# apcamargo/genomad

Hardware: AMD Instinct MI355X
Metric: 6 kbp windows classified/sec (higher is better)
Workload: dtype f16x3tk (conv2 read from a 137 GB table of all 14-mers in HBM - x2[t] is a function of the bases t-10 .. t+3 -, head A's pair products from an (entry, 9-mer) table, head A's y @ w_v rows from a 9-mer table, all exact f32; conv3 by Toom-Cook F(3,6) with split-f16 MFMA, 3 products per operand pair, f3

## Files before the change

genomad_amd/_lib.py:

```python
import ctypes as C
import os
from pathlib import Path

_HERE = Path(__file__).resolve().parent
LIB_PATH = Path(os.environ.get("GENOMAD_AMD_LIB", _HERE / "csrc" / "libgenomad_nn_hip.so"))

WINDOW, TOKENS, DEPTH, CH = 6000, 5997, 257, 128
PATCHES, PATCH_SIZE, POOLED, FEAT, HIDDEN, CLASSES = 2100, 4, 749, 256, 512, 3
EMBED_DIM = 512
EMB_F32, EMB_BF16 = 0, 1
EMB_DTYPES = {"f32": EMB_F32, "bf16": EMB_BF16}

PREC_F32, PREC_BF16X3, PREC_BF16, PREC_F16C8, PREC_F16X3, PREC_F16C6, PREC_F16X3TC, PREC_F16X3TK = 0, 1, 2, 3, 4, 5, 6, 7
PRECISIONS = {"f32": PREC_F32, "bf16x3": PREC_BF16X3, "f16x3": PREC_F16X3, "f16c6": PREC_F16C6, "f16x3tc": PREC_F16X3TC,
              "f16x3tk": PREC_F16X3TK}
OUT_OF_TOLERANCE = {"f16c6": 1.2e-4}
DEFAULT_PRECISION = "f16x3tc"
ERR_ARG, ERR_HIP, ERR_STATE, ERR_WEIGHTS, ERR_NOMEM = -1, -2, -3, -4, -5
OH_U8, OH_BF16, OH_F32 = 0, 1, 2
STRAND_FORWARD, STRAND_REVERSE, STRAND_BOTH = 0, 1, 2
STRANDS = {"forward": STRAND_FORWARD, "reverse": STRAND_REVERSE, "both": STRAND_BOTH}
K_FUSED, K_BACKEND, K_ENCODER, K_F32_FRONT, K_ATTR_HEAD, K_ATTR_CONTRIB, K_REGIONS = 0, 1, 2, 3, 4, 5, 6

_f32p = C.POINTER(C.c_float)
_i32p = C.POINTER(C.c_int32)


class IglooWeights(C.Structure):
    _fields_ = [("patches", _i32p), ("w_mult", _f32p), ("w_summer", _f32p), ("w_bias", _f32p),
                ("w_qk", _f32p), ("w_v", _f32p)]


class DenseBN(C.Structure):
    _fields_ = [("kernel", _f32p), ("bias", _f32p), ("gamma", _f32p), ("beta", _f32p),
                ("mean", _f32p), ("var", _f32p)]


class Weights(C.Structure):
    _fields_ = [("conv1_kernel", _f32p), ("conv1_bias", _f32p), ("conv2_kernel", _f32p),
                ("conv2_bias", _f32p), ("conv3_kernel", _f32p), ("conv3_bias", _f32p),
                ("igloo_a", IglooWeights), ("igloo_b", IglooWeights), ("enc", DenseBN),
                ("head", DenseBN), ("out_kernel", _f32p), ("out_bias", _f32p)]


class Taps(C.Structure):
    _fields_ = [(k, _f32p) for k in ("x1", "x2", "x3", "m_a", "m_b", "yp_a", "yp_b",
                                     "alpha_a", "alpha_b", "feat")]


_vp, _i64, _int, _sz, _u64 = C.c_void_p, C.c_int64, C.c_int, C.c_size_t, C.c_uint64
SIGNATURES = {
    "gnn_last_error": (C.c_char_p, []),
    "gnn_version": (_int, []),
    "gnn_has_experimental": (_int, []),
    "gnn_device_count": (_int, [C.POINTER(_int)]),
    "gnn_create": (_int, [_int, C.POINTER(_vp)]),
    "gnn_destroy": (_int, [_vp]),
    "gnn_sync": (_int, [_vp]),
    "gnn_device_info": (_int, [_vp, C.c_char_p, _sz, C.POINTER(_int), C.POINTER(_i64)]),
    "gnn_device_mem_info": (_int, [_vp, C.POINTER(_i64), C.POINTER(_i64)]),
    "gnn_device_pci_bus_id": (_int, [_vp, C.c_char_p, _sz]),
    "gnn_load_weights": (_int, [_vp, C.POINTER(Weights)]),
    "gnn_build_kmer_tables": (_int, [_vp, _i64]),
    "gnn_has_kmer_tables": (_int, [_vp]),
    "gnn_drop_kmer_tables": (_int, [_vp]),
    "gnn_kmer_tables_bytes": (_i64, []),
    "gnn_debug_kmer_table_row": (_int, [_vp, _int, _u64, _vp]),
    "gnn_dev_alloc": (_int, [_vp, _sz, C.POINTER(_vp)]),
    "gnn_dev_free": (_int, [_vp, _vp]),
    "gnn_memcpy_h2d": (_int, [_vp, _vp, _vp, _sz]),
    "gnn_memcpy_d2h": (_int, [_vp, _vp, _vp, _sz]),
    "gnn_tokenize": (_int, [_vp, _vp, _i64, _vp]),
    "gnn_tokenize_dev": (_int, [_vp, _vp, _i64, _vp]),
    "gnn_onehot_dev": (_int, [_vp, _vp, _i64, _int, _vp]),
    "gnn_classify": (_int, [_vp, _vp, _i64, _int, _vp]),
    "gnn_classify_dev": (_int, [_vp, _vp, _i64, _int, _vp]),
    "gnn_classify_dev_async": (_int, [_vp, _vp, _i64, _int, _vp]),
    "gnn_classify_flush": (_int, [_vp]),
    "gnn_segment_mean": (_int, [_vp, _vp, _vp, _i64, _i64, _vp]),
    "gnn_span_byte_count": (_int, [_vp, _vp, _vp, _vp, _i64, _int, _vp]),
    "gnn_classify_spans": (_int, [_vp, _vp, _vp, _vp, _i64, _int, _vp]),
    "gnn_classify_contigs": (_int, [_vp, _vp, _int, _i64, _vp, _i64, _int, _int, _vp, _vp, _i64, C.POINTER(_i64)]),
    "gnn_classify_contigs_embed": (_int, [_vp, _vp, _int, _i64, _vp, _i64, _int, _int, _vp, _vp, _i64, C.POINTER(_i64), _vp]),
    "gnn_scan_plan": (_int, [_vp, _i64, _int, _int, C.POINTER(_i64), C.POINTER(_i64), _vp, _vp, _vp, _vp]),
    "gnn_scan_contigs": (_int, [_vp, _vp, _int, _i64, _vp, _i64, _int, _int, _int, _vp, _vp, _i64, _vp, _vp, _i64, _vp]),
    "gnn_revcomp_spans_dev": (_int, [_vp, _vp, _vp, _vp, _i64, _vp]),
    "gnn_classify_contigs_strand": (_int, [_vp, _vp, _int, _i64, _vp, _i64, _int, _int, _vp, _vp, _i64, C.POINTER(_i64), _vp, _int, _vp,
                                           _vp]),
    "gnn_scan_contigs_strand": (_int, [_vp, _vp, _int, _i64, _vp, _i64, _int, _int, _int, _vp, _vp, _i64, _vp, _vp, _i64, _vp, _int, _vp,
                                       _vp]),
    "gnn_occlusion_plan": (_int, [_vp, _i64, _int, _int, C.POINTER(_i64), C.POINTER(_i64), _vp, _vp, _vp, _vp]),
    "gnn_occlude_spans_dev": (_int, [_vp, _vp, _vp, _vp, _vp, _vp, _i64, _vp]),
    "gnn_occlude_contigs": (_int, [_vp, _vp, _int, _i64, _vp, _i64, _int, _int, _int, _vp, _vp, _i64, _vp, _i64, _vp]),
    "gnn_attribute": (_int, [_vp, _vp, _i64, _int, _int, _vp, _vp, _vp, _vp]),
    "gnn_attribute_dev": (_int, [_vp, _vp, _i64, _int, _int, _vp, _vp, _vp, _vp]),
    "gnn_attribute_contigs": (_int, [_vp, _vp, _int, _i64, _vp, _i64, _int, _int, _int, _vp, _i64, _vp, _vp, _vp, _vp, _vp]),
    "gnn_call_regions": (_int, [_vp, _vp, _vp, _i64, C.c_double, _vp, _vp, _vp, _vp, _vp, _vp, _vp, _i64, C.POINTER(_i64)]),
    "gnn_region_states_dev": (_int, [_vp, _vp, _vp, _i64, C.c_double, _vp]),
    "gnn_debug_set_region_tile": (_int, [_vp, _int]),
    "gnn_embed": (_int, [_vp, _vp, _i64, _int, _int, _vp, _vp]),
    "gnn_embed_dev": (_int, [_vp, _vp, _i64, _int, _int, _vp, _vp]),
    "gnn_debug_forward": (_int, [_vp, _vp, _i64, _int, _vp, C.POINTER(Taps)]),
    "gnn_synth_windows_dev": (_int, [_vp, _u64, _i64, _i64, _vp]),
    "gnn_profile_enable": (_int, [_vp, _int]),
    "gnn_profile_reset": (_int, [_vp]),
    "gnn_profile_get": (_int, [_vp, _int, C.POINTER(C.c_double), C.POINTER(_i64)]),
    "gnn_set_chunk": (_int, [_vp, _i64]),
    "gnn_phase_cycles": (_int, [_vp, _int, C.POINTER(C.c_uint64)]),
    "gnn_mfma_probe": (_int, [_vp, _int, C.POINTER(C.c_double)]),
    "gnn_mfma_probe_kind": (_int, [_vp, _int, _int, C.POINTER(C.c_double)]),
    "gnn_fused_rows_per_step": (_int, [_int]),
    "gnn_debug_set_pad_skip": (_int, [_vp, _int]),
    "gnn_debug_set_time_split": (_int, [_vp, _int]),
    "gnn_debug_last_split": (_int, [_vp, C.POINTER(_int)]),
    "gnn_debug_pack_c6": (_int, [_f32p, _int, _int, C.POINTER(C.c_uint32), _sz, C.POINTER(_sz)]),
    "gnn_crc32c": (C.c_uint32, [_vp, _sz]),
    "gnn_fasta_scan": (_int, [_vp, _i64, C.POINTER(C.c_int64), C.POINTER(C.c_int64), C.POINTER(C.c_int)]),
    "gnn_fasta_pack": (_int, [_vp, _i64, _int, _vp, _vp, _vp, _vp, _i64, C.POINTER(C.c_int64)]),
    "gnn_fasta_accession_digests": (_int, [_vp, _i64, _vp, _i64, C.POINTER(C.c_int64), C.POINTER(C.c_int)]),
    "gnn_comm_unique_id": (_int, [_vp]),
    "gnn_comm_init": (_int, [_vp, _int, _int, _vp]),
    "gnn_comm_destroy": (_int, [_vp]),
    "gnn_comm_info": (_int, [_vp, C.POINTER(_int), C.POINTER(_int)]),
    "gnn_comm_gather_dev": (_int, [_vp, _vp, _vp, _sz, _int]),
    "gnn_comm_gather": (_int, [_vp, _vp, _vp, _sz, _int]),
    "gnn_comm_allgather": (_int, [_vp, _vp, _vp, _sz]),
    "gnn_comm_allreduce_max": (_int, [_vp, C.POINTER(C.c_double), _int]),
    "gnn_comm_barrier": (_int, [_vp]),
    "gnn_branch_attention": (_int, [_vp, _vp, _vp, _vp, _i64, C.c_double, _vp]),
    "gnn_score_calibration": (_int, [_vp, _vp, _vp, _vp, _vp, _vp, _vp, _vp, _vp, _i64, _vp]),
}

_lib = None


class GnnError(RuntimeError):
    pass


def load():
    global _lib
    if _lib is not None:
        return _lib
    if not LIB_PATH.is_file():
        raise GnnError(
            f"{LIB_PATH} not found: build it with genomad_amd/csrc/build.sh (or "
            "python -c 'import __graft_entry__ as g; g.build()').  There is no CPU fallback.")
    lib = C.CDLL(str(LIB_PATH))
    for name, (res, args) in SIGNATURES.items():
        fn = getattr(lib, name)
        fn.restype, fn.argtypes = res, args
    _lib = lib
    return lib


def check(rc: int):
    if rc != 0:
        msg = load().gnn_last_error()
        raise GnnError(f"libgenomad_nn_hip error {rc}: {msg.decode() if msg else '?'}")
```

genomad_amd/csrc/gnn_api.hip:

```cpp
#include <algorithm>
#include <map>
#include <mutex>
#include <cstdio>
#include <cmath>
#include <cstdlib>
#include <cstring>

#include "gnn_common.h"

namespace gnn {

static thread_local std::string g_last_error;
void set_error(const std::string& msg) { g_last_error = msg; }

bool debug_switch(const char* name) {
    static std::mutex mu;
    static std::map<std::string, bool> seen;
    std::lock_guard<std::mutex> lock(mu);
    auto it = seen.find(name);
    if (it != seen.end()) return it->second;
    const bool on = std::getenv(name) != nullptr;
    if (on)
        std::fprintf(stderr, "libgenomad_nn_hip: debug switch %s is set: NOT the production path (ordering or arithmetic may differ)\n", name);
    seen[name] = on;
    return on;
}

static void free_ws(Workspace& ws) { ws = Workspace(); }

constexpr size_t WS_BYTES_PER_WINDOW = ((size_t)2 * NPAIR + 2 * NP + (size_t)2 * POOLED * C + 4 * POOLED + FEAT) * sizeof(float);
constexpr int64_t MIN_CHUNK = 256;

static int ensure_ws(gnn_ctx* ctx, Workspace& ws, int64_t chunk, int64_t x_chunk) {
    if (ws.chunk < chunk || ws.x_chunk < x_chunk) {
        if (ctx->stream2) GNN_HIP(hipStreamSynchronize(ctx->stream2));
        ctx->back_pending[0] = ctx->back_pending[1] = false;
    }
    if (ws.chunk < chunk) {
        GNN_HIP(hipStreamSynchronize(ctx->stream));
        int rc = ws.mp.reserve((size_t)chunk * 2 * NPAIR);
        if (!rc) rc = ws.m.reserve((size_t)chunk * 2 * NP);
        if (!rc) rc = ws.yp.reserve((size_t)chunk * 2 * POOLED * C);
        if (!rc) rc = ws.logits.reserve((size_t)chunk * 2 * POOLED);
        if (!rc) rc = ws.alpha.reserve((size_t)chunk * 2 * POOLED);
        if (!rc) rc = ws.feat.reserve((size_t)chunk * FEAT);
        if (rc) {
            free_ws(ws);
            return rc;
        }
        ws.chunk = chunk;
    }
    if (ws.x_chunk < x_chunk) {
        GNN_HIP(hipStreamSynchronize(ctx->stream));
        ws.x_chunk = 0;
        for (DevBuf<float>& x : ws.x) x.reset();
        ws.tokens.reset();
        int rc = GNN_OK;
        for (DevBuf<float>& x : ws.x)
            if (!rc) rc = x.reserve((size_t)x_chunk * T * C);
        if (!rc) rc = ws.tokens.reserve((size_t)x_chunk * T);
        if (rc) {
            free_ws(ws);
            return rc;
        }
        ws.x_chunk = x_chunk;
    }
    return GNN_OK;
}

int flush_backend(gnn_ctx* ctx) {
    for (int i = 0; i < 2; ++i)
        if (ctx->back_pending[i]) {
            GNN_HIP(hipStreamWaitEvent(ctx->stream, ctx->ev_back[i], 0));
            ctx->back_pending[i] = false;
        }
    return GNN_OK;
}

int finish_pending(gnn_ctx* ctx) {
    if (ctx->back_pending[0] || ctx->back_pending[1]) {
        GNN_HIP(hipStreamSynchronize(ctx->stream2));
        ctx->back_pending[0] = ctx->back_pending[1] = false;
    }
    return GNN_OK;
}

int check_ctx(gnn_ctx* ctx, bool flush) {
    if (!ctx) {
        set_error("ctx is NULL");
        return GNN_ERR_ARG;
    }
    GNN_HIP(hipSetDevice(ctx->device));
    if (!flush) return GNN_OK;
    static const bool event_wait = debug_switch("GNN_ASYNC_EVENT_WAIT");
    return event_wait ? flush_backend(ctx) : finish_pending(ctx);
}

void build_conv1_pair_tables(const float* k1, std::vector<float>& pt) {
    pt.assign((size_t)3 * PAIR_ROWS * C, 0.f);
    auto row = [&](int j, int r) { return &pt[((size_t)j * PAIR_ROWS + r) * C]; };
    auto add = [&](float* dst, int k, int tok) {
        const float* src = k1 + ((size_t)k * GNN_DEPTH + tok) * C;
        for (int c = 0; c < C; ++c) dst[c] += src[c];
    };
    for (int j = 0; j < 3; ++j) {
        for (int code5 = 0; code5 < 1024; ++code5) {
            add(row(j, code5), 2 * j, 1 + (code5 >> 2));
            add(row(j, code5), 2 * j + 1, 1 + (code5 & 255));
        }
        for (int b = 1; b <= 256; ++b) {
            add(row(j, 1024 + b - 1), 2 * j, 0);
            add(row(j, 1024 + b - 1), 2 * j + 1, b);
        }
        for (int a = 1; a <= 256; ++a) {
            add(row(j, 1280 + a - 1), 2 * j, a);
            add(row(j, 1280 + a - 1), 2 * j + 1, 0);
        }
        add(row(j, 1536), 2 * j, 0);
        add(row(j, 1536), 2 * j + 1, 0);
        for (int b = 0; b <= 256; ++b) add(row(j, 1538 + b), 2 * j + 1, b);
    }
}

constexpr int64_t STAGE_MAX_WINDOWS = 32768;
constexpr size_t PIN_BYTES = (size_t)8 << 20;

static int64_t stage_windows(const gnn_ctx* ctx) {
    return (int64_t)std::min({ctx->stage_bases.capacity() / W, ctx->stage_scores.capacity() / GNN_CLASSES,
                              ctx->stage_scores_host.capacity() / GNN_CLASSES});
}

void free_stage(gnn_ctx* ctx) {
    ctx->stage_bases.reset();
    ctx->stage_scores.reset();
    ctx->stage_scores_host.reset();
    ctx->stage_emb.reset();
    ctx->emb_scores.reset();
    ctx->stage_attr.reset();
    for (int i = 0; i < 2; ++i) {
        ctx->pin[i].reset();
        if (ctx->pin_ev[i]) (void)hipEventDestroy(ctx->pin_ev[i]);
        ctx->pin_ev[i] = nullptr;
        ctx->pin_busy[i] = false;
    }
}

static int ensure_stage(gnn_ctx* ctx, int64_t windows) {
    int rc;
    for (int i = 0; i < 2; ++i)
        if (!ctx->pin[i]) {
            if ((rc = ctx->pin[i].reserve(PIN_BYTES))) return rc;
            GNN_HIP(hipEventCreateWithFlags(&ctx->pin_ev[i], hipEventDisableTiming));
        }
    const int64_t have = stage_windows(ctx);
    if (have >= windows) return GNN_OK;
    GNN_HIP(hipStreamSynchronize(ctx->stream));
    const size_t want = (size_t)std::max<int64_t>(windows, std::min<int64_t>(2 * have, STAGE_MAX_WINDOWS));
    ctx->stage_bases.reset();
    ctx->stage_scores.reset();
    ctx->stage_scores_host.reset();
    rc = ctx->stage_bases.reserve(want * W);
    if (!rc) rc = ctx->stage_scores.reserve(want * GNN_CLASSES);
    if (!rc && (rc = ctx->stage_scores_host.reserve(want * GNN_CLASSES))) set_error("hipHostMalloc of the score landing buffer failed");
    if (rc) {
        ctx->stage_bases.reset();
        ctx->stage_scores.reset();
    }
    return rc;
}

static int stage_upload(gnn_ctx* ctx, const uint8_t* src, size_t bytes) {
    int j = 0;
    for (size_t off = 0; off < bytes; off += PIN_BYTES, j ^= 1) {
        const size_t len = std::min(PIN_BYTES, bytes - off);
        if (ctx->pin_busy[j]) GNN_HIP(hipEventSynchronize(ctx->pin_ev[j]));
        std::memcpy(ctx->pin[j], src + off, len);
        GNN_HIP(hipMemcpyAsync(ctx->stage_bases + off, ctx->pin[j], len, hipMemcpyHostToDevice, ctx->stream));
        GNN_HIP(hipEventRecord(ctx->pin_ev[j], ctx->stream));
        ctx->pin_busy[j] = true;
    }
    return GNN_OK;
}

size_t emb_elem_bytes(int emb_dtype) {
    return emb_dtype == GNN_EMB_F32 ? sizeof(float) : emb_dtype == GNN_EMB_BF16 ? sizeof(uint16_t) : 0;
}

int classify_chunks(gnn_ctx* ctx, const uint8_t* bases_dev, int64_t n, int precision, float* scores_dev, bool defer_last,
                    void* emb_dev, int emb_dtype, const AttribOut* attr) {
    if (!ctx->has_weights) {
        set_error("gnn_load_weights has not been called");
        return GNN_ERR_STATE;
    }
    if (precision == GNN_PREC_BF16 || precision == GNN_PREC_F16C8) {
        set_error(std::string(precision == GNN_PREC_BF16 ? "GNN_PREC_BF16" : "GNN_PREC_F16C8") +
                  " was removed in round 6 (it fails the 1e-4 score tolerance; the enum value is kept so that old callers get this error)");
        return GNN_ERR_STATE;
    }
    if (precision != GNN_PREC_F32 && precision != GNN_PREC_BF16X3 && precision != GNN_PREC_F16X3 && precision != GNN_PREC_F16C6 &&
        precision != GNN_PREC_F16X3TC && precision != GNN_PREC_F16X3TK) {
        set_error("unknown precision " + std::to_string(precision));
        return GNN_ERR_ARG;
    }
    if (precision == GNN_PREC_F16X3TK && !(ctx->w.tk_x2_tbl && ctx->w.tk_mpa_tbl)) {
        set_error("GNN_PREC_F16X3TK needs the k-mer tables: call gnn_build_kmer_tables first (it answers GNN_ERR_NOMEM on a device without ~190 GB free)");
        return GNN_ERR_STATE;
    }
    const bool f32 = precision == GNN_PREC_F32;
    int64_t chunk = std::min<int64_t>(f32 ? ctx->chunk_f32 : ctx->chunk_fused, std::max<int64_t>(n, 1));
    if (!f32 && ctx->ws.chunk < chunk) {
        if (!ctx->chunk_explicit) {
            size_t free_b = 0, total_b = 0;
            if (hipMemGetInfo(&free_b, &total_b) == hipSuccess) {
                const int64_t cap = std::max<int64_t>(MIN_CHUNK, (int64_t)(free_b / 4 / WS_BYTES_PER_WINDOW) / MIN_CHUNK * MIN_CHUNK);
                if (cap < chunk) {
                    std::fprintf(stderr, "libgenomad_nn_hip: %lld windows per launch need %.1f GB of workspace, %.1f GB of device memory are free: "
                                 "using launches of %lld windows (gnn_set_chunk overrides)\n", (long long)chunk,
                                 chunk * (double)WS_BYTES_PER_WINDOW / 1e9, free_b / 1e9, (long long)cap);
                    chunk = cap;
                }
            }
        }
    }
    int rc = ensure_ws(ctx, ctx->ws, chunk, f32 ? chunk : 0);
    while (rc == GNN_ERR_NOMEM && !f32 && chunk > MIN_CHUNK) {
        chunk = std::max<int64_t>(MIN_CHUNK, chunk / 2);
        std::fprintf(stderr, "libgenomad_nn_hip: workspace allocation failed, retrying with launches of %lld windows\n", (long long)chunk);
        rc = ensure_ws(ctx, ctx->ws, chunk, 0);
    }
    if (rc) return rc;
    if (!f32 && chunk < std::min<int64_t>(ctx->chunk_fused, std::max<int64_t>(n, 1))) ctx->chunk_fused = chunk;
    if (attr && ctx->attr_g.capacity() < (size_t)chunk * FEAT * GNN_CLASSES) {
        if (ctx->stream2) GNN_HIP(hipStreamSynchronize(ctx->stream2));
        GNN_HIP(hipStreamSynchronize(ctx->stream));
        if ((rc = ctx->attr_g.reserve((size_t)chunk * FEAT * GNN_CLASSES))) return rc;
    }
    static const bool allow_overlap = !debug_switch("GNN_NO_BACKEND_OVERLAP");
    static const bool chunk_overlap = debug_switch("GNN_BACKEND_OVERLAP");
    const bool pending = ctx->back_pending[0] || ctx->back_pending[1];
    if (pending && (f32 || !allow_overlap)) {
        if ((rc = flush_backend(ctx))) return rc;
    }
    bool overlap = allow_overlap && !f32 && ((chunk_overlap && n > chunk) || defer_last || pending);
    if (overlap && ctx->alt_failed_chunk > 0 && chunk >= ctx->alt_failed_chunk && ctx->ws_alt.chunk < chunk) {
        if ((rc = flush_backend(ctx))) return rc;
        overlap = false;
    }
    if (overlap && (rc = ensure_ws(ctx, ctx->ws_alt, chunk, 0)) == GNN_ERR_NOMEM) {
        std::fprintf(stderr, "libgenomad_nn_hip: no device memory for the second workspace of %lld windows: asynchronous calls run in order "
                     "(back end not overlapped) from here on\n", (long long)chunk);
        ctx->alt_failed_chunk = chunk;
        if ((rc = flush_backend(ctx))) return rc;
        overlap = false;
    } else if (rc) {
        return rc;
    }
    if (overlap) {
        if (!ctx->stream2) {
            GNN_HIP(hipStreamCreateWithFlags(&ctx->stream2, hipStreamNonBlocking));
            for (int i = 0; i < 2; ++i) {
                GNN_HIP(hipEventCreateWithFlags(&ctx->ev_front[i], hipEventDisableTiming));
                GNN_HIP(hipEventCreateWithFlags(&ctx->ev_back[i], hipEventDisableTiming));
            }
        }
    }
    struct StreamGuard {
        gnn_ctx* c;
        hipStream_t main;
        ~StreamGuard() { c->stream = main; }
    } guard{ctx, ctx->stream};
    for (int64_t a = 0; a < n; a += chunk) {
        const int64_t m = std::min(chunk, n - a);
        const uint8_t* b = bases_dev + a * W;
        if (!f32 && (reinterpret_cast<uintptr_t>(b) & 3u)) {
            if (ctx->align_buf.capacity() < (size_t)m * W) {
                GNN_HIP(hipStreamSynchronize(guard.main));
                if ((rc = ctx->align_buf.reserve((size_t)chunk * W))) return rc;
            }
            GNN_HIP(hipMemcpyAsync(ctx->align_buf, b, (size_t)m * W, hipMemcpyDeviceToDevice, guard.main));
            b = ctx->align_buf;
        }
        const int buf = ctx->buf_cur;
        if (overlap && ctx->back_pending[buf]) {
            GNN_HIP(hipStreamWaitEvent(guard.main, ctx->ev_back[buf], 0));
            ctx->back_pending[buf] = false;
        }
        static const bool poison = debug_switch("GNN_DEBUG_POISON");
        if (poison) {
            const Workspace& ws = ctx->ws;
            const size_t mm = (size_t)std::min<int64_t>(m, ws.chunk);
            auto fill = [&](float* p, size_t per_window) -> int {
                if (p && mm) GNN_HIP(hipMemsetAsync(p, 0xFF, mm * per_window * sizeof(float), guard.main));
                return GNN_OK;
            };
            if ((rc = fill(ws.mp, 2 * NPAIR)) || (rc = fill(ws.m, 2 * NP)) || (rc = fill(ws.yp, (size_t)2 * POOLED * C)) ||
                (rc = fill(ws.logits, 2 * POOLED)) || (rc = fill(ws.alpha, 2 * POOLED)) || (rc = fill(ws.feat, FEAT)))
                return rc;
            if (emb_dev)
                GNN_HIP(hipMemsetAsync(static_cast<uint8_t*>(emb_dev) + (size_t)a * HID * emb_elem_bytes(emb_dtype), 0xFF,
                                       (size_t)m * HID * emb_elem_bytes(emb_dtype), guard.main));
        }
        if (f32) {
            ProfScope ps(ctx, GNN_K_F32_FRONT);
            if ((rc = launch_front_f32(ctx, b, m))) return rc;
        } else {
            ProfScope ps(ctx, GNN_K_FUSED);
            rc = precision == GNN_PREC_F16X3TK ? launch_front_tk(ctx, b, m)
                 : precision == GNN_PREC_F16X3TC ? launch_front_tc(ctx, b, m)
                 : precision == GNN_PREC_F16C6 ? launch_front_c6(ctx, b, m)
                                               : launch_front_x3(ctx, b, m, precision);
            if (rc) return rc;
        }
        if (overlap) {
            GNN_HIP(hipEventRecord(ctx->ev_front[buf], guard.main));
            ctx->stream = ctx->stream2;
            GNN_HIP(hipStreamWaitEvent(ctx->stream2, ctx->ev_front[buf], 0));
        }
        {
            ProfScope ps(ctx, GNN_K_BACKEND);
            void* emb = emb_dev ? static_cast<uint8_t*>(emb_dev) + (size_t)a * HID * emb_elem_bytes(emb_dtype) : nullptr;
            rc = launch_backend(ctx, m, (precision == GNN_PREC_F16X3TC || precision == GNN_PREC_F16X3TK) ? GNN_PREC_F16X3 : precision,
                                scores_dev ? scores_dev + a * GNN_CLASSES : nullptr, emb, emb_dtype, !attr);
        }
        if (attr && !rc) {
            ProfScope ps(ctx, GNN_K_ATTR_HEAD);
            rc = launch_attrib_head(ctx, m, scores_dev ? scores_dev + a * GNN_CLASSES : nullptr, *attr, a);
        }
        if (attr && !rc) {
            ProfScope ps(ctx, GNN_K_ATTR_CONTRIB);
            rc = launch_attrib_contrib(ctx, m, *attr, a);
        }
        if (overlap) {
            if (!rc) {
                GNN_HIP(hipEventRecord(ctx->ev_back[buf], ctx->stream2));
                ctx->back_pending[buf] = true;
            }
            ctx->stream = guard.main;
            std::swap(ctx->ws, ctx->ws_alt);
            ctx->buf_cur ^= 1;
        }
        if (rc) return rc;
    }
    return defer_last ? GNN_OK : flush_backend(ctx);
}

int check_embed_precision(int precision, const char* fn) {
    if (precision != GNN_PREC_F16C6) return GNN_OK;
    set_error(std::string(fn) + ": GNN_PREC_F16C6 has no embedding path (the frozen mode's dense head runs on the matrix pipe "
              "and is outside the tolerance); use f16x3tc, f16x3tk, f16x3, bf16x3 or f32");
    return GNN_ERR_ARG;
}

}

using namespace gnn;

extern "C" {

const char* gnn_last_error(void) { return g_last_error.c_str(); }

int gnn_version(void) { return 300; }

int gnn_debug_pack_c6(const float* w, int k, int n, uint32_t* out, size_t out_words, size_t* need_words) {
    std::vector<uint32_t> v;
    const int rc = c6_pack_matrix(w, k, n, v);
    if (rc) {
        set_error("gnn_debug_pack_c6: w is NULL or K is not a multiple of 128 or N not a multiple of 32");
        return rc;
    }
    if (need_words) *need_words = v.size();
    if (out) {
        if (out_words < v.size()) {
            set_error("gnn_debug_pack_c6: output buffer too small");
            return GNN_ERR_ARG;
        }
        std::memcpy(out, v.data(), v.size() * sizeof(uint32_t));
    }
    return GNN_OK;
}

int gnn_debug_set_pad_skip(gnn_ctx* ctx, int on) {
    int rc = check_ctx(ctx);
    if (rc) return rc;
    ctx->c6_pad_skip = on != 0;
    return GNN_OK;
}

int gnn_debug_set_time_split(gnn_ctx* ctx, int on) {
    int rc = check_ctx(ctx);
    if (rc) return rc;
    ctx->time_split = on != 0;
    return GNN_OK;
}

int gnn_debug_last_split(gnn_ctx* ctx, int* workgroups_per_window) {
    if (!ctx || !workgroups_per_window) {
        set_error("bad argument to gnn_debug_last_split");
        return GNN_ERR_ARG;
    }
    *workgroups_per_window = ctx->last_split;
    return GNN_OK;
}

int gnn_fused_rows_per_step(int precision) {
    switch (precision) {
        case GNN_PREC_F32: return 0;
        case GNN_PREC_F16C6: return c6_rows_per_step();
        case GNN_PREC_F16X3TC: case GNN_PREC_F16X3TK: return 96;
        case GNN_PREC_BF16X3: case GNN_PREC_F16X3: return FT;
        default: return GNN_ERR_ARG;
    }
}

uint32_t gnn_crc32c(const void* data, size_t n) {
    struct Table {
        uint32_t t[8][256];
        Table() {
            for (uint32_t i = 0; i < 256; ++i) {
                uint32_t c = i;
                for (int k = 0; k < 8; ++k) c = (c >> 1) ^ (0x82F63B78u & (0u - (c & 1u)));
                t[0][i] = c;
            }
            for (uint32_t i = 0; i < 256; ++i)
                for (int s = 1; s < 8; ++s) t[s][i] = (t[s - 1][i] >> 8) ^ t[0][t[s - 1][i] & 0xFF];
        }
    };
    static const Table table;
    const uint32_t(*tab)[256] = table.t;
    const unsigned char* p = static_cast<const unsigned char*>(data);
    uint32_t c = 0xFFFFFFFFu;
    while (n >= 8) {
        uint32_t lo, hi;
        std::memcpy(&lo, p, 4);
        std::memcpy(&hi, p + 4, 4);
        lo ^= c;
        c = tab[7][lo & 0xFF] ^ tab[6][(lo >> 8) & 0xFF] ^ tab[5][(lo >> 16) & 0xFF] ^ tab[4][lo >> 24] ^
            tab[3][hi & 0xFF] ^ tab[2][(hi >> 8) & 0xFF] ^ tab[1][(hi >> 16) & 0xFF] ^ tab[0][hi >> 24];
        p += 8;
        n -= 8;
    }
    while (n--) c = (c >> 8) ^ tab[0][(c ^ *p++) & 0xFF];
    return c ^ 0xFFFFFFFFu;
}

int gnn_device_count(int* count) {
    if (!count) {
        set_error("count is NULL");
        return GNN_ERR_ARG;
    }
    GNN_HIP(hipGetDeviceCount(count));
    return GNN_OK;
}

int gnn_create(int device, gnn_ctx** out) {
    if (!out) {
        set_error("out is NULL");
        return GNN_ERR_ARG;
    }
    *out = nullptr;
    int count = 0;
    GNN_HIP(hipGetDeviceCount(&count));
    if (device < 0 || device >= count) {
        set_error("device " + std::to_string(device) + " out of range (" + std::to_string(count) + " visible)");
        return GNN_ERR_ARG;
    }
    GNN_HIP(hipSetDevice(device));
    hipDeviceProp_t prop;
    GNN_HIP(hipGetDeviceProperties(&prop, device));
    if (std::string(prop.gcnArchName).rfind("gfx950", 0) != 0) {
        set_error(std::string("this library is built for gfx950 only; device is ") + prop.gcnArchName);
        return GNN_ERR_HIP;
    }
    gnn_ctx* ctx = new gnn_ctx();
    ctx->device = device;
    ctx->c6_pad_skip = !debug_switch("GNN_NO_PAD_SKIP");
    ctx->time_split = !debug_switch("GNN_NO_TIME_SPLIT");
    ctx->cu_count = prop.multiProcessorCount;
    hipError_t e = hipStreamCreateWithFlags(&ctx->stream, hipStreamNonBlocking);
    if (e != hipSuccess) {
        set_error(std::string("hipStreamCreate failed: ") + hipGetErrorString(e));
        delete ctx;
        return GNN_ERR_HIP;
    }
    *out = ctx;
    return GNN_OK;
}

int gnn_destroy(gnn_ctx* ctx) {
    if (!ctx) return GNN_OK;
    (void)hipSetDevice(ctx->device);
    if (ctx->stream2) (void)hipStreamSynchronize(ctx->stream2);
    (void)hipStreamSynchronize(ctx->stream);
    if (ctx->comm || ctx->comm_scratch) (void)gnn_comm_destroy(ctx);
    free_contig_ws(ctx);
    free_stage(ctx);
    if (ctx->stream2) {
        for (int i = 0; i < 2; ++i) {
            if (ctx->ev_front[i]) (void)hipEventDestroy(ctx->ev_front[i]);
            if (ctx->ev_back[i]) (void)hipEventDestroy(ctx->ev_back[i]);
        }
        (void)hipStreamDestroy(ctx->stream2);
    }
    for (auto& s : ctx->prof)
        for (auto& pr : s.pending) {
            (void)hipEventDestroy(pr.first);
            (void)hipEventDestroy(pr.second);
        }
    for (hipEvent_t e : ctx->event_pool) (void)hipEventDestroy(e);
    (void)hipStreamDestroy(ctx->stream);
    delete ctx;
    return GNN_OK;
}

int gnn_sync(gnn_ctx* ctx) {
    int rc = check_ctx(ctx);
    if (rc) return rc;
    GNN_HIP(hipStreamSynchronize(ctx->stream));
    return GNN_OK;
}

int gnn_device_info(gnn_ctx* ctx, char* name, size_t name_len, int* cus, int64_t* hbm_bytes) {
    int rc = check_ctx(ctx);
    if (rc) return rc;
    hipDeviceProp_t prop;
    GNN_HIP(hipGetDeviceProperties(&prop, ctx->device));
    if (name && name_len) {
        std::string s = std::string(prop.name) + " (" + prop.gcnArchName + ")";
        std::strncpy(name, s.c_str(), name_len - 1);
        name[name_len - 1] = 0;
    }
    if (cus) *cus = prop.multiProcessorCount;
    if (hbm_bytes) *hbm_bytes = (int64_t)prop.totalGlobalMem;
    return GNN_OK;
}

int gnn_device_pci_bus_id(gnn_ctx* ctx, char* out, size_t out_len) {
    int rc = check_ctx(ctx, false);
    if (rc) return rc;
    if (!out || out_len < 16) {
        set_error("gnn_device_pci_bus_id: out must hold at least 16 bytes");
        return GNN_ERR_ARG;
    }
    GNN_HIP(hipDeviceGetPCIBusId(out, (int)out_len, ctx->device));
    return GNN_OK;
}

int gnn_device_mem_info(gnn_ctx* ctx, int64_t* free_bytes, int64_t* total_bytes) {
    int rc = check_ctx(ctx);
    if (rc) return rc;
    size_t f = 0, t = 0;
    GNN_HIP(hipMemGetInfo(&f, &t));
    if (free_bytes) *free_bytes = (int64_t)f;
    if (total_bytes) *total_bytes = (int64_t)t;
    return GNN_OK;
}

int gnn_set_chunk(gnn_ctx* ctx, int64_t windows_per_chunk) {
    if (!ctx || windows_per_chunk < 1) {
        set_error("bad chunk");
        return GNN_ERR_ARG;
    }
    ctx->chunk_fused = windows_per_chunk;
    ctx->chunk_explicit = true;
    return GNN_OK;
}

int gnn_load_weights(gnn_ctx* ctx, const gnn_weights* w) {
    int rc = check_ctx(ctx);
    if (rc) return rc;
    if (!w) {
        set_error("weights is NULL");
        return GNN_ERR_ARG;
    }
    const void* req[] = {w->conv1_kernel, w->conv1_bias, w->conv2_kernel, w->conv2_bias, w->conv3_kernel,
                         w->conv3_bias,   w->out_kernel, w->out_bias,     w->enc.kernel,  w->enc.bias,
                         w->enc.gamma,    w->enc.beta,   w->enc.mean,     w->enc.var,     w->head.kernel,
                         w->head.bias,    w->head.gamma, w->head.beta,    w->head.mean,   w->head.var};
    for (const void* p : req)
        if (!p) {
            set_error("a weight pointer is NULL");
            return GNN_ERR_ARG;
        }
    if (ctx->has_weights) {
        set_error("weights already loaded into this ctx (create a new ctx)");
        return GNN_ERR_STATE;
    }
    DeviceWeights& d = ctx->w;
    if ((rc = upload(ctx, w->conv1_kernel, (size_t)KS * GNN_DEPTH * C, &d.conv1_k))) return rc;
    if ((rc = upload(ctx, w->conv1_bias, (size_t)C, &d.conv1_b))) return rc;
    const float* ck[2] = {w->conv2_kernel, w->conv3_kernel};
    const float* cb[2] = {w->conv2_bias, w->conv3_bias};
    for (int i = 0; i < 2; ++i) {
        if ((rc = upload(ctx, ck[i], (size_t)KS * C * C, &d.conv_k[i]))) return rc;
        if ((rc = upload(ctx, cb[i], (size_t)C, &d.conv_b[i]))) return rc;
    }
    const gnn_igloo_weights* ig[2] = {&w->igloo_a, &w->igloo_b};
    for (int h = 0; h < 2; ++h) {
        const gnn_igloo_weights* g = ig[h];
        if (!g->patches || !g->w_mult || !g->w_summer || !g->w_bias || !g->w_qk || !g->w_v) {
            set_error("an IGLOO weight pointer is NULL");
            return GNN_ERR_ARG;
        }
        std::vector<int32_t> order(NPAIR);
        for (int i = 0; i < NPAIR; ++i) {
            const int32_t t = g->patches[i];
            if (t < 0 || t >= T) {
                set_error("patch index out of range [0,5997)");
                return GNN_ERR_WEIGHTS;
            }
            order[i] = i;
        }
        std::stable_sort(order.begin(), order.end(),
                         [&](int32_t a, int32_t b) { return g->patches[a] < g->patches[b]; });
        std::vector<float> weff((size_t)NPAIR * C);
        std::vector<int32_t> pos(NPAIR), slot(NPAIR), ptr(FSTEPS + 1, 0);
        for (int e = 0; e < NPAIR; ++e) {
            const int pair = order[e], j = pair % PS;
            pos[e] = g->patches[pair];
            slot[pair] = e;
            ptr[pos[e] / FT + 1] += 1;
            for (int c = 0; c < C; ++c)
                weff[(size_t)e * C + c] = g->w_mult[(size_t)pair * C + c] * g->w_summer[j * C + c];
        }
        for (int s2 = 0; s2 < FSTEPS; ++s2) ptr[s2 + 1] += ptr[s2];
        if ((rc = upload(ctx, weff.data(), weff.size(), &d.weff_sorted[h]))) return rc;
        if ((rc = upload(ctx, pos.data(), pos.size(), &d.pos_sorted[h]))) return rc;
        if ((rc = upload(ctx, slot.data(), slot.size(), &d.slot[h]))) return rc;
        if ((rc = upload(ctx, ptr.data(), ptr.size(), &d.bucket_ptr[h]))) return rc;
        if ((rc = upload(ctx, g->w_bias, (size_t)NP, &d.w_bias[h]))) return rc;
        if ((rc = upload(ctx, g->w_qk, (size_t)NP * POOLED, &d.w_qk[h]))) return rc;
        if ((rc = upload(ctx, g->w_v, (size_t)C * C, &d.w_v[h]))) return rc;
    }
    {
        std::vector<float> pt;
        build_conv1_pair_tables(w->conv1_kernel, pt);
        if ((rc = upload(ctx, pt.data(), pt.size(), &d.conv1_pairs))) return rc;
    }
    auto fold = [&](const gnn_dense_bn& l, int in, float** dk, float** db, uint16_t** dfrag) -> int {
        std::vector<float> k((size_t)in * HID), b(HID);
        for (int o = 0; o < HID; ++o) {
            const float s = l.gamma[o] / std::sqrt(l.var[o] + BN_EPS);
            b[o] = (l.bias[o] - l.mean[o]) * s + l.beta[o];
            for (int i = 0; i < in; ++i) k[(size_t)i * HID + o] = l.kernel[(size_t)i * HID + o] * s;
        }
        int r = upload(ctx, k.data(), k.size(), dk);
        if (r) return r;
        if ((r = upload(ctx, b.data(), b.size(), db))) return r;
        const std::vector<uint16_t> fr = pack_frags(k.data(), in, HID, true);
        return upload(ctx, fr, dfrag);
    };
    if ((rc = fold(w->enc, FEAT, &d.d1_k, &d.d1_b, &d.d1_frag))) return rc;
    if ((rc = fold(w->head, HID, &d.d2_k, &d.d2_b, &d.d2_frag))) return rc;
    if ((rc = upload(ctx, w->out_kernel, (size_t)HID * GNN_CLASSES, &d.d3_k))) return rc;
    if ((rc = upload(ctx, w->out_bias, (size_t)GNN_CLASSES, &d.d3_b))) return rc;
    if ((rc = pack_fused_weights(ctx, w))) return rc;
    if ((rc = pack_fused_c6_weights(ctx, w))) return rc;
    if ((rc = pack_fused_x3_consts(ctx))) return rc;
    if ((rc = pack_fused_tc_weights(ctx, w))) return rc;
    ctx->has_weights = true;
    return GNN_OK;
}

int gnn_build_kmer_tables(gnn_ctx* ctx, int64_t reserve_bytes) {
    int rc = check_ctx(ctx);
    if (rc) return rc;
    if (!ctx->has_weights) {
        set_error("gnn_load_weights has not been called");
        return GNN_ERR_STATE;
    }
    if ((rc = finish_pending(ctx))) return rc;
    const size_t reserve = reserve_bytes >= 0 ? (size_t)reserve_bytes : 2 * (size_t)ctx->chunk_fused * WS_BYTES_PER_WINDOW + ((size_t)8 << 30);
    return build_kmer_tables(ctx, reserve);
}

int gnn_has_kmer_tables(gnn_ctx* ctx) {
    return ctx && ctx->w.tk_x2_tbl && ctx->w.tk_mpa_tbl && ctx->w.tk_pt_tbl && ctx->w.tk_x1t_tbl && ctx->w.tk_yp_const ? 1 : 0;
}

int gnn_drop_kmer_tables(gnn_ctx* ctx) {
    int rc = check_ctx(ctx);
    if (rc) return rc;
    if ((rc = finish_pending(ctx))) return rc;
    GNN_HIP(hipStreamSynchronize(ctx->stream));
    free_kmer_tables(ctx);
    return GNN_OK;
}

int64_t gnn_kmer_tables_bytes(void) { return (int64_t)kmer_tables_bytes(); }

int gnn_debug_kmer_table_row(gnn_ctx* ctx, int which, uint64_t row, float* out_host) {
    int rc = check_ctx(ctx);
    if (rc) return rc;
    if (!gnn_has_kmer_tables(ctx) || !out_host) {
        set_error("gnn_debug_kmer_table_row: no tables / NULL output");
        return GNN_ERR_STATE;
    }
    if (which == 0) {
        if (row > ((uint64_t)1 << 28)) { set_error("14-mer row out of range"); return GNN_ERR_ARG; }
        GNN_HIP(hipMemcpy(out_host, ctx->w.tk_x2_tbl + (size_t)row * C, C * sizeof(float), hipMemcpyDeviceToHost));
    } else {
        const uint64_t e = row >> 32, n = row & 0xffffffffu;
        if (e >= (uint64_t)NPAIR || n > ((uint64_t)1 << 18)) { set_error("(entry, 9-mer) out of range"); return GNN_ERR_ARG; }
        GNN_HIP(hipMemcpy(out_host, ctx->w.tk_mpa_tbl + (size_t)e * (((size_t)1 << 18) + 1) + n, sizeof(float), hipMemcpyDeviceToHost));
    }
    return GNN_OK;
}

int gnn_dev_alloc(gnn_ctx* ctx, size_t bytes, void** dev_ptr) {
    int rc = check_ctx(ctx);
    if (rc) return rc;
    if (!dev_ptr) {
        set_error("dev_ptr is NULL");
        return GNN_ERR_ARG;
    }
    DevBuf<unsigned char> b;
    if ((rc = b.reserve(bytes ? bytes : 1))) return rc;
    *dev_ptr = b.release();
    return GNN_OK;
}

int gnn_dev_free(gnn_ctx* ctx, void* dev_ptr) {
    int rc = check_ctx(ctx);
    if (rc) return rc;
    GNN_HIP(hipStreamSynchronize(ctx->stream));
    if (dev_ptr) GNN_HIP(hipFree(dev_ptr));
    return GNN_OK;
}

int gnn_memcpy_h2d(gnn_ctx* ctx, void* dst_dev, const void* src_host, size_t bytes) {
    int rc = check_ctx(ctx);
    if (rc) return rc;
    GNN_HIP(hipMemcpyAsync(dst_dev, src_host, bytes, hipMemcpyHostToDevice, ctx->stream));
    GNN_HIP(hipStreamSynchronize(ctx->stream));
    return GNN_OK;
}

int gnn_memcpy_d2h(gnn_ctx* ctx, void* dst_host, const void* src_dev, size_t bytes) {
    int rc = check_ctx(ctx);
    if (rc) return rc;
    GNN_HIP(hipMemcpyAsync(dst_host, src_dev, bytes, hipMemcpyDeviceToHost, ctx->stream));
    GNN_HIP(hipStreamSynchronize(ctx->stream));
    return GNN_OK;
}

int gnn_tokenize_dev(gnn_ctx* ctx, const uint8_t* bases_dev, int64_t n, uint16_t* tokens_dev) {
    int rc = check_ctx(ctx);
    if (rc) return rc;
    if (n < 0 || (n > 0 && (!bases_dev || !tokens_dev))) {
        set_error("bad argument to gnn_tokenize_dev");
        return GNN_ERR_ARG;
    }
    if (n == 0) return GNN_OK;
    return launch_tokenize(ctx, bases_dev, n, tokens_dev);
}

int gnn_tokenize(gnn_ctx* ctx, const uint8_t* bases_host, int64_t n, uint16_t* tokens_host) {
    int rc = check_ctx(ctx);
    if (rc) return rc;
    if (n < 0 || (n > 0 && (!bases_host || !tokens_host))) {
        set_error("bad argument to gnn_tokenize");
        return GNN_ERR_ARG;
    }
    if (n == 0) return GNN_OK;
    DevBuf<uint8_t> b;
    DevBuf<uint16_t> t;
    if ((rc = b.reserve((size_t)n * W)) || (rc = t.reserve((size_t)n * T))) return rc;
    rc = gnn_memcpy_h2d(ctx, b, bases_host, (size_t)n * W);
    if (!rc) rc = launch_tokenize(ctx, b, n, t);
    if (!rc) rc = gnn_memcpy_d2h(ctx, tokens_host, t, (size_t)n * T * sizeof(uint16_t));
    return rc;
}

int gnn_onehot_dev(gnn_ctx* ctx, const uint8_t* bases_dev, int64_t n, int dtype, void* out) {
    int rc = check_ctx(ctx);
    if (rc) return rc;
    if (n < 0 || (n > 0 && (!bases_dev || !out)) || dtype < GNN_OH_U8 || dtype > GNN_OH_F32) {
        set_error("bad argument to gnn_onehot_dev");
        return GNN_ERR_ARG;
    }
    if (n == 0) return GNN_OK;
    ProfScope ps(ctx, GNN_K_ENCODER);
    return launch_onehot(ctx, bases_dev, n, dtype, out);
}

int gnn_synth_windows_dev(gnn_ctx* ctx, uint64_t seed, int64_t first, int64_t n, uint8_t* bases_dev) {
    int rc = check_ctx(ctx);
    if (rc) return rc;
    if (n < 0 || first < 0 || (n > 0 && !bases_dev)) {
        set_error("bad argument to gnn_synth_windows_dev");
        return GNN_ERR_ARG;
    }
    if (n == 0) return GNN_OK;
    return launch_synth(ctx, seed, first, n, bases_dev);
}

int gnn_classify_dev(gnn_ctx* ctx, const uint8_t* bases_dev, int64_t n, int precision, float* scores_dev) {
    int rc = check_ctx(ctx);
    if (rc) return rc;
    if (n < 0 || (n > 0 && (!bases_dev || !scores_dev))) {
        set_error("bad argument to gnn_classify_dev");
        return GNN_ERR_ARG;
    }
    if (n == 0) return GNN_OK;
    return classify_chunks(ctx, bases_dev, n, precision, scores_dev);
}

int gnn_classify_dev_async(gnn_ctx* ctx, const uint8_t* bases_dev, int64_t n, int precision, float* scores_dev) {
    int rc = check_ctx(ctx, false);
    if (rc) return rc;
    if (n < 0 || (n > 0 && (!bases_dev || !scores_dev))) {
        set_error("bad argument to gnn_classify_dev_async");
        return GNN_ERR_ARG;
    }
    if (n == 0) return GNN_OK;
    return classify_chunks(ctx, bases_dev, n, precision, scores_dev, true);
}

int gnn_classify_flush(gnn_ctx* ctx) { return check_ctx(ctx); }

static int embed_args(int precision, int emb_dtype, const char* what) {
    if (int rc = check_embed_precision(precision, what)) return rc;
    if (!emb_elem_bytes(emb_dtype)) {
        set_error(std::string(what) + ": unknown gnn_emb_dtype " + std::to_string(emb_dtype));
        return GNN_ERR_ARG;
    }
    return GNN_OK;
}

int gnn_embed_dev(gnn_ctx* ctx, const uint8_t* bases_dev, int64_t n, int precision, int emb_dtype, void* emb_dev,
                  float* scores_dev) {
    int rc = check_ctx(ctx);
    if (rc) return rc;
    if (n < 0 || (n > 0 && (!bases_dev || !emb_dev))) {
        set_error("bad argument to gnn_embed_dev");
        return GNN_ERR_ARG;
    }
    if ((rc = embed_args(precision, emb_dtype, "gnn_embed_dev"))) return rc;
    if (n == 0) return GNN_OK;
    if (!scores_dev) {
        if (ctx->emb_scores.capacity() < (size_t)n * GNN_CLASSES) {
            GNN_HIP(hipStreamSynchronize(ctx->stream));
            if ((rc = ctx->emb_scores.reserve((size_t)n * GNN_CLASSES))) return rc;
        }
        scores_dev = ctx->emb_scores;
    }
    return classify_chunks(ctx, bases_dev, n, precision, scores_dev, false, emb_dev, emb_dtype);
}

int gnn_embed(gnn_ctx* ctx, const uint8_t* bases_host, int64_t n, int precision, int emb_dtype, void* emb_host,
              float* scores_host) {
    int rc = check_ctx(ctx);
    if (rc) return rc;
    if (n < 0 || (n > 0 && (!bases_host || !emb_host))) {
        set_error("bad argument to gnn_embed");
        return GNN_ERR_ARG;
    }
    if ((rc = embed_args(precision, emb_dtype, "gnn_embed"))) return rc;
    if (n == 0) return GNN_OK;
    const int64_t slab = std::min<int64_t>(n, STAGE_MAX_WINDOWS);
    const size_t row = (size_t)HID * emb_elem_bytes(emb_dtype);
    if ((rc = ensure_stage(ctx, slab))) return rc;
    if (ctx->stage_emb.capacity() * sizeof(float) < (size_t)slab * row) {
        GNN_HIP(hipStreamSynchronize(ctx->stream));
        if ((rc = ctx->stage_emb.reserve((size_t)slab * HID))) return rc;
    }
    for (int64_t a0 = 0; a0 < n && !rc; a0 += slab) {
        const int64_t m = std::min(slab, n - a0);
        rc = stage_upload(ctx, bases_host + a0 * W, (size_t)m * W);
        if (!rc) rc = classify_chunks(ctx, ctx->stage_bases, m, precision, ctx->stage_scores, false, ctx->stage_emb, emb_dtype);
        if (!rc) {
            if (scores_host)
                GNN_HIP(hipMemcpyAsync(ctx->stage_scores_host, ctx->stage_scores, (size_t)m * GNN_CLASSES * sizeof(float),
                                       hipMemcpyDeviceToHost, ctx->stream));
            GNN_HIP(hipMemcpyAsync(static_cast<uint8_t*>(emb_host) + (size_t)a0 * row, ctx->stage_emb, (size_t)m * row,
                                   hipMemcpyDeviceToHost, ctx->stream));
            GNN_HIP(hipStreamSynchronize(ctx->stream));
            if (scores_host)
                std::memcpy(scores_host + a0 * GNN_CLASSES, ctx->stage_scores_host, (size_t)m * GNN_CLASSES * sizeof(float));
        }
    }
    return rc;
}

int gnn_attribute_dev(gnn_ctx* ctx, const uint8_t* bases_dev, int64_t n, int precision, int bin, float* contrib_dev, float* bias_dev,
                      float* logits_dev, float* scores_dev) {
    int rc = check_ctx(ctx);
    if (rc) return rc;
    if (n < 0 || (n > 0 && (!bases_dev || !contrib_dev))) {
        set_error("bad argument to gnn_attribute_dev");
        return GNN_ERR_ARG;
    }
    if ((rc = check_attrib_args(precision, bin, "gnn_attribute_dev"))) return rc;
    if (n == 0) return GNN_OK;
    const AttribOut at{bin, contrib_dev, bias_dev, logits_dev};
    return classify_chunks(ctx, bases_dev, n, precision, scores_dev, false, nullptr, GNN_EMB_F32, &at);
}

int gnn_attribute(gnn_ctx* ctx, const uint8_t* bases_host, int64_t n, int precision, int bin, float* contrib_host, float* bias_host,
                  float* logits_host, float* scores_host) {
    int rc = check_ctx(ctx);
    if (rc) return rc;
    if (n < 0 || (n > 0 && (!bases_host || !contrib_host))) {
        set_error("bad argument to gnn_attribute");
        return GNN_ERR_ARG;
    }
    if ((rc = check_attrib_args(precision, bin, "gnn_attribute"))) return rc;
    if (n == 0) return GNN_OK;
    constexpr int64_t ATTR_SLAB = 4096;
    const int64_t slab = std::min<int64_t>(n, ATTR_SLAB);
    const size_t map = (size_t)2 * attrib_bins(bin) * GNN_CLASSES;
    if ((rc = ensure_stage(ctx, slab))) return rc;
    if (ctx->stage_attr.capacity() < (size_t)slab * (map + 2 * GNN_CLASSES)) {
        GNN_HIP(hipStreamSynchronize(ctx->stream));
        if ((rc = ctx->stage_attr.reserve((size_t)slab * (map + 2 * GNN_CLASSES)))) return rc;
    }
    float* const d_contrib = ctx->stage_attr;
    float* const d_bias = d_contrib + (size_t)slab * map;
    float* const d_logits = d_bias + (size_t)slab * GNN_CLASSES;
    const AttribOut at{bin, d_contrib, d_bias, d_logits};
    for (int64_t a0 = 0; a0 < n && !rc; a0 += slab) {
        const int64_t m = std::min(slab, n - a0);
        rc = stage_upload(ctx, bases_host + a0 * W, (size_t)m * W);
        if (!rc) rc = classify_chunks(ctx, ctx->stage_bases, m, precision, ctx->stage_scores, false, nullptr, GNN_EMB_F32, &at);
        if (!rc) {
            const size_t row = (size_t)GNN_CLASSES * sizeof(float);
            if (scores_host) GNN_HIP(hipMemcpyAsync(ctx->stage_scores_host, ctx->stage_scores, (size_t)m * row, hipMemcpyDeviceToHost, ctx->stream));
            GNN_HIP(hipMemcpyAsync(contrib_host + (size_t)a0 * map, d_contrib, (size_t)m * map * sizeof(float), hipMemcpyDeviceToHost, ctx->stream));
            if (bias_host) GNN_HIP(hipMemcpyAsync(bias_host + a0 * GNN_CLASSES, d_bias, (size_t)m * row, hipMemcpyDeviceToHost, ctx->stream));
            if (logits_host) GNN_HIP(hipMemcpyAsync(logits_host + a0 * GNN_CLASSES, d_logits, (size_t)m * row, hipMemcpyDeviceToHost, ctx->stream));
            GNN_HIP(hipStreamSynchronize(ctx->stream));
            if (scores_host) std::memcpy(scores_host + a0 * GNN_CLASSES, ctx->stage_scores_host, (size_t)m * row);
        }
    }
    return rc;
}

int gnn_classify(gnn_ctx* ctx, const uint8_t* bases_host, int64_t n, int precision, float* scores_host) {
    return gnn_debug_forward(ctx, bases_host, n, precision, scores_host, nullptr);
}

int gnn_debug_forward(gnn_ctx* ctx, const uint8_t* bases_host, int64_t n, int precision,
                      float* scores_host, const gnn_taps* taps) {
    int rc = check_ctx(ctx);
    if (rc) return rc;
    if (n < 0 || (n > 0 && (!bases_host || !scores_host))) {
        set_error("bad argument to gnn_classify");
        return GNN_ERR_ARG;
    }
    if (n == 0) return GNN_OK;
    if (taps) {
        const int64_t lim = precision == GNN_PREC_F32 ? ctx->chunk_f32 : ctx->chunk_fused;
        if (n > lim) {
            set_error("gnn_debug_forward with taps: n_windows exceeds one chunk (" + std::to_string(lim) + ")");
            return GNN_ERR_ARG;
        }
        if ((taps->x1 || taps->x2 || taps->x3) && precision != GNN_PREC_F32) {
            set_error("x1/x2/x3 taps exist only on the f32 path (the fused path keeps them in LDS)");
            return GNN_ERR_ARG;
        }
    }
    const int64_t slab = std::min<int64_t>(n, STAGE_MAX_WINDOWS);
    if ((rc = ensure_stage(ctx, slab))) return rc;
    for (int64_t a0 = 0; a0 < n && !rc; a0 += slab) {
        const int64_t m = std::min(slab, n - a0);
        rc = stage_upload(ctx, bases_host + a0 * W, (size_t)m * W);
        if (!rc) rc = classify_chunks(ctx, ctx->stage_bases, m, precision, ctx->stage_scores);
        if (!rc) {
            GNN_HIP(hipMemcpyAsync(ctx->stage_scores_host, ctx->stage_scores, (size_t)m * GNN_CLASSES * sizeof(float),
                                   hipMemcpyDeviceToHost, ctx->stream));
            GNN_HIP(hipStreamSynchronize(ctx->stream));
            std::memcpy(scores_host + a0 * GNN_CLASSES, ctx->stage_scores_host, (size_t)m * GNN_CLASSES * sizeof(float));
        }
    }
    if (!rc && taps && precision != GNN_PREC_F32 && n > ctx->chunk_fused) {
        set_error("gnn_debug_forward with taps: the launch size was reduced to " + std::to_string(ctx->chunk_fused) +
                  " windows for lack of device memory; the taps of " + std::to_string(n) + " windows do not fit one launch");
        return GNN_ERR_STATE;
    }
    if (!rc && taps) {
        const Workspace& ws = ctx->ws;
        auto out = [&](float* dst, const float* src, size_t count) {
            if (dst && !rc) rc = gnn_memcpy_d2h(ctx, dst, src, count * sizeof(float));
        };
        out(taps->x1, ws.x[0], (size_t)n * T * C);
        out(taps->x2, ws.x[1], (size_t)n * T * C);
        out(taps->x3, ws.x[2], (size_t)n * T * C);
        out(taps->feat, ws.feat, (size_t)n * FEAT);
        auto out2 = [&](float* dst_a, float* dst_b, const float* src, size_t per) {
            if ((!dst_a && !dst_b) || rc) return;
            std::vector<float> tmp((size_t)n * 2 * per);
            rc = gnn_memcpy_d2h(ctx, tmp.data(), src, tmp.size() * sizeof(float));
            if (rc) return;
            for (int64_t i = 0; i < n; ++i) {
                if (dst_a) std::memcpy(dst_a + i * per, tmp.data() + (i * 2 + 0) * per, per * sizeof(float));
                if (dst_b) std::memcpy(dst_b + i * per, tmp.data() + (i * 2 + 1) * per, per * sizeof(float));
            }
        };
        out2(taps->yp_a, taps->yp_b, ws.yp, (size_t)POOLED * C);
        out2(taps->alpha_a, taps->alpha_b, ws.alpha, (size_t)POOLED);
        out2(taps->m_a, taps->m_b, ws.m, (size_t)NP);
    }
    return rc;
}

static int upload_spans(gnn_ctx* ctx, const int64_t* starts_host, const int32_t* lens_host, int64_t n,
                        DevBuf<int64_t>& starts_dev, DevBuf<int32_t>& lens_dev) {
    for (int64_t i = 0; i < n; ++i)
        if (starts_host[i] < 0 || lens_host[i] < 0 || lens_host[i] > W) {
            set_error("span " + std::to_string(i) + " has a negative start or a length outside [0, 6000]");
            return GNN_ERR_ARG;
        }
    int rc = starts_dev.reserve((size_t)n);
    if (!rc) rc = lens_dev.reserve((size_t)n);
    if (!rc) rc = gnn_memcpy_h2d(ctx, starts_dev, starts_host, (size_t)n * sizeof(int64_t));
    if (!rc) rc = gnn_memcpy_h2d(ctx, lens_dev, lens_host, (size_t)n * sizeof(int32_t));
    return rc;
}

int gnn_span_byte_count(gnn_ctx* ctx, const uint8_t* seq_dev, const int64_t* starts_host, const int32_t* lens_host,
                        int64_t n, int byte, int32_t* counts_host) {
    int rc = check_ctx(ctx);
    if (rc) return rc;
    if (n < 0 || byte < 0 || byte > 255 || (n > 0 && (!seq_dev || !starts_host || !lens_host || !counts_host))) {
        set_error("bad argument to gnn_span_byte_count");
        return GNN_ERR_ARG;
    }
    if (n == 0) return GNN_OK;
    DevBuf<int64_t> ds;
    DevBuf<int32_t> dl, dc;
    if ((rc = upload_spans(ctx, starts_host, lens_host, n, ds, dl))) return rc;
    rc = dc.reserve((size_t)n);
    if (!rc) rc = launch_span_count(ctx, seq_dev, ds, dl, n, byte, dc);
    if (!rc) rc = gnn_memcpy_d2h(ctx, counts_host, dc, (size_t)n * sizeof(int32_t));
    return rc;
}

int gnn_classify_spans(gnn_ctx* ctx, const uint8_t* seq_dev, const int64_t* starts_host, const int32_t* lens_host,
                       int64_t n, int precision, float* scores_host) {
    int rc = check_ctx(ctx);
    if (rc) return rc;
    if (n < 0 || (n > 0 && (!seq_dev || !starts_host || !lens_host || !scores_host))) {
        set_error("bad argument to gnn_classify_spans");
        return GNN_ERR_ARG;
    }
    if (n == 0) return GNN_OK;
    DevBuf<int64_t> ds;
    DevBuf<int32_t> dl;
    if ((rc = upload_spans(ctx, starts_host, lens_host, n, ds, dl))) return rc;
    const int64_t slab = std::min<int64_t>(n, 4 * std::max<int64_t>(ctx->chunk_fused, 1));
    DevBuf<uint8_t> db;
    DevBuf<float> dsc;
    rc = db.reserve((size_t)slab * W);
    if (!rc) rc = dsc.reserve((size_t)n * GNN_CLASSES);
    for (int64_t a = 0; a < n && !rc; a += slab) {
        const int64_t m = std::min(slab, n - a);
        rc = launch_materialize(ctx, seq_dev, ds + a, dl + a, m, db);
        if (!rc) rc = classify_chunks(ctx, db, m, precision, dsc + a * GNN_CLASSES);
    }
    if (!rc) rc = gnn_memcpy_d2h(ctx, scores_host, dsc, (size_t)n * GNN_CLASSES * sizeof(float));
    return rc;
}

int gnn_revcomp_spans_dev(gnn_ctx* ctx, const uint8_t* seq_dev, const int64_t* starts_host, const int32_t* lens_host,
                          int64_t n, uint8_t* bases_dev_out) {
    int rc = check_ctx(ctx);
    if (rc) return rc;
    if (n < 0 || (n > 0 && (!seq_dev || !starts_host || !lens_host || !bases_dev_out))) {
        set_error("bad argument to gnn_revcomp_spans_dev");
        return GNN_ERR_ARG;
    }
    if ((uintptr_t)bases_dev_out & 3) {
        set_error("gnn_revcomp_spans_dev: bases_dev_out is not 4-byte aligned");
        return GNN_ERR_ARG;
    }
    if (n == 0) return GNN_OK;
    DevBuf<int64_t> ds;
    DevBuf<int32_t> dl;
    if ((rc = upload_spans(ctx, starts_host, lens_host, n, ds, dl))) return rc;
    if ((rc = launch_revcomp(ctx, seq_dev, ds, dl, n, bases_dev_out))) return rc;
    GNN_HIP(hipStreamSynchronize(ctx->stream));
    return GNN_OK;
}

int gnn_profile_enable(gnn_ctx* ctx, int on) {
    if (!ctx) {
        set_error("ctx is NULL");
        return GNN_ERR_ARG;
    }
    ctx->profile = on != 0;
    return GNN_OK;
}

static int drain_profile(gnn_ctx* ctx) {
    GNN_HIP(hipStreamSynchronize(ctx->stream));
    for (auto& s : ctx->prof) {
        for (auto& pr : s.pending) {
            float ms = 0.f;
            GNN_HIP(hipEventElapsedTime(&ms, pr.first, pr.second));
            s.total_ms += ms;
            s.launches += 1;
            ctx->event_pool.push_back(pr.first);
            ctx->event_pool.push_back(pr.second);
        }
        s.pending.clear();
    }
    return GNN_OK;
}

int gnn_phase_cycles(gnn_ctx* ctx, int on, unsigned long long* out16) {
    int rc = check_ctx(ctx);
    if (rc) return rc;
    GNN_HIP(hipStreamSynchronize(ctx->stream));
    if (out16 && ctx->phase_cycles)
        GNN_HIP(hipMemcpy(out16, ctx->phase_cycles, 16 * sizeof(unsigned long long), hipMemcpyDeviceToHost));
    if (on) {
        if ((rc = ctx->phase_cycles.reserve(16))) return rc;
        GNN_HIP(hipMemset(ctx->phase_cycles, 0, 16 * sizeof(unsigned long long)));
    } else {
        ctx->phase_cycles.reset();
    }
    return GNN_OK;
}

int gnn_profile_reset(gnn_ctx* ctx) {
    int rc = check_ctx(ctx);
    if (rc) return rc;
    if ((rc = drain_profile(ctx))) return rc;
    for (auto& s : ctx->prof) {
        s.total_ms = 0.0;
        s.launches = 0;
    }
    return GNN_OK;
}

int gnn_profile_get(gnn_ctx* ctx, int kernel_id, double* total_ms, int64_t* launches) {
    int rc = check_ctx(ctx);
    if (rc) return rc;
    if (kernel_id < 0 || kernel_id >= GNN_K_COUNT) {
        set_error("bad kernel id");
        return GNN_ERR_ARG;
    }
    if ((rc = drain_profile(ctx))) return rc;
    if (total_ms) *total_ms = ctx->prof[kernel_id].total_ms;
    if (launches) *launches = ctx->prof[kernel_id].launches;
    return GNN_OK;
}

}
```

genomad_amd/csrc/gnn_backend.hip:

```cpp
#include <cstdlib>

#include "gnn_common.h"

namespace gnn {

__global__ __launch_bounds__(256) void m_kernel(const float* __restrict__ mp, const float* __restrict__ w_bias0,
                                                const float* __restrict__ w_bias1,
                                                const int32_t* __restrict__ slot0,
                                                const int32_t* __restrict__ slot1, float* __restrict__ m) {
    __shared__ float s[NPAIR];
    const int wi = blockIdx.x, h = blockIdx.y;
    const float* w_bias = h ? w_bias1 : w_bias0;
    const int32_t* slot = h ? slot1 : slot0;
    const float4* src = reinterpret_cast<const float4*>(mp + ((size_t)wi * 2 + h) * NPAIR);
    for (int i = threadIdx.x; i < NPAIR / 4; i += 256) reinterpret_cast<float4*>(s)[i] = src[i];
    __syncthreads();
    for (int p = threadIdx.x; p < NP; p += 256) {
        const int4 sl = reinterpret_cast<const int4*>(slot)[p];
        m[((size_t)wi * 2 + h) * NP + p] = w_bias[p] + s[sl.x] + s[sl.y] + s[sl.z] + s[sl.w];
    }
}

constexpr int LW = 64, LQ = 128, LK = 16;

__global__ __launch_bounds__(256) void logits_kernel(const float* __restrict__ m,
                                                     const float* __restrict__ w_qk0,
                                                     const float* __restrict__ w_qk1, int n,
                                                     float* __restrict__ logits) {
    __shared__ __attribute__((aligned(16))) float ms[LK][LW + 4];
    __shared__ __attribute__((aligned(16))) float qs[LK][LQ];
    const int h = blockIdx.z;
    const float* w_qk = h ? w_qk1 : w_qk0;
    const int w0 = blockIdx.y * LW;
    const int q0 = blockIdx.x * LQ;
    const int tw = threadIdx.x >> 4;
    const int tq = threadIdx.x & 15;
    float acc[4][8];
#pragma unroll
    for (int i = 0; i < 4; ++i)
#pragma unroll
        for (int k = 0; k < 8; ++k) acc[i][k] = 0.f;
    for (int p0 = 0; p0 < NP; p0 += LK) {
        {
            const int w = threadIdx.x >> 2, pq = (threadIdx.x & 3) * 4;
            float4 v = make_float4(0.f, 0.f, 0.f, 0.f);
            if (w0 + w < n && p0 + pq < NP)
                v = *reinterpret_cast<const float4*>(m + ((size_t)(w0 + w) * 2 + h) * NP + p0 + pq);
            ms[pq][w] = v.x;
            ms[pq + 1][w] = v.y;
            ms[pq + 2][w] = v.z;
            ms[pq + 3][w] = v.w;
        }
        for (int i = threadIdx.x; i < LK * LQ; i += 256) {
            const int q = i % LQ, p = i / LQ;
            qs[p][q] = (p0 + p < NP && q0 + q < POOLED) ? w_qk[(size_t)(p0 + p) * POOLED + q0 + q] : 0.f;
        }
        __syncthreads();
#pragma unroll 4
        for (int p = 0; p < LK; ++p) {
            const float4 a = *reinterpret_cast<const float4*>(&ms[p][tw * 4]);
            const float4 b0 = *reinterpret_cast<const float4*>(&qs[p][tq * 4]);
            const float4 b1 = *reinterpret_cast<const float4*>(&qs[p][64 + tq * 4]);
            const float av[4] = {a.x, a.y, a.z, a.w};
            const float bv[8] = {b0.x, b0.y, b0.z, b0.w, b1.x, b1.y, b1.z, b1.w};
#pragma unroll
            for (int i = 0; i < 4; ++i)
#pragma unroll
                for (int k = 0; k < 8; ++k) acc[i][k] = fmaf(av[i], bv[k], acc[i][k]);
        }
        __syncthreads();
    }
#pragma unroll
    for (int i = 0; i < 4; ++i) {
        const int w = w0 + tw * 4 + i;
        if (w >= n) continue;
#pragma unroll
        for (int k = 0; k < 8; ++k) {
            const int q = q0 + (k >> 2) * 64 + tq * 4 + (k & 3);
            if (q < POOLED) logits[((size_t)w * 2 + h) * POOLED + q] = acc[i][k];
        }
    }
}

typedef __bf16 bf16x8 __attribute__((ext_vector_type(8)));
typedef float f32x16 __attribute__((ext_vector_type(16)));

struct QkA {
    float4 v[2][2];
};
struct QkB {
    uint4 v[2][2];
};

__device__ __forceinline__ void qk_load(QkA& a, QkB& b, const float* __restrict__ mrow0, const float* __restrict__ mrow1,
                                        const uint4* __restrict__ bfrag, int ks, int lane) {
    const int k = ks * 16 + (lane >> 5) * 8;
    const float* rows[2] = {mrow0, mrow1};
#pragma unroll
    for (int mb = 0; mb < 2; ++mb) {
        if (k + 8 <= NP) {
            a.v[mb][0] = *reinterpret_cast<const float4*>(rows[mb] + k);
            a.v[mb][1] = *reinterpret_cast<const float4*>(rows[mb] + k + 4);
        } else {
            float t[8];
#pragma unroll
            for (int e = 0; e < 8; ++e) t[e] = k + e < NP ? rows[mb][k + e] : 0.f;
            a.v[mb][0] = make_float4(t[0], t[1], t[2], t[3]);
            a.v[mb][1] = make_float4(t[4], t[5], t[6], t[7]);
        }
    }
    const uint4* bp = bfrag + (size_t)ks * (QK_NBLK * 2 * 64);
#pragma unroll
    for (int nb = 0; nb < 2; ++nb) {
        b.v[nb][0] = bp[nb * 2 * 64];
        b.v[nb][1] = bp[nb * 2 * 64 + 64];
    }
}

template <int PASSES, bool F16>
__device__ __forceinline__ void qk_mfma(const QkA& a, const QkB& b, f32x16 (&acc)[2][2]) {
    typedef float f32x8 __attribute__((ext_vector_type(8)));
    typedef _Float16 f16x8q __attribute__((ext_vector_type(8)));
#pragma unroll
    for (int mb = 0; mb < 2; ++mb) {
        const f32x8 x = {a.v[mb][0].x, a.v[mb][0].y, a.v[mb][0].z, a.v[mb][0].w,
                         a.v[mb][1].x, a.v[mb][1].y, a.v[mb][1].z, a.v[mb][1].w};
        if constexpr (F16) {
            const f16x8q ah = __builtin_convertvector(x, f16x8q);
            const f16x8q al = __builtin_convertvector(x - __builtin_convertvector(ah, f32x8), f16x8q);
#pragma unroll
            for (int nb = 0; nb < 2; ++nb) {
                const f16x8q bh = __builtin_bit_cast(f16x8q, b.v[nb][0]);
                if constexpr (PASSES == 3) {
                    const f16x8q bl = __builtin_bit_cast(f16x8q, b.v[nb][1]);
                    acc[mb][nb] = __builtin_amdgcn_mfma_f32_32x32x16_f16(ah, bl, acc[mb][nb], 0, 0, 0);
                    acc[mb][nb] = __builtin_amdgcn_mfma_f32_32x32x16_f16(al, bh, acc[mb][nb], 0, 0, 0);
                }
                acc[mb][nb] = __builtin_amdgcn_mfma_f32_32x32x16_f16(ah, bh, acc[mb][nb], 0, 0, 0);
            }
        } else {
            const bf16x8 ah = __builtin_convertvector(x, bf16x8);
            const bf16x8 al = __builtin_convertvector(x - __builtin_convertvector(ah, f32x8), bf16x8);
#pragma unroll
            for (int nb = 0; nb < 2; ++nb) {
                const bf16x8 bh = __builtin_bit_cast(bf16x8, b.v[nb][0]);
                if constexpr (PASSES == 3) {
                    const bf16x8 bl = __builtin_bit_cast(bf16x8, b.v[nb][1]);
                    acc[mb][nb] = __builtin_amdgcn_mfma_f32_32x32x16_bf16(ah, bl, acc[mb][nb], 0, 0, 0);
                    acc[mb][nb] = __builtin_amdgcn_mfma_f32_32x32x16_bf16(al, bh, acc[mb][nb], 0, 0, 0);
                }
                acc[mb][nb] = __builtin_amdgcn_mfma_f32_32x32x16_bf16(ah, bh, acc[mb][nb], 0, 0, 0);
            }
        }
    }
}

template <int PASSES, bool F16 = false>
__global__ __launch_bounds__(256) void logits_mfma_kernel(const float* __restrict__ m, const uint4* __restrict__ frag0,
                                                          const uint4* __restrict__ frag1, int n,
                                                          float* __restrict__ logits) {
    const int lane = threadIdx.x & 63, wave = threadIdx.x >> 6;
    const int h = blockIdx.z;
    const int w0 = blockIdx.y * 64;
    const int nb0 = blockIdx.x * 8 + wave * 2;
    const uint4* bfrag = (h ? frag1 : frag0) + (size_t)nb0 * 2 * 64 + lane;
    const float* mrow0 = m + ((size_t)min(w0 + (lane & 31), n - 1) * 2 + h) * NP;
    const float* mrow1 = m + ((size_t)min(w0 + 32 + (lane & 31), n - 1) * 2 + h) * NP;
    f32x16 acc[2][2];
#pragma unroll
    for (int i = 0; i < 2; ++i)
#pragma unroll
        for (int j = 0; j < 2; ++j)
#pragma unroll
            for (int r = 0; r < 16; ++r) acc[i][j][r] = 0.f;
    QkA a0, a1;
    QkB b0, b1;
    qk_load(a0, b0, mrow0, mrow1, bfrag, 0, lane);
#pragma unroll 1
    for (int ks = 0; ks < QK_KSTEPS; ks += 2) {
        qk_load(a1, b1, mrow0, mrow1, bfrag, ks + 1, lane);
        qk_mfma<PASSES, F16>(a0, b0, acc);
        qk_load(a0, b0, mrow0, mrow1, bfrag, min(ks + 2, QK_KSTEPS - 1), lane);
        qk_mfma<PASSES, F16>(a1, b1, acc);
    }
#pragma unroll
    for (int mb = 0; mb < 2; ++mb)
#pragma unroll
        for (int r = 0; r < 16; ++r) {
            const int w = w0 + mb * 32 + (r & 3) + 8 * (r >> 2) + 4 * (lane >> 5);
            if (w >= n) continue;
#pragma unroll
            for (int nb = 0; nb < 2; ++nb) {
                const int q = (nb0 + nb) * 32 + (lane & 31);
                if (q < POOLED) logits[((size_t)w * 2 + h) * POOLED + q] = acc[mb][nb][r];
            }
        }
}

__global__ __launch_bounds__(256) void attn_kernel(const float* __restrict__ logits,
                                                   const float* __restrict__ yp,
                                                   float* __restrict__ alpha_out,
                                                   float* __restrict__ feat) {
    __shared__ float a[POOLED + 3];
    __shared__ float red[256];
    const int wi = blockIdx.x, h = blockIdx.y;
    const float* lg = logits + ((size_t)wi * 2 + h) * POOLED;
    float mx = -INFINITY;
    for (int q = threadIdx.x; q < POOLED; q += 256) {
        const float v = lg[q];
        a[q] = v;
        mx = fmaxf(mx, v);
    }
    red[threadIdx.x] = mx;
    __syncthreads();
    for (int s = 128; s > 0; s >>= 1) {
        if (threadIdx.x < s) red[threadIdx.x] = fmaxf(red[threadIdx.x], red[threadIdx.x + s]);
        __syncthreads();
    }
    mx = red[0];
    __syncthreads();
    float sum = 0.f;
    for (int q = threadIdx.x; q < POOLED; q += 256) {
        const float e = expf(a[q] - mx);
        a[q] = e;
        sum += e;
    }
    red[threadIdx.x] = sum;
    __syncthreads();
    for (int s = 128; s > 0; s >>= 1) {
        if (threadIdx.x < s) red[threadIdx.x] += red[threadIdx.x + s];
        __syncthreads();
    }
    const float inv = 1.f / red[0];
    __syncthreads();
    for (int q = threadIdx.x; q < POOLED; q += 256) {
        const float v = a[q] * inv;
        a[q] = v;
        alpha_out[((size_t)wi * 2 + h) * POOLED + q] = v;
    }
    __syncthreads();
    const int cq = threadIdx.x & 31, g = threadIdx.x >> 5;
    const float4* y = reinterpret_cast<const float4*>(yp + ((size_t)wi * 2 + h) * POOLED * C) + cq;
    float4 acc = make_float4(0.f, 0.f, 0.f, 0.f);
    int q = g;
    for (; q + 24 < POOLED; q += 32) {
        typedef float ntf4 __attribute__((ext_vector_type(4)));
        const ntf4* yn = reinterpret_cast<const ntf4*>(y);
        const ntf4 v0 = __builtin_nontemporal_load(yn + (size_t)q * (C / 4)), v1 = __builtin_nontemporal_load(yn + (size_t)(q + 8) * (C / 4)),
                   v2 = __builtin_nontemporal_load(yn + (size_t)(q + 16) * (C / 4)), v3 = __builtin_nontemporal_load(yn + (size_t)(q + 24) * (C / 4));
        const float a0 = a[q], a1 = a[q + 8], a2 = a[q + 16], a3 = a[q + 24];
        acc.x = fmaf(a0, v0.x, acc.x); acc.y = fmaf(a0, v0.y, acc.y); acc.z = fmaf(a0, v0.z, acc.z); acc.w = fmaf(a0, v0.w, acc.w);
        acc.x = fmaf(a1, v1.x, acc.x); acc.y = fmaf(a1, v1.y, acc.y); acc.z = fmaf(a1, v1.z, acc.z); acc.w = fmaf(a1, v1.w, acc.w);
        acc.x = fmaf(a2, v2.x, acc.x); acc.y = fmaf(a2, v2.y, acc.y); acc.z = fmaf(a2, v2.z, acc.z); acc.w = fmaf(a2, v2.w, acc.w);
        acc.x = fmaf(a3, v3.x, acc.x); acc.y = fmaf(a3, v3.y, acc.y); acc.z = fmaf(a3, v3.z, acc.z); acc.w = fmaf(a3, v3.w, acc.w);
    }
    for (; q < POOLED; q += 8) {
        const float4 v = y[(size_t)q * (C / 4)];
        const float aq = a[q];
        acc.x = fmaf(aq, v.x, acc.x); acc.y = fmaf(aq, v.y, acc.y); acc.z = fmaf(aq, v.z, acc.z); acc.w = fmaf(aq, v.w, acc.w);
    }
    __shared__ float4 part[8][32];
    part[g][cq] = acc;
    __syncthreads();
    if (threadIdx.x < 128) {
        const int c = threadIdx.x;
        float s = 0.f;
#pragma unroll
        for (int k = 0; k < 8; ++k) s += reinterpret_cast<const float*>(&part[k][c >> 2])[c & 3];
        feat[(size_t)wi * FEAT + h * C + c] = s;
    }
}

constexpr int DW = 8;

__device__ __forceinline__ uint16_t f32_to_bf16_rne(float v) {
    const uint32_t u = __float_as_uint(v);
    if ((u & 0x7fffffffu) > 0x7f800000u) return (uint16_t)((u >> 16) | 0x0040u);
    return (uint16_t)((u + 0x7fffu + ((u >> 16) & 1u)) >> 16);
}

template <int EMB>
__global__ __launch_bounds__(512) void dense_kernel(const float* __restrict__ feat,
                                                    const float* __restrict__ d1k, const float* __restrict__ d1b,
                                                    const float* __restrict__ d2k, const float* __restrict__ d2b,
                                                    const float* __restrict__ d3k, const float* __restrict__ d3b,
                                                    int n, float* __restrict__ scores, void* __restrict__ emb) {
    __shared__ float f[DW][FEAT];
    __shared__ float h1[DW][HID];
    __shared__ float h2[DW][HID];
    __shared__ float lg[DW][4];
    const int w0 = blockIdx.x * DW;
    const int j = threadIdx.x;
    for (int i = j; i < DW * FEAT; i += 512) {
        const int w = i / FEAT, k = i % FEAT;
        f[w][k] = (w0 + w < n) ? feat[(size_t)(w0 + w) * FEAT + k] : 0.f;
    }
    __syncthreads();
    float acc[DW];
#pragma unroll
    for (int w = 0; w < DW; ++w) acc[w] = d1b[j];
    for (int k = 0; k < FEAT; ++k) {
        const float wv = d1k[(size_t)k * HID + j];
#pragma unroll
        for (int w = 0; w < DW; ++w) acc[w] = fmaf(f[w][k], wv, acc[w]);
    }
#pragma unroll
    for (int w = 0; w < DW; ++w) h1[w][j] = acc[w] < 0.f ? 0.f : acc[w];
    if constexpr (EMB == GNN_EMB_F32 + 1) {
#pragma unroll
        for (int w = 0; w < DW; ++w)
            if (w0 + w < n) static_cast<float*>(emb)[(size_t)(w0 + w) * HID + j] = acc[w] < 0.f ? 0.f : acc[w];
    } else if constexpr (EMB == GNN_EMB_BF16 + 1) {
#pragma unroll
        for (int w = 0; w < DW; ++w)
            if (w0 + w < n) static_cast<uint16_t*>(emb)[(size_t)(w0 + w) * HID + j] = f32_to_bf16_rne(acc[w] < 0.f ? 0.f : acc[w]);
    }
    __syncthreads();
#pragma unroll
    for (int w = 0; w < DW; ++w) acc[w] = d2b[j];
    for (int k = 0; k < HID; ++k) {
        const float wv = d2k[(size_t)k * HID + j];
#pragma unroll
        for (int w = 0; w < DW; ++w) acc[w] = fmaf(h1[w][k], wv, acc[w]);
    }
#pragma unroll
    for (int w = 0; w < DW; ++w) h2[w][j] = acc[w] < 0.f ? 0.f : acc[w];
    __syncthreads();
    const int wave = j >> 6, lane = j & 63;
    for (int o = wave; o < DW * GNN_CLASSES; o += 8) {
        const int w = o / GNN_CLASSES, cl = o % GNN_CLASSES;
        float s = 0.f;
        for (int k = lane; k < HID; k += 64) s = fmaf(h2[w][k], d3k[(size_t)k * GNN_CLASSES + cl], s);
#pragma unroll
        for (int off = 32; off >= 1; off >>= 1) s += __shfl_xor(s, off, 64);
        if (lane == 0) lg[w][cl] = s + d3b[cl];
    }
    __syncthreads();
    if (j < DW && w0 + j < n) {
        const float a = lg[j][0], b = lg[j][1], c = lg[j][2];
        const float mx = fmaxf(a, fmaxf(b, c));
        const float ea = expf(a - mx), eb = expf(b - mx), ec = expf(c - mx);
        const float inv = 1.f / (ea + eb + ec);
        float* o = scores + (size_t)(w0 + j) * GNN_CLASSES;
        o[0] = ea * inv;
        o[1] = eb * inv;
        o[2] = ec * inv;
    }
}

constexpr int DM_MB = 1;
constexpr int DM_ROWS = 32 * DM_MB;
constexpr int DM_STRIDE = HID + 4;

template <int KSTEPS, bool FROM_LDS>
__device__ __forceinline__ void dense_mfma_layer(const float* __restrict__ a0, int row_stride, const uint4* __restrict__ frag,
                                                 int wave, int lane, f32x16 (&acc)[DM_MB][4]) {
    typedef float f32x8 __attribute__((ext_vector_type(8)));
    typedef _Float16 f16x8 __attribute__((ext_vector_type(8)));
#pragma unroll
    for (int i = 0; i < DM_MB; ++i)
#pragma unroll
        for (int j = 0; j < 4; ++j)
#pragma unroll
            for (int r = 0; r < 16; ++r) acc[i][j][r] = 0.f;
#pragma unroll 2
    for (int ks = 0; ks < KSTEPS; ++ks) {
        const int k = ks * 16 + (lane >> 5) * 8;
        f16x8 ah[DM_MB], al[DM_MB];
#pragma unroll
        for (int mb = 0; mb < DM_MB; ++mb) {
            const float4 lo4 = *reinterpret_cast<const float4*>(a0 + mb * row_stride + k), hi4 = *reinterpret_cast<const float4*>(a0 + mb * row_stride + k + 4);
            const f32x8 x = {lo4.x, lo4.y, lo4.z, lo4.w, hi4.x, hi4.y, hi4.z, hi4.w};
            ah[mb] = __builtin_convertvector(x, f16x8);
            al[mb] = __builtin_convertvector(x - __builtin_convertvector(ah[mb], f32x8), f16x8);
        }
        const uint4* bp = frag + ((size_t)ks * (HID / 32) + wave * 4) * 2 * 64 + lane;
#pragma unroll
        for (int nb = 0; nb < 4; ++nb) {
            const f16x8 bh = __builtin_bit_cast(f16x8, bp[nb * 2 * 64]), bl = __builtin_bit_cast(f16x8, bp[nb * 2 * 64 + 64]);
#pragma unroll
            for (int mb = 0; mb < DM_MB; ++mb) {
                acc[mb][nb] = __builtin_amdgcn_mfma_f32_32x32x16_f16(ah[mb], bl, acc[mb][nb], 0, 0, 0);
                acc[mb][nb] = __builtin_amdgcn_mfma_f32_32x32x16_f16(al[mb], bh, acc[mb][nb], 0, 0, 0);
                acc[mb][nb] = __builtin_amdgcn_mfma_f32_32x32x16_f16(ah[mb], bh, acc[mb][nb], 0, 0, 0);
            }
        }
    }
}

__device__ __forceinline__ void dense_mfma_store(float* __restrict__ hs, const float* __restrict__ bias, int wave, int lane,
                                                 const f32x16 (&acc)[DM_MB][4]) {
#pragma unroll
    for (int nb = 0; nb < 4; ++nb) {
        const int col = (wave * 4 + nb) * 32 + (lane & 31);
        const float b = bias[col];
#pragma unroll
        for (int mb = 0; mb < DM_MB; ++mb)
#pragma unroll
            for (int r = 0; r < 16; ++r) {
                const int row = mb * 32 + (r & 3) + 8 * (r >> 2) + 4 * (lane >> 5);
                const float v = acc[mb][nb][r] + b;
                hs[row * DM_STRIDE + col] = v < 0.f ? 0.f : v;
            }
    }
}

__global__ __launch_bounds__(256) void dense_mfma_kernel(const float* __restrict__ feat, const uint4* __restrict__ f1,
                                                         const float* __restrict__ d1b, const uint4* __restrict__ f2,
                                                         const float* __restrict__ d2b, const float* __restrict__ d3k,
                                                         const float* __restrict__ d3b, int n, float* __restrict__ scores) {
    __shared__ __attribute__((aligned(16))) float hs[DM_ROWS * DM_STRIDE];
    __shared__ float lg[DM_ROWS][4];
    const int lane = threadIdx.x & 63, wave = threadIdx.x >> 6;
    const int w0 = blockIdx.x * DM_ROWS;
    f32x16 acc[DM_MB][4];
    static_assert(DM_MB == 1, "the first layer's row clamp is written for one 32-window block per workgroup");
    dense_mfma_layer<FEAT / 16, false>(feat + (size_t)min(w0 + (lane & 31), n - 1) * FEAT, 32 * FEAT, f1, wave, lane, acc);
    dense_mfma_store(hs, d1b, wave, lane, acc);
    __syncthreads();
    dense_mfma_layer<HID / 16, true>(hs + (lane & 31) * DM_STRIDE, 32 * DM_STRIDE, f2, wave, lane, acc);
    __syncthreads();
    dense_mfma_store(hs, d2b, wave, lane, acc);
    __syncthreads();
    for (int o = wave; o < DM_ROWS * GNN_CLASSES; o += 4) {
        const int w = o / GNN_CLASSES, cl = o % GNN_CLASSES;
        float s = 0.f;
        for (int k = lane; k < HID; k += 64) s = fmaf(hs[w * DM_STRIDE + k], d3k[(size_t)k * GNN_CLASSES + cl], s);
#pragma unroll
        for (int off = 32; off >= 1; off >>= 1) s += __shfl_xor(s, off, 64);
        if (lane == 0) lg[w][cl] = s + d3b[cl];
    }
    __syncthreads();
    const int j = threadIdx.x;
    if (j < DM_ROWS && w0 + j < n) {
        const float a = lg[j][0], b = lg[j][1], c = lg[j][2];
        const float mx = fmaxf(a, fmaxf(b, c));
        const float ea = expf(a - mx), eb = expf(b - mx), ec = expf(c - mx);
        const float inv = 1.f / (ea + eb + ec);
        float* o = scores + (size_t)(w0 + j) * GNN_CLASSES;
        o[0] = ea * inv;
        o[1] = eb * inv;
        o[2] = ec * inv;
    }
}

int launch_backend(gnn_ctx* ctx, int64_t n, int precision, float* scores_dev, void* emb_dev, int emb_dtype, bool dense) {
    if (emb_dev && (precision == GNN_PREC_F16C6 || precision == GNN_PREC_F16C8 || (emb_dtype != GNN_EMB_F32 && emb_dtype != GNN_EMB_BF16))) {
        set_error("embeddings: the dense head of this arithmetic does not produce them (f16c6 is frozen), or a bad gnn_emb_dtype");
        return GNN_ERR_ARG;
    }
    const DeviceWeights& d = ctx->w;
    Workspace& ws = ctx->ws;
    hipLaunchKernelGGL(m_kernel, dim3((unsigned)n, 2), dim3(256), 0, ctx->stream, ws.mp, d.w_bias[0], d.w_bias[1],
                       d.slot[0], d.slot[1], ws.m);
    static_assert(QK_KSTEPS % 2 == 0 && QK_NBLK % 8 == 0, "logits_mfma_kernel tiling");
    static const bool logits_f32 = debug_switch("GNN_LOGITS_F32");
    const dim3 qk_grid(QK_NBLK / 8, (unsigned)((n + 63) / 64), 2);
    const uint4* qf0 = reinterpret_cast<const uint4*>(d.wqk_frag[0]);
    const uint4* qf1 = reinterpret_cast<const uint4*>(d.wqk_frag[1]);
    if (precision == GNN_PREC_BF16X3 || precision == GNN_PREC_F16C8 || precision == GNN_PREC_F16C6)
        hipLaunchKernelGGL(logits_mfma_kernel<3>, qk_grid, dim3(256), 0, ctx->stream, ws.m, qf0, qf1, (int)n, ws.logits);
    else if (precision == GNN_PREC_BF16)
        hipLaunchKernelGGL(logits_mfma_kernel<1>, qk_grid, dim3(256), 0, ctx->stream, ws.m, qf0, qf1, (int)n, ws.logits);
    else if (precision == GNN_PREC_F16X3 && !logits_f32)
        hipLaunchKernelGGL((logits_mfma_kernel<3, true>), qk_grid, dim3(256), 0, ctx->stream, ws.m,
                           reinterpret_cast<const uint4*>(d.wqk_frag_h[0]), reinterpret_cast<const uint4*>(d.wqk_frag_h[1]), (int)n, ws.logits);
    else
        hipLaunchKernelGGL(logits_kernel, dim3((POOLED + LQ - 1) / LQ, (unsigned)((n + LW - 1) / LW), 2), dim3(256), 0,
                           ctx->stream, ws.m, d.w_qk[0], d.w_qk[1], (int)n, ws.logits);
    hipLaunchKernelGGL(attn_kernel, dim3((unsigned)n, 2), dim3(256), 0, ctx->stream, ws.logits, ws.yp, ws.alpha,
                       ws.feat);
    if (!dense) {
        GNN_HIP(hipGetLastError());
        return GNN_OK;
    }
    if (precision != GNN_PREC_F16C6 && precision != GNN_PREC_F16C8) {
        const dim3 grid((unsigned)((n + DW - 1) / DW));
        if (!emb_dev)
            hipLaunchKernelGGL(dense_kernel<0>, grid, dim3(512), 0, ctx->stream, ws.feat, d.d1_k, d.d1_b, d.d2_k, d.d2_b, d.d3_k,
                               d.d3_b, (int)n, scores_dev, nullptr);
        else if (emb_dtype == GNN_EMB_F32)
            hipLaunchKernelGGL(dense_kernel<GNN_EMB_F32 + 1>, grid, dim3(512), 0, ctx->stream, ws.feat, d.d1_k, d.d1_b, d.d2_k, d.d2_b,
                               d.d3_k, d.d3_b, (int)n, scores_dev, emb_dev);
        else
            hipLaunchKernelGGL(dense_kernel<GNN_EMB_BF16 + 1>, grid, dim3(512), 0, ctx->stream, ws.feat, d.d1_k, d.d1_b, d.d2_k, d.d2_b,
                               d.d3_k, d.d3_b, (int)n, scores_dev, emb_dev);
    } else {
        hipLaunchKernelGGL(dense_mfma_kernel, dim3((unsigned)((n + DM_ROWS - 1) / DM_ROWS)), dim3(256), 0, ctx->stream, ws.feat,
                           reinterpret_cast<const uint4*>(d.d1_frag), d.d1_b, reinterpret_cast<const uint4*>(d.d2_frag), d.d2_b,
                           d.d3_k, d.d3_b, (int)n, scores_dev);
    }
    GNN_HIP(hipGetLastError());
    return GNN_OK;
}

__global__ void segment_mean_kernel(const float* __restrict__ scores, const int64_t* __restrict__ ids,
                                    int64_t n, int64_t n_seg, float* __restrict__ out) {
    const int64_t i = (int64_t)blockIdx.x * blockDim.x + threadIdx.x;
    if (i >= n_seg * GNN_CLASSES) return;
    const int64_t seg = i / GNN_CLASSES;
    const int cl = (int)(i % GNN_CLASSES);
    int64_t lo = 0, hi = n;
    while (lo < hi) {
        const int64_t mid = (lo + hi) >> 1;
        if (ids[mid] < seg) lo = mid + 1; else hi = mid;
    }
    const int64_t a = lo;
    hi = n;
    while (lo < hi) {
        const int64_t mid = (lo + hi) >> 1;
        if (ids[mid] <= seg) lo = mid + 1; else hi = mid;
    }
    float s = 0.f;
    for (int64_t k = a; k < lo; ++k) s += scores[k * GNN_CLASSES + cl];
    out[i] = lo > a ? s / (float)(lo - a) : 0.f;
}

}

using namespace gnn;

extern "C" int gnn_segment_mean(gnn_ctx* ctx, const float* scores_host, const int64_t* ids_host, int64_t n,
                                int64_t n_segments, float* out_host) {
    if (!ctx || n < 0 || n_segments < 0 || (n > 0 && (!scores_host || !ids_host)) ||
        (n_segments > 0 && !out_host)) {
        set_error("bad argument to gnn_segment_mean");
        return GNN_ERR_ARG;
    }
    if (n_segments == 0) return GNN_OK;
    for (int64_t i = 1; i < n; ++i)
        if (ids_host[i] < ids_host[i - 1]) {
            set_error("segment ids are not sorted");
            return GNN_ERR_ARG;
        }
    if (n > 0 && (ids_host[0] < 0 || ids_host[n - 1] >= n_segments)) {
        set_error("segment id out of range");
        return GNN_ERR_ARG;
    }
    GNN_HIP(hipSetDevice(ctx->device));
    DevBuf<float> ds, dout;
    DevBuf<int64_t> di;
    int rc = ds.reserve(std::max<size_t>(1, (size_t)n * GNN_CLASSES));
    if (!rc) rc = di.reserve(std::max<size_t>(1, (size_t)n));
    if (!rc) rc = dout.reserve((size_t)n_segments * GNN_CLASSES);
    auto step = [&](hipError_t e, const char* what) {
        if (rc == GNN_OK && e != hipSuccess) {
            set_error(std::string(what) + " failed: " + hipGetErrorString(e));
            rc = GNN_ERR_HIP;
        }
    };
    if (n > 0 && rc == GNN_OK) {
        step(hipMemcpyAsync(ds, scores_host, (size_t)n * GNN_CLASSES * sizeof(float), hipMemcpyHostToDevice, ctx->stream), "copy scores");
        step(hipMemcpyAsync(di, ids_host, (size_t)n * sizeof(int64_t), hipMemcpyHostToDevice, ctx->stream), "copy ids");
    }
    if (rc == GNN_OK) {
        const int64_t threads = n_segments * GNN_CLASSES;
        hipLaunchKernelGGL(segment_mean_kernel, dim3((unsigned)((threads + 255) / 256)), dim3(256), 0, ctx->stream,
                           ds.get(), di.get(), n, n_segments, dout.get());
        step(hipGetLastError(), "segment_mean launch");
        step(hipMemcpyAsync(out_host, dout, (size_t)n_segments * GNN_CLASSES * sizeof(float), hipMemcpyDeviceToHost, ctx->stream), "copy out");
        step(hipStreamSynchronize(ctx->stream), "sync");
    }
    return rc;
}
```

genomad_amd/csrc/gnn_common.h:

```cpp
#pragma once
#include <hip/hip_runtime.h>
#include <stdint.h>
#include <algorithm>
#include <string>
#include <vector>

#include "../../include/genomad_nn.h"
#include "gnn_devmem.h"

namespace gnn {

constexpr int W = GNN_WINDOW;
constexpr int T = GNN_TOKENS;
constexpr int C = GNN_CH;
constexpr int KS = GNN_KSIZE;
constexpr int NP = GNN_PATCHES;
constexpr int PS = GNN_PATCH_SIZE;
constexpr int NPAIR = NP * PS;
constexpr int POOLED = GNN_POOLED;
constexpr int FEAT = GNN_FEAT;
constexpr int HID = GNN_HIDDEN;
constexpr float LRELU = 0.1f;
constexpr float BN_EPS = 1e-3f;

constexpr int FT = 128;
constexpr int FSTEPS = (T + FT - 1) / FT;
constexpr int PAIR_ROWS = 1024 + 256 + 256 + 1 + 1 + 257;
constexpr int QK_KSTEPS = (NP + 15) / 16;
constexpr int QK_NBLK = (POOLED + 31) / 32;

void set_error(const std::string& msg);
bool debug_switch(const char* name);

#define GNN_HIP(call)                                                                          \
    do {                                                                                       \
        hipError_t e_ = (call);                                                                \
        if (e_ != hipSuccess) {                                                                \
            gnn::set_error(std::string(#call) + " failed: " + hipGetErrorString(e_));          \
            return GNN_ERR_HIP;                                                                \
        }                                                                                      \
    } while (0)

struct DeviceWeights {
    float* conv1_k = nullptr;
    float* conv1_b = nullptr;
    float* conv_k[2] = {nullptr, nullptr};
    float* conv_b[2] = {nullptr, nullptr};
    float* weff_sorted[2] = {nullptr, nullptr};
    int32_t* pos_sorted[2] = {nullptr, nullptr};
    int32_t* slot[2] = {nullptr, nullptr};
    int32_t* bucket_ptr[2] = {nullptr, nullptr};
    float* conv1_pairs = nullptr;
    float* w_bias[2] = {nullptr, nullptr};
    float* w_qk[2] = {nullptr, nullptr};
    float* w_v[2] = {nullptr, nullptr};
    float* d1_k = nullptr;
    float* d1_b = nullptr;
    float* d2_k = nullptr;
    float* d2_b = nullptr;
    float* d3_k = nullptr;
    float* d3_b = nullptr;
    uint16_t* d1_frag = nullptr;
    uint16_t* d2_frag = nullptr;
    uint16_t* conv_frag[2] = {nullptr, nullptr};
    uint16_t* wv_frag[2] = {nullptr, nullptr};
    uint16_t* wqk_frag[2] = {nullptr, nullptr};
    uint16_t* wqk_frag_h[2] = {nullptr, nullptr};
    uint16_t* conv_frag_h[2] = {nullptr, nullptr};
    uint16_t* wv_frag_h[2] = {nullptr, nullptr};
    uint32_t* conv_c6[2] = {nullptr, nullptr};
    uint32_t* wv_c6[2] = {nullptr, nullptr};
    float* conv1_pairs6 = nullptr;
    float* weff6[2] = {nullptr, nullptr};
    int32_t* bucket_ptr6[2] = {nullptr, nullptr};
    DevBuf<float> c6_yp_const;
    DevBuf<float> c6_mp_const;
    uint16_t* tc_frag[2] = {nullptr, nullptr};
    float tc_inv_s[2] = {1.f, 1.f};
    int32_t* bucket_ptr96[2] = {nullptr, nullptr};
    DevBuf<float> tc_yp_const;
    DevBuf<float> tc_mp_const;
    DevBuf<float> tc_wva_tbl;
    DevBuf<float> tk_x2_tbl;
    DevBuf<float> tk_mpa_tbl;
    DevBuf<float> tk_x1t_tbl;
    DevBuf<float> tk_pt_tbl;
    DevBuf<float> tk_yp_const;
    DevBuf<float> tk_mp_const;
    DevBuf<float> x3_yp_const[2];
    DevBuf<float> x3_mp_const[2];
};

struct Workspace {
    int64_t chunk = 0;
    DevBuf<uint16_t> tokens;
    DevBuf<float> x[3];
    int64_t x_chunk = 0;
    DevBuf<float> mp;
    DevBuf<float> m;
    DevBuf<float> yp;
    DevBuf<float> logits;
    DevBuf<float> alpha;
    DevBuf<float> feat;
};

constexpr int MIN_TAIL = 2500;
constexpr int MAX_N = 4000;
constexpr int64_t PIECE = 64ll << 20;

struct RegionWorkspace {
    int tile = 256;
    PinnedBuf<int64_t> h_off;
    hipEvent_t tables_read = nullptr;
    DevBuf<int64_t> d_off;
    DevBuf<int64_t> d_transfer, d_entry;
    DevBuf<uint8_t> d_comp, d_exit;
    DevBuf<uint8_t> d_psi;
    DevBuf<float> d_track;
    DevBuf<uint8_t> d_state, d_flag;
    DevBuf<int32_t> d_blk_count;
    DevBuf<int64_t> d_blk_off;
    DevBuf<int64_t> d_r_contig, d_r_lo, d_r_hi, d_r_evidence, d_r_qsum;
    DevBuf<uint8_t> d_r_state;
    ~RegionWorkspace() {
        if (tables_read) (void)hipEventDestroy(tables_read);
    }
};

struct ContigWorkspace {
    hipStream_t copy_stream = nullptr;
    std::vector<hipEvent_t> piece_done;
    std::vector<int64_t> starts, ids;
    std::vector<int32_t> lens, window_n, counts;
    DevBuf<uint8_t> seq;
    DevBuf<int64_t> d_starts, d_ids;
    DevBuf<int32_t> d_lens, d_window_n, d_counts;
    DevBuf<float> d_scores;
    DevBuf<uint8_t> d_bases;
    DevBuf<float> d_out;
    DevBuf<float> d_emb, d_emb_sum;
    DevBuf<int32_t> d_emb_kept;
    std::vector<int64_t> win_off, bin_off;
    DevBuf<int64_t> d_win_off, d_bin_off;
    DevBuf<float> d_track;
    DevBuf<int32_t> d_cover;
    DevBuf<float> d_scores_rev, d_scores_mix, d_slab_scores, d_out_strand;
    DevBuf<float> d_emb_sum_rev;
    DevBuf<int32_t> d_emb_kept_rev;
    std::vector<int64_t> blk_off;
    DevBuf<int64_t> d_blk_off;
    DevBuf<float> d_occ;
    DevBuf<float> d_attr;
    RegionWorkspace regions;

    size_t span_cap() const {
        return std::min({d_starts.capacity(), d_ids.capacity(), d_lens.capacity(), d_window_n.capacity(), d_counts.capacity(),
                         d_scores.capacity() / GNN_CLASSES});
    }
    size_t strand_cap() const { return std::min(d_scores_rev.capacity(), d_scores_mix.capacity()) / GNN_CLASSES; }
    size_t off_cap() const { return std::min(d_win_off.capacity(), d_bin_off.capacity()); }
    size_t bin_cap() const { return std::min(d_track.capacity() / GNN_CLASSES, d_cover.capacity()); }
};

template <typename F>
static inline void for_each_window(int64_t len, int64_t stride, int single_window, F&& f) {
    for (int64_t k = 0; k * stride < len; ++k) {
        const int64_t l = std::min<int64_t>(W, len - k * stride);
        if (l < MIN_TAIL && k > 0) break;
        f(k, l);
        if (l < MIN_TAIL || (single_window && k == 0) || k * stride + W >= len) break;
    }
}

struct WindowWalk {
    int64_t* win_off = nullptr;
    int64_t* bin_off = nullptr;
    int64_t windows = 0, bins = 0;
};
template <typename F>
static int walk_windows(const int64_t* offsets, int64_t n_contigs, int64_t stride, int single_window, WindowWalk& out, F&& f) {
    for (int64_t c = 0; c < n_contigs; ++c)
        if (offsets[c + 1] < offsets[c]) {
            set_error("contig offsets are not non-decreasing");
            return GNN_ERR_ARG;
        }
    out.windows = out.bins = 0;
    if (out.win_off) out.win_off[0] = 0;
    if (out.bin_off) out.bin_off[0] = 0;
    for (int64_t c = 0; c < n_contigs; ++c) {
        const int64_t len = offsets[c + 1] - offsets[c];
        for_each_window(len, stride, single_window, [&](int64_t k, int64_t l) {
            f(c, k, l);
            ++out.windows;
        });
        out.bins += (len + stride - 1) / stride;
        if (out.win_off) out.win_off[c + 1] = out.windows;
        if (out.bin_off) out.bin_off[c + 1] = out.bins;
    }
    return GNN_OK;
}

__host__ __device__ inline bool window_kept(int32_t window_n, int32_t n_count) {
    return window_n == 0 || n_count <= MAX_N;
}

template <typename Tp>
static int reserve_roomy(DevBuf<Tp>& b, size_t need) {
    return b.reserve(need, need / 4 + 64);
}

template <typename... Bufs>
static void reset_all(Bufs&... bufs) {
    (bufs.reset(), ...);
}

template <typename... P, typename... A>
static int launch_1d(void (*kernel)(P...), int64_t cells, hipStream_t stream, A&&... args) {
    hipLaunchKernelGGL(kernel, dim3((unsigned)((cells + 255) / 256)), dim3(256), 0, stream, static_cast<P>(args)...);
    GNN_HIP(hipGetLastError());
    return GNN_OK;
}

struct AttribOut {
    int bin;
    float* contrib;
    float* bias;
    float* logits;
};
static inline int attrib_bins(int bin) { return (POOLED + bin - 1) / bin; }

struct ProfileSlot {
    double total_ms = 0.0;
    int64_t launches = 0;
    std::vector<std::pair<hipEvent_t, hipEvent_t>> pending;
};

}

struct gnn_ctx {
    int device = 0;
    hipStream_t stream = nullptr;
    bool has_weights = false;
    gnn::DeviceWeights w;
    gnn::Workspace ws;
    gnn::Workspace ws_alt;
    hipStream_t stream2 = nullptr;
    hipEvent_t ev_front[2] = {nullptr, nullptr}, ev_back[2] = {nullptr, nullptr};
    bool back_pending[2] = {false, false};
    int buf_cur = 0;
    int64_t chunk_fused = 16384;
    int64_t alt_failed_chunk = 0;
    bool chunk_explicit = false;
    int64_t chunk_f32 = 64;
    bool profile = false;
    gnn::ProfileSlot prof[GNN_K_COUNT];
    std::vector<hipEvent_t> event_pool;
    std::vector<gnn::DevBuf<unsigned char>> owned;
    int cu_count = 0;
    int last_split = 1;
    bool time_split = true;
    bool c6_pad_skip = true;
    gnn::DevBuf<unsigned long long> phase_cycles;
    gnn::ContigWorkspace* contig_ws = nullptr;
    gnn::DevBuf<uint8_t> stage_bases;
    gnn::DevBuf<float> stage_emb;
    gnn::DevBuf<float> emb_scores;
    gnn::DevBuf<float> stage_attr;
    gnn::DevBuf<float> attr_g;
    gnn::DevBuf<float> stage_scores;
    gnn::PinnedBuf<float> stage_scores_host;
    gnn::PinnedBuf<uint8_t> pin[2];
    hipEvent_t pin_ev[2] = {nullptr, nullptr};
    bool pin_busy[2] = {false, false};
    gnn::DevBuf<uint8_t> align_buf;
    void* comm = nullptr;
    int comm_ranks = 1, comm_rank = 0;
    gnn::DevBuf<unsigned char> comm_scratch;
};

namespace gnn {

struct ProfScope {
    gnn_ctx* ctx;
    int id;
    hipEvent_t a = nullptr, b = nullptr;
    ProfScope(gnn_ctx* c, int kid) : ctx(c), id(kid) {
        if (!ctx->profile) return;
        auto take = [&]() {
            hipEvent_t e = nullptr;
            if (!ctx->event_pool.empty()) {
                e = ctx->event_pool.back();
                ctx->event_pool.pop_back();
            } else if (hipEventCreate(&e) != hipSuccess) {
                e = nullptr;
            }
            return e;
        };
        a = take();
        b = take();
        if (a) (void)hipEventRecord(a, ctx->stream);
    }
    ~ProfScope() {
        if (!ctx->profile || !a || !b) return;
        (void)hipEventRecord(b, ctx->stream);
        ctx->prof[id].pending.emplace_back(a, b);
    }
};

template <typename Tp>
int upload(gnn_ctx* ctx, const Tp* host, size_t count, Tp** dev) {
    DevBuf<unsigned char> b;
    if (int rc = b.upload(reinterpret_cast<const unsigned char*>(host), count * sizeof(Tp))) return rc;
    *dev = reinterpret_cast<Tp*>(b.get());
    ctx->owned.emplace_back(std::move(b));
    return GNN_OK;
}
template <typename Tp>
int upload(gnn_ctx* ctx, const std::vector<Tp>& v, Tp** dev) {
    return upload(ctx, v.data(), v.size(), dev);
}

template <typename Run>
int all_n_consts(gnn_ctx* ctx, DevBuf<float>& yp, DevBuf<float>& mp, Run&& run) {
    DevBuf<uint8_t> bn;
    int rc = bn.reserve(W);
    if (!rc) rc = yp.reserve((size_t)2 * POOLED * C);
    if (!rc) rc = mp.reserve((size_t)2 * NPAIR);
    if (rc) return rc;
    hipError_t e = hipMemsetAsync(bn, 'N', W, ctx->stream);
    if (e == hipSuccess) {
        run(bn.get(), yp.get(), mp.get());
        e = hipGetLastError();
    }
    if (e == hipSuccess) e = hipStreamSynchronize(ctx->stream);
    if (e == hipSuccess) return GNN_OK;
    yp.reset();
    mp.reset();
    set_error(std::string("the all-N window's launch failed: ") + hipGetErrorString(e));
    return GNN_ERR_HIP;
}

int launch_tokenize(gnn_ctx* ctx, const uint8_t* bases, int64_t n, uint16_t* tokens);
int launch_onehot(gnn_ctx* ctx, const uint8_t* bases, int64_t n, int dtype, void* out);
int launch_synth(gnn_ctx* ctx, uint64_t seed, int64_t first, int64_t n, uint8_t* bases);
int launch_span_count(gnn_ctx* ctx, const uint8_t* seq, const int64_t* starts, const int32_t* lens, int64_t n,
                      int byte, int32_t* counts);
int launch_materialize(gnn_ctx* ctx, const uint8_t* seq, const int64_t* starts, const int32_t* lens, int64_t n,
                       uint8_t* bases);
int launch_revcomp(gnn_ctx* ctx, const uint8_t* seq, const int64_t* starts, const int32_t* lens, int64_t n,
                   uint8_t* bases);
int launch_occlude(gnn_ctx* ctx, const uint8_t* seq, const int64_t* starts, const int32_t* lens, const int64_t* blk_off,
                   int64_t n_windows, int64_t pair0, int block, const int32_t* lo, const int32_t* hi, int64_t n_rows, uint8_t* bases);
int launch_masked_segment_mean(gnn_ctx* ctx, const float* scores, const int64_t* ids, const int32_t* window_n, const int32_t* counts,
                               int64_t n, int64_t n_seg, float* out);
int launch_front_f32(gnn_ctx* ctx, const uint8_t* bases, int64_t n);
int launch_backend(gnn_ctx* ctx, int64_t n, int precision, float* scores_dev, void* emb_dev = nullptr, int emb_dtype = GNN_EMB_F32,
                   bool dense = true);
int check_attrib_args(int precision, int bin, const char* fn);
int launch_attrib_head(gnn_ctx* ctx, int64_t n, float* scores_dev, const AttribOut& at, int64_t row0);
int launch_attrib_contrib(gnn_ctx* ctx, int64_t n, const AttribOut& at, int64_t row0);
int classify_chunks(gnn_ctx* ctx, const uint8_t* bases_dev, int64_t n, int precision, float* scores_dev, bool defer_last = false,
                    void* emb_dev = nullptr, int emb_dtype = GNN_EMB_F32, const AttribOut* attr = nullptr);
size_t emb_elem_bytes(int emb_dtype);
int flush_backend(gnn_ctx* ctx);
int finish_pending(gnn_ctx* ctx);
int check_ctx(gnn_ctx* ctx, bool flush = true);
int check_embed_precision(int precision, const char* fn);
void free_stage(gnn_ctx* ctx);

struct ContigIn {
    gnn_ctx* ctx;
    const uint8_t* seq;
    int seq_on_host;
    int64_t seq_bytes;
    const int64_t* offsets;
    int64_t n_contigs;
    int single_window, precision;
    int64_t stride;
};

class SeqFeed {
  public:
    int begin(const ContigIn& in, ContigWorkspace& w);
    int upto(int64_t end);
    const uint8_t* dev() const { return dev_; }

  private:
    gnn_ctx* ctx_ = nullptr;
    ContigWorkspace* w_ = nullptr;
    const uint8_t* host_ = nullptr;
    const uint8_t* dev_ = nullptr;
    int64_t bytes_ = 0, n_pieces_ = 0, uploaded_ = 0;
};

int contig_begin(const ContigIn& in, const char* fn, bool outputs_ok, ContigWorkspace** w);
int plan_windows(const ContigIn& in, ContigWorkspace& w, bool csr, int block);
int upload_span_table(gnn_ctx* ctx, ContigWorkspace& w);
int slab_pass(const ContigIn& in, ContigWorkspace& w, SeqFeed& feed, int64_t a, int64_t m, bool fwd, bool rev, float* scores,
              float* emb, const AttribOut* attr = nullptr);
int64_t kept_windows(const ContigWorkspace& w, uint8_t* mask_or_null, int64_t* ids_or_null);
void free_contig_ws(gnn_ctx* ctx);

int launch_front_c6(gnn_ctx* ctx, const uint8_t* bases, int64_t n);
int launch_front_x3(gnn_ctx* ctx, const uint8_t* bases, int64_t n, int precision);
int launch_front_tc(gnn_ctx* ctx, const uint8_t* bases, int64_t n);
int launch_front_tk(gnn_ctx* ctx, const uint8_t* bases, int64_t n);
int build_kmer_tables(gnn_ctx* ctx, size_t reserve);
void free_kmer_tables(gnn_ctx* ctx);
size_t kmer_tables_bytes();
int build_wva_rows_table(gnn_ctx* ctx, const float* w_kc, float* tbl);
int pack_fused_tc_weights(gnn_ctx* ctx, const gnn_weights* w);
int pack_fused_x3_consts(gnn_ctx* ctx);

int pack_fused_weights(gnn_ctx* ctx, const gnn_weights* w);
std::vector<uint16_t> pack_frags(const float* wmat, int K, int N, bool f16 = false);
int pack_fused_c6_weights(gnn_ctx* ctx, const gnn_weights* w);
int c6_rows_per_step();
int c6_pack_matrix(const float* wmat, int K, int N, std::vector<uint32_t>& out);
void build_conv1_pair_tables(const float* conv1_kernel, std::vector<float>& pt);

}
```

genomad_amd/csrc/gnn_fused_tk.hip:

```cpp
#include <chrono>
#include <vector>
#include <cstdio>

#include "gnn_tc_dev.h"

#define __noinline__ __noinline__

namespace gnn {
namespace tk {

using namespace tc;

constexpr int YP_NT = 2;
constexpr uint32_t X2_ROWS = (1u << 28) + 1u;
constexpr uint32_t X2_NN = 1u << 28;
constexpr uint32_t K9_ROWS = (1u << 18) + 1u;
constexpr uint32_t K9_NN = 1u << 18;
constexpr int QUADS = W / 4;
constexpr int QUAD_N = QUADS + 4;
constexpr int QUAD_OFF = VRING_OFF + VRING * VSLOT;
constexpr int BIASK_OFF = QUAD_OFF + ((QUAD_N * 2 + 15) / 16) * 16;
constexpr int DIRTY_OFF = BIASK_OFF + C * 4;
constexpr int DIRTY_MAX = BUF_ROWS;
constexpr int PIDX_N = 32;
constexpr int PIDX_OFF = DIRTY_OFF + ((4 + DIRTY_MAX + 15) / 16) * 16;
constexpr int BKT_OFF = PIDX_OFF + 4 * PIDX_N * 4;
constexpr int LASTK_OFF = BKT_OFF + 2 * (STEPST + 1) * 4;
constexpr int SMEMK = LASTK_OFF + 16;
constexpr int X2_PER_WAVE = (BUF_ROWS + 3) / 4;
static_assert(SMEMK <= 160 * 1024, "LDS budget");

struct ArgsK {
    const uint8_t* bases;
    const unsigned char* tcw3;
    float inv_s3;
    const float* conv_b3;
    const unsigned char* wv_w;
    const float* weff_b;
    const int32_t* pos_sorted[2];
    const int32_t* bucket_ptr[2];
    const unsigned char* wva_tbl;
    const float* x2_tbl;
    const float* mpa_tbl;
    const float* x1t_tbl;
    const float* pt_tbl;
    const float* conv2_b;
    const float* weff_a;
    float* mp;
    float* yp;
    const float* yp_c;
    const float* mp_c;
    unsigned long long* cycles;
    int split;
};

__device__ __forceinline__ uint32_t quad_of(uint32_t w4) {
    uint32_t code = 0, dirty = 0;
#pragma unroll
    for (int i = 0; i < 4; ++i) {
        const uint32_t d = wva_digit((w4 >> (8 * i)) & 255u);
        code = (code << 2) | (d & 3u);
        dirty = (dirty << 1) | (d >> 2);
    }
    return (dirty << 8) | code;
}
template <int LEN>
__device__ __forceinline__ void kmer_q(const uint16_t* __restrict__ quads, int b, uint32_t& code, uint32_t& dirty) {
    constexpr int NQ = (LEN + 6) / 4;
    const int q0 = b >> 2, r = b & 3;
    unsigned long long c = 0;
    uint32_t d = 0;
#pragma unroll
    for (int i = 0; i < NQ; ++i) {
        const uint32_t v = quads[q0 + i];
        c = (c << 8) | (v & 255u);
        d = (d << 4) | (v >> 8);
    }
    const int drop = 4 * NQ - r - LEN;
    code = (uint32_t)(c >> (2 * drop)) & ((1u << (2 * LEN)) - 1u);
    dirty = (d >> drop) & ((1u << LEN) - 1u);
}
template <int LEN>
__device__ __forceinline__ bool all_n_tokens(uint32_t dirty) {
    const uint32_t clean = ~dirty & ((1u << LEN) - 1u);
    return ((clean & (clean >> 1) & (clean >> 2) & (clean >> 3)) & ((1u << (LEN - 3)) - 1u)) == 0u;
}
constexpr uint32_t ROW_DIRTY = 0x80000000u;
__device__ __forceinline__ uint32_t x2_index(const uint16_t* __restrict__ quads, int t) {
    if (t < 10) return ROW_DIRTY | X2_NN;
    uint32_t code, dirty;
    kmer_q<14>(quads, min(t, T - 1) - 10, code, dirty);
    if (dirty == 0u) return code;
    return all_n_tokens<14>(dirty) ? X2_NN : (ROW_DIRTY | X2_NN);
}
__device__ __forceinline__ uint32_t wva_index_q(const uint16_t* __restrict__ quads, int t) {
    uint32_t code, dirty;
    kmer_q<9>(quads, max(t - 5, 0), code, dirty);
    if (t >= 5 && dirty == 0u) return code;
    const int np = min(t, 5) + 4;
    uint32_t i5 = 0;
#pragma unroll
    for (int k = 0; k < 9; ++k) {
        const uint32_t d = ((dirty >> (8 - k)) & 1u) ? 4u : (code >> (2 * (8 - k))) & 3u;
        i5 = k < np ? i5 * 5u + d : i5;
    }
    return t < 5 ? WvaTable::s5_off(t) + i5 : WvaTable::D5_OFF + i5;
}
__device__ __forceinline__ uint32_t wva_step_index_q(const uint16_t* __restrict__ quads, int t0, int hw, int lane) {
    return wva_index_q(quads, wva_row(t0, hw, lane));
}

__device__ __noinline__ float pair_a_slow(const uint16_t* __restrict__ quads, const float* __restrict__ x1t, const float* __restrict__ weff_a, int e, int u) {
    const float4* x = reinterpret_cast<const float4*>(x1t + (size_t)wva_index_q(quads, u) * C);
    const float4* w = reinterpret_cast<const float4*>(weff_a + (size_t)e * C);
    float s0 = 0.f, s1 = 0.f, s2 = 0.f, s3 = 0.f;
#pragma unroll 8
    for (int i = 0; i < C / 4; ++i) {
        const float4 xv = x[i], wv = w[i];
        s0 = fmaf(xv.x, wv.x, s0);
        s1 = fmaf(xv.y, wv.y, s1);
        s2 = fmaf(xv.z, wv.z, s2);
        s3 = fmaf(xv.w, wv.w, s3);
    }
    return (s0 + s2) + (s1 + s3);
}
__device__ __forceinline__ uint32_t dirty_count(const unsigned char* __restrict__ smem) {
    return *reinterpret_cast<const volatile uint32_t*>(smem + DIRTY_OFF);
}
template <int NT, bool PIDX>
__device__ __noinline__ void dirty_rows_fill(unsigned char* __restrict__ smem, unsigned char* __restrict__ buf, int tb, const uint16_t* __restrict__ quads,
                                             const float* __restrict__ pt, const float* __restrict__ conv2_b, int tid) {
    const int n = (int)dirty_count(smem);
    const unsigned char* drows = smem + DIRTY_OFF + 4;
    const int c = tid & (C - 1);
    const float b2 = conv2_b[c];
    constexpr int G = NT / 128, U = 4;
    for (int i0 = tid >> 7; i0 < n; i0 += G * U) {
        float v[U][KS];
        int rr[U], tt[U];
#pragma unroll
        for (int u = 0; u < U; ++u) {
            const int i = min(i0 + u * G, n - 1);
            rr[u] = drows[i];
            tt[u] = min(tb + rr[u], T - 1);
#pragma unroll
            for (int j = 0; j < KS; ++j) {
                const int p = tt[u] - CARRY + j;
                const uint32_t row = PIDX ? reinterpret_cast<const uint32_t*>(smem + PIDX_OFF)[(rr[u] / X2_PER_WAVE) * PIDX_N + rr[u] % X2_PER_WAVE + j]
                                          : wva_index_q(quads, max(p, 0));
                v[u][j] = pt[((size_t)j * WvaTable::ROWS + row) * C + c];
                v[u][j] = p >= 0 ? v[u][j] : 0.f;
            }
        }
#pragma unroll
        for (int u = 0; u < U; ++u) {
            if (i0 + u * G < n) {
                float s = b2;
#pragma unroll
                for (int j = 0; j < KS; ++j) s += v[u][j];
                s = vmax_raw(s, s * LRELU);
                *reinterpret_cast<float*>(buf + rr[u] * ROWX + c * 4) = tt[u] >= 0 ? s : 0.f;
            }
        }
    }
}

constexpr int DIRTY_FAST_MAX = 16;
__device__ __forceinline__ void dirty_rows_fill_prologue(unsigned char* __restrict__ smem, unsigned char* __restrict__ buf, int tb,
                                                         const uint16_t* __restrict__ quads, const float* __restrict__ pt,
                                                         const float* __restrict__ conv2_b, int tid) {
    const int n = (int)dirty_count(smem);
    if (n > DIRTY_FAST_MAX) {
        dirty_rows_fill<512, false>(smem, buf, tb, quads, pt, conv2_b, tid);
        return;
    }
    const unsigned char* drows = smem + DIRTY_OFF + 4;
    uint32_t* idxs = reinterpret_cast<uint32_t*>(smem + VRING_OFF);
    if (tid < n * KS) {
        const int i = tid / KS, j = tid - i * KS;
        const int t = min(tb + drows[i], T - 1), p = t - CARRY + j;
        idxs[tid] = (t >= 0 && p >= 0) ? wva_index_q(quads, p) : ~0u;
    }
    __syncthreads();
    const int c = tid & (C - 1), q = tid >> 7;
    float v[DIRTY_FAST_MAX / 4][KS];
#pragma unroll
    for (int k = 0; k < DIRTY_FAST_MAX / 4; ++k)
#pragma unroll
        for (int j = 0; j < KS; ++j) {
            const int i = q + 4 * k;
            const uint32_t idx = i < n ? idxs[i * KS + j] : ~0u;
            v[k][j] = idx != ~0u ? pt[((size_t)j * WvaTable::ROWS + idx) * C + c] : 0.f;
        }
    const float b2 = conv2_b[c];
#pragma unroll
    for (int k = 0; k < DIRTY_FAST_MAX / 4; ++k) {
        const int i = q + 4 * k;
        if (i < n) {
            const int r = drows[i];
            float s = b2;
#pragma unroll
            for (int j = 0; j < KS; ++j) s += v[k][j];
            s = vmax_raw(s, s * LRELU);
            *reinterpret_cast<float*>(buf + r * ROWX + c * 4) = (tb + r) >= 0 ? s : 0.f;
        }
    }
}

struct X2Rows {
    u32x4 v[X2_PER_WAVE / 2];
};
__device__ __forceinline__ uint32_t x2_rows_index(unsigned char* __restrict__ smem, const uint16_t* __restrict__ quads, int tb, int w, int lane, bool list) {
    const int r = min(X2_PER_WAVE * w + min(lane, X2_PER_WAVE - 1), BUF_ROWS - 1);
    const uint32_t idx = x2_index(quads, tb + r);
    const bool mine = list && (idx & ROW_DIRTY) && lane < X2_PER_WAVE && X2_PER_WAVE * w + lane < BUF_ROWS;
    if (mine) {
        uint32_t* dl = reinterpret_cast<uint32_t*>(smem + DIRTY_OFF);
        const uint32_t slot = atomicAdd(dl, 1u);
        smem[DIRTY_OFF + 4 + slot] = (unsigned char)r;
    }
    if (__builtin_amdgcn_ballot_w64(mine) && lane < PIDX_N - 1)
        reinterpret_cast<uint32_t*>(smem + PIDX_OFF)[w * PIDX_N + lane] = wva_index_q(quads, min(max(tb + X2_PER_WAVE * w - CARRY + lane, 0), T - 1));
    return idx;
}
template <int I0, int I1>
__device__ __forceinline__ void x2_rows_issue(X2Rows& x, const float* __restrict__ tbl, uint32_t my_row, int lane) {
    static_assert(I0 % 2 == 0 && I1 % 2 == 0, "two rows per request");
#pragma unroll
    for (int i = I0 / 2; i < I1 / 2; ++i) {
        const uint32_t r0 = __builtin_amdgcn_readlane(my_row, 2 * i), r1 = __builtin_amdgcn_readlane(my_row, 2 * i + 1);
        const uint32_t row = (lane < 32 ? r0 : r1) & ~ROW_DIRTY;
        const unsigned char* p = reinterpret_cast<const unsigned char*>(tbl) + (size_t)row * (C * 4) + (lane & 31) * 16;
        x.v[i] = __builtin_nontemporal_load(reinterpret_cast<const u32x4*>(p));
    }
}
__device__ __forceinline__ void x2_rows_store(const X2Rows& x, unsigned char* __restrict__ buf, uint32_t my_row, int w, int lane) {
#pragma unroll
    for (int i = 0; i < X2_PER_WAVE / 2; ++i) {
        const int r = X2_PER_WAVE * w + 2 * i + (lane >> 5);
        const uint32_t r0 = __builtin_amdgcn_readlane(my_row, 2 * i), r1 = __builtin_amdgcn_readlane(my_row, 2 * i + 1);
        const bool dirty = ((lane < 32 ? r0 : r1) & ROW_DIRTY) != 0u;
        if (r < BUF_ROWS && !dirty) *reinterpret_cast<u32x4*>(buf + r * ROWX + (lane & 31) * 16) = x.v[i];
    }
}

template <bool PROF>
__global__ __launch_bounds__(512, 2) void fused_front_tk_kernel(ArgsK a) {
    __shared__ __attribute__((aligned(16))) unsigned char smem[SMEMK];
    const unsigned long long t_entry = PROF ? __builtin_readcyclecounter() : 0ull;
    uint16_t* quads = reinterpret_cast<uint16_t*>(smem + QUAD_OFF);
    float* bias_s = reinterpret_cast<float*>(smem + BIASK_OFF);
    int* s_last = reinterpret_cast<int*>(smem + LASTK_OFF);
    const int tid = threadIdx.x;
    const int lane = tid & 63;
    const int wave = __builtin_amdgcn_readfirstlane(tid >> 6);
    const bool helper = wave >= 4;
    const int hw = wave & 3;
    const int ht = tid & 255;
    const int64_t wi = blockIdx.x / a.split;
    const int part = blockIdx.x % a.split;
    const uint8_t* bases = a.bases + wi * W;
    float* mp_w[2] = {a.mp + (wi * 2 + 0) * NPAIR, a.mp + (wi * 2 + 1) * NPAIR};
    const int woff = hw * WNBLK_B;

    for (int q = tid; q < QUAD_N; q += 512)
        quads[q] = q < QUADS ? (uint16_t)quad_of(reinterpret_cast<const uint32_t*>(bases)[q]) : (uint16_t)0;
    if (tid < C) bias_s[tid] = a.conv_b3[tid];
    int* bkt = reinterpret_cast<int*>(smem + BKT_OFF);
    if (tid >= 128 && tid < 128 + 2 * (STEPST + 1)) bkt[tid - 128] = a.bucket_ptr[(tid - 128) / (STEPST + 1)][(tid - 128) % (STEPST + 1)];
    if (tid == 0) {
        *s_last = -1;
        *reinterpret_cast<uint32_t*>(smem + DIRTY_OFF) = 0u;
    }
    __syncthreads();
    if (a.yp_c) {
        int last = -1;
        for (int q = tid; q < QUADS; q += 512) {
            const uint32_t clean = ~((uint32_t)quads[q] >> 8) & 15u;
            if (clean) last = max(last, 4 * q + 3 - (int)__builtin_ctz(clean));
        }
        if (last >= 0) atomicMax(s_last, last);
    }
    __syncthreads();
    const int nsteps = a.yp_c ? max(1, min(STEPST, (*s_last + 1 + 15 + FTT - 1) / FTT)) : STEPST;
    const int per = (nsteps + a.split - 1) / a.split;
    const int s_lo = min(part * per, nsteps), s_hi = min(s_lo + per, nsteps);
    unsigned jitter_state = 0x9E3779B9u * (unsigned)(wave + 1) + (unsigned)blockIdx.x * 7919u;
    (void)jitter_state;
    unsigned long long cyc[16] = {0, 0, 0, 0, 0, 0, 0, 0, 0, 0, 0, 0, 0, 0, 0, 0};
    unsigned long long tick_ = 0;
    if constexpr (PROF) tick_ = t_entry;

    if (s_hi > s_lo) {
        WvaRows w0;
        {
            const int tb = s_lo * FTT - CARRY;
            unsigned char* buf = smem + (s_lo & 1) * BUF_BYTES;
            constexpr int PR = 14;
            const int r = min(PR * wave + min(lane, PR - 1), BUF_ROWS - 1);
            const uint32_t idx = x2_index(quads, tb + r);
            if ((idx & ROW_DIRTY) && lane < PR && PR * wave + lane < BUF_ROWS) {
                const uint32_t slot = atomicAdd(reinterpret_cast<uint32_t*>(smem + DIRTY_OFF), 1u);
                smem[DIRTY_OFF + 4 + slot] = (unsigned char)r;
            }
            u32x4 v[PR / 2];
#pragma unroll
            for (int i = 0; i < PR / 2; ++i) {
                const uint32_t r0 = __builtin_amdgcn_readlane(idx, 2 * i), r1 = __builtin_amdgcn_readlane(idx, 2 * i + 1);
                const uint32_t row = (lane < 32 ? r0 : r1) & ~ROW_DIRTY;
                const unsigned char* p = reinterpret_cast<const unsigned char*>(a.x2_tbl) + (size_t)row * (C * 4) + (lane & 31) * 16;
                v[i] = __builtin_nontemporal_load(reinterpret_cast<const u32x4*>(p));
            }
            if (!helper)
                wva_issue(w0, make_wrsrc(a.wva_tbl, (int)(WvaTable::ROWS * WvaTable::ROW_BYTES)), wva_step_index_q(quads, s_lo * FTT, hw, lane), lane);
#pragma unroll
            for (int i = 0; i < PR / 2; ++i) {
                const int rr = PR * wave + 2 * i + (lane >> 5);
                const uint32_t r0 = __builtin_amdgcn_readlane(idx, 2 * i), r1 = __builtin_amdgcn_readlane(idx, 2 * i + 1);
                const bool dirty = ((lane < 32 ? r0 : r1) & ROW_DIRTY) != 0u;
                if (rr < BUF_ROWS && !dirty) *reinterpret_cast<u32x4*>(buf + rr * ROWX + (lane & 31) * 16) = v[i];
            }
            __syncthreads();
            GNN_TICK(6)
            if (dirty_count(smem)) {
                dirty_rows_fill_prologue(smem, buf, tb, quads, a.pt_tbl, a.conv2_b, tid);
                __syncthreads();
                if (tid == 0) *reinterpret_cast<uint32_t*>(smem + DIRTY_OFF) = 0u;
            }
            __syncthreads();
            GNN_TICK(7)
        }

        if (!helper) {
            __builtin_amdgcn_s_setprio(2);
            const wrsrc_t cw = make_wrsrc(a.tcw3 + woff, 64 * WUNIT_B - woff);
            const wrsrc_t vw = make_wrsrc(a.wv_w + woff, 8 * WUNIT_B - woff);
            const wrsrc_t tblr = make_wrsrc(a.wva_tbl, (int)(WvaTable::ROWS * WvaTable::ROW_BYTES));
            const wrsrc_t yp_w = make_wrsrc(reinterpret_cast<const unsigned char*>(a.yp + wi * 2 * (size_t)POOLED * C), 2 * POOLED * C * 4);
            WU ring[RINGT];
            prime_tc(ring, cw, 0, lane);
            wva_pool_store<YP_NT>(w0, yp_w, s_lo * FTT, hw, lane);
            {
                const HLane h0 = hlane(smem, (s_lo & 1) * BUF_BYTES, hw, lane);
                Raw16 rm;
                load_rows(rm, h0, 1);
                transform_store(rm, h0, 1);
            }
            uint32_t wva_next = wva_step_index_q(quads, (s_lo + 1) * FTT, hw, lane);
            asm volatile("s_waitcnt lgkmcnt(0)" ::: "memory");
            GNN_TICK(6)
#pragma unroll 1
            for (int step = s_lo; step < s_hi; ++step) {
                const int t0 = step * FTT;
                const int xoff = (step & 1) * BUF_BYTES, yoff = BUF_BYTES - xoff;
                f32x16 acc[NXI];
#pragma unroll
                for (int xi = 0; xi < NXI; ++xi)
#pragma unroll
                    for (int r = 0; r < 16; ++r) acc[xi][r] = 0.f;
                GNN_TICK(5)
                conv_tc(smem, cw, 0, ring, acc, lane, jitter_state);
                GNN_TICK(0)
                prime_wv(ring, vw, lane);
                epilogue_x3(smem + xoff, acc, a.inv_s3, bias_s, hw, lane);
                GNN_TICK(1)
                TC_BARRIER_W();
                GNN_TICK(2)
                {
                    WvaRows wr;
                    wva_issue(wr, tblr, wva_next, lane);
                    f32x16 ac[NMB];
#pragma unroll
                    for (int mb = 0; mb < NMB; ++mb)
#pragma unroll
                        for (int r = 0; r < 16; ++r) ac[mb][r] = 0.f;
                    wv_tile(smem, xoff + CARRY * ROWX, ring, ac, lane);
                    prime_tc(ring, cw, 0, lane);
                    wv_pool_store<YP_NT>(ac, yp_w, POOLED * C * 4, t0, hw, lane);
                    GNN_TICK(3)
                    if (step + 1 < s_hi) {
                        const HLane hn = hlane(smem, yoff, hw, lane);
                        Raw16 rm;
                        load_rows(rm, hn, 1);
                        transform_store(rm, hn, 1);
                        wva_pool_store<YP_NT>(wr, yp_w, t0 + FTT, hw, lane);
                    }
                    wva_next = wva_step_index_q(quads, t0 + 2 * FTT, hw, lane);
                    asm volatile("s_waitcnt lgkmcnt(0)" ::: "memory");
                    GNN_TICK(4)
                }
            }
        } else {
            __builtin_amdgcn_s_setprio(3);
            if constexpr (PROF) tick_ = __builtin_readcyclecounter();
            Raw16 ra, rb;
            PairPass p0, p1, p2;
            p0.u = p1.u = p2.u = 0;
            struct StepA {
                int ea, ea_end, ua;
            };
            StepA cur, nxt;
            cur.ea = cur.ea_end = cur.ua = 0;
            float va = 0.f;
            bool va_slow = false, nxt_slow = false;
            const float* nxt_ptr = a.mpa_tbl;
            auto fetch = [&](int st, bool valid) {
                nxt.ea = valid ? bkt[st] + ht : 0;
                nxt.ea_end = valid ? bkt[st + 1] : 0;
                nxt.ua = nxt.ea < nxt.ea_end ? a.pos_sorted[0][nxt.ea] : 0;
            };
            auto locate = [&]() {
                nxt_slow = false;
                uint32_t code = 0, dirty = 0;
                if (nxt.ea < nxt.ea_end) {
                    kmer_q<9>(quads, max(nxt.ua - 5, 0), code, dirty);
                    const bool nn = all_n_tokens<9>(dirty);
                    nxt_slow = nxt.ua < 5 || (dirty != 0u && !nn);
                }
                nxt_ptr = a.mpa_tbl + ((size_t)max(nxt.ea, 0) * K9_ROWS + (dirty == 0u ? code : K9_NN));
            };
            fetch(s_lo, true);
            {
                const HLane h0 = hlane(smem, (s_lo & 1) * BUF_BYTES, hw, lane);
                load_rows(ra, h0, 0);
                transform_store(ra, h0, 0);
                load_rows(ra, h0, 2);
            }
            __builtin_amdgcn_s_waitcnt(0x0F70);

#pragma unroll 1
            for (int step = s_lo; step < s_hi; ++step) {
                const int t0 = step * FTT;
                const int xoff = (step & 1) * BUF_BYTES, yoff = BUF_BYTES - xoff;
                const HLane hx = hlane(smem, xoff, hw, lane), hy = hlane(smem, yoff, hw, lane);
                const bool more = step + 1 < s_hi;
                const bool prev = step > s_lo;
                const PairJob jb = {smem + xoff, a.weff_b, a.pos_sorted[1], mp_w[1], t0, bkt[STEPST + 1 + step], bkt[STEPST + 1 + step + 1]};
                const PairJob jp = {smem + yoff, a.weff_b, a.pos_sorted[1], mp_w[1], t0 - FTT, prev ? bkt[STEPST + 1 + step - 1] : 0, prev ? bkt[STEPST + 1 + step] : 0};
                locate();
                cur = nxt;
                va_slow = nxt_slow;
                const float* va_ptr = nxt_ptr;
                X2Rows xr;
                const uint32_t my_row = x2_rows_index(smem, quads, t0 + FTT - CARRY, hw, lane, more);
                GNN_REGION_END();
                x2_rows_issue<0, X2_PER_WAVE>(xr, a.x2_tbl, my_row, lane);
                GNN_REGION_END();
                va = cur.ea < cur.ea_end ? __builtin_nontemporal_load(va_ptr) : 0.f;
                GNN_TICK(15)
                pass_compute(p0, jp, 0, hw, lane);
                pass_compute(p1, jp, 1, hw, lane);
                pass_compute(p2, jp, 2, hw, lane);
                pass_rest(p0, jp, 3, hw, lane);
                TC_HPRIO_HIGH();
                HBAR_W(14, 8);
                load_rows(rb, hx, 3);
                transform_store(ra, hx, 2);
                HBAR_W(9, 8);
                load_rows(ra, hx, 4);
                transform_store(rb, hx, 0);
                HBAR_W(10, 8);
                load_rows(rb, hx, 5);
                transform_store(ra, hx, 1);
                HBAR_W(10, 8);
                load_rows(ra, hx, 6);
                transform_store(rb, hx, 2);
                HBAR_W(10, 8);
                load_rows(rb, hx, 7);
                transform_store(ra, hx, 0);
                HBAR_W(10, 8);
                transform_store(rb, hx, 1);
                HBAR_W(11, 8);
                x2_rows_store(xr, smem + yoff, my_row, hw, lane);
                if (more && dirty_count(smem)) {
                    dirty_rows_fill<256, true>(smem, smem + yoff, t0 + FTT - CARRY, quads, a.pt_tbl, a.conv2_b, ht);
                }
                HBAR_W(12, 8);
                TC_HPRIO_LOW();
                if (ht == 0) *reinterpret_cast<volatile uint32_t*>(smem + DIRTY_OFF) = 0u;
                if (more) {
                    load_rows(ra, hy, 0);
                    transform_store(ra, hy, 0);
                    load_rows(ra, hy, 2);
                }
                if (cur.ea < cur.ea_end) {
                    if (va_slow) va = pair_a_slow(quads, a.x1t_tbl, a.weff_a, cur.ea, cur.ua);
                    mp_w[0][cur.ea] = va;
                    for (int e = cur.ea + 256; e < cur.ea_end; e += 256) {
                        const int u = a.pos_sorted[0][e];
                        uint32_t code, dirty;
                        kmer_q<9>(quads, max(u - 5, 0), code, dirty);
                        const bool nn = all_n_tokens<9>(dirty);
                        mp_w[0][e] = (u < 5 || (dirty != 0u && !nn)) ? pair_a_slow(quads, a.x1t_tbl, a.weff_a, e, u)
                                                                      : a.mpa_tbl[(size_t)e * K9_ROWS + (dirty == 0u ? code : K9_NN)];
                    }
                }
                pass_issue(p0, jb, 0, hw, lane);
                pass_issue(p1, jb, 1, hw, lane);
                pass_issue(p2, jb, 2, hw, lane);
                fetch(step + 1, more);
                asm volatile("s_waitcnt lgkmcnt(0)" ::: "memory");
                HBAR(13, 8);
                __builtin_amdgcn_s_waitcnt(0x0F70);
            }
            {
                const int ls = s_hi - 1;
                const PairJob jl = {smem + (ls & 1) * BUF_BYTES, a.weff_b, a.pos_sorted[1], mp_w[1], ls * FTT, bkt[STEPST + 1 + ls], bkt[STEPST + 1 + ls + 1]};
                pass_compute(p0, jl, 0, hw, lane);
                pass_compute(p1, jl, 1, hw, lane);
                pass_compute(p2, jl, 2, hw, lane);
                pass_rest(p0, jl, 3, hw, lane);
            }
        }
    }
    __syncthreads();
    if (nsteps < STEPST && part == a.split - 1) {
        const int q0 = nsteps * (FTT / GNN_POOL);
        const int nrow4 = (POOLED - q0) * (C / 4);
        for (int i = tid; i < 2 * nrow4; i += 512) {
            const int h = i >= nrow4, j = i - h * nrow4;
            const size_t off = (size_t)h * POOLED * C + (size_t)q0 * C + (size_t)j * 4;
            *reinterpret_cast<float4*>(a.yp + wi * 2 * (size_t)POOLED * C + off) = *reinterpret_cast<const float4*>(a.yp_c + off);
        }
#pragma unroll
        for (int h = 0; h < 2; ++h)
            for (int e = a.bucket_ptr[h][nsteps] + tid; e < NPAIR; e += 512) mp_w[h][e] = a.mp_c[h * NPAIR + e];
    }
    if constexpr (PROF) {
        if (tid == 0)
            for (int i = 0; i < 8; ++i) atomicAdd(a.cycles + i, cyc[i]);
        if (tid == 256)
            for (int i = 8; i < 16; ++i) atomicAdd(a.cycles + i, cyc[i]);
    }
}

__global__ __launch_bounds__(128) void x1tab_kernel(const float* __restrict__ pairs6, float* __restrict__ x1tab) {
    const uint32_t n = blockIdx.x;
    const int c = threadIdx.x;
    int tk[6];
#pragma unroll
    for (int i = 0; i < 6; ++i) tk[i] = n == K9_NN ? 0 : 1 + (int)((n >> (2 * (5 - i))) & 255u);
    const int perm = ((c >> 2) & 3) * 32 + (c >> 4) * 4 + (c & 3);
    float v = 0.f;
#pragma unroll
    for (int j = 0; j < 3; ++j) v += pairs6[((size_t)j * PAIR_ROWS + pair_row(tk[2 * j], tk[2 * j + 1])) * C + perm];
    x1tab[(size_t)n * C + c] = vmax_raw(v, v * LRELU);
}
constexpr int PJ_ROWS = 64;
__global__ __launch_bounds__(128) void pj_kernel(const float* __restrict__ x1tab, const float* __restrict__ conv2_k, double* __restrict__ P) {
    __shared__ float xs[C];
    const int c = threadIdx.x, j = blockIdx.y;
    float wcol[C];
#pragma unroll
    for (int k = 0; k < C; ++k) wcol[k] = conv2_k[((size_t)j * C + k) * C + c];
    const uint32_t r_end = min((uint32_t)(blockIdx.x + 1) * PJ_ROWS, K9_ROWS);
    for (uint32_t n = blockIdx.x * PJ_ROWS; n < r_end; ++n) {
        xs[c] = x1tab[(size_t)n * C + c];
        __syncthreads();
        double acc = 0.0;
#pragma unroll
        for (int k = 0; k < C; ++k) acc = __builtin_fma((double)xs[k], (double)wcol[k], acc);
        P[((size_t)j * K9_ROWS + n) * C + c] = acc;
        __syncthreads();
    }
}
constexpr uint32_t X2TAB_ROWS = 128;
__global__ __launch_bounds__(256) void x2tab_kernel(const double* __restrict__ P, const float* __restrict__ conv2_b, float* __restrict__ tbl) {
    const int sub = threadIdx.x & 31;
    double b[4];
#pragma unroll
    for (int i = 0; i < 4; ++i) b[i] = (double)conv2_b[sub * 4 + i];
    for (uint32_t k = 0; k < X2TAB_ROWS / 8; ++k) {
        const uint32_t row = blockIdx.x * X2TAB_ROWS + k * 8u + (threadIdx.x >> 5);
        if (row >= X2_ROWS) return;
        double s[4] = {b[0], b[1], b[2], b[3]};
#pragma unroll
        for (int j = 0; j < KS; ++j) {
            const uint32_t n9 = row == X2_NN ? K9_NN : (row >> (2 * (5 - j))) & 0x3FFFFu;
            const double4 p = *reinterpret_cast<const double4*>(P + ((size_t)j * K9_ROWS + n9) * C + sub * 4);
            s[0] += p.x; s[1] += p.y; s[2] += p.z; s[3] += p.w;
        }
        float4 o;
        float v;
        v = (float)s[0]; o.x = vmax_raw(v, v * LRELU);
        v = (float)s[1]; o.y = vmax_raw(v, v * LRELU);
        v = (float)s[2]; o.z = vmax_raw(v, v * LRELU);
        v = (float)s[3]; o.w = vmax_raw(v, v * LRELU);
        *reinterpret_cast<float4*>(tbl + (size_t)row * C + sub * 4) = o;
    }
}
constexpr int MPA_T = 64, MPA_LD = C + 1;
__global__ __launch_bounds__(256) void mpa_kernel(const float* __restrict__ x1tab, const float* __restrict__ weff_a, float* __restrict__ tbl) {
    __shared__ float xa[MPA_T * MPA_LD], wb[MPA_T * MPA_LD];
    const uint32_t n0 = blockIdx.x * MPA_T;
    const int e0 = blockIdx.y * MPA_T;
    for (int i = threadIdx.x; i < MPA_T * C; i += 256) {
        const int r = i >> 7, k = i & (C - 1);
        xa[r * MPA_LD + k] = n0 + r < K9_ROWS ? x1tab[(size_t)(n0 + r) * C + k] : 0.f;
        wb[r * MPA_LD + k] = e0 + r < NPAIR ? weff_a[(size_t)(e0 + r) * C + k] : 0.f;
    }
    __syncthreads();
    const int tn = threadIdx.x & 15, te = threadIdx.x >> 4;
    double acc[4][4];
#pragma unroll
    for (int i = 0; i < 4; ++i)
#pragma unroll
        for (int j = 0; j < 4; ++j) acc[i][j] = 0.0;
    for (int k = 0; k < C; ++k) {
        double x[4], w[4];
#pragma unroll
        for (int i = 0; i < 4; ++i) {
            x[i] = (double)xa[(tn + 16 * i) * MPA_LD + k];
            w[i] = (double)wb[(te * 4 + i) * MPA_LD + k];
        }
#pragma unroll
        for (int i = 0; i < 4; ++i)
#pragma unroll
            for (int j = 0; j < 4; ++j) acc[i][j] = __builtin_fma(x[i], w[j], acc[i][j]);
    }
#pragma unroll
    for (int j = 0; j < 4; ++j) {
        const int e = e0 + te * 4 + j;
        if (e >= NPAIR) continue;
#pragma unroll
        for (int i = 0; i < 4; ++i) {
            const uint32_t n = n0 + tn + 16 * i;
            if (n < K9_ROWS) tbl[(size_t)e * K9_ROWS + n] = (float)acc[i][j];
        }
    }
}

static void fill_args(const gnn_ctx* ctx, ArgsK& a, const uint8_t* bases) {
    const DeviceWeights& d = ctx->w;
    a.bases = bases;
    a.tcw3 = reinterpret_cast<const unsigned char*>(d.tc_frag[1]);
    a.inv_s3 = d.tc_inv_s[1];
    a.conv_b3 = d.conv_b[1];
    a.wv_w = reinterpret_cast<const unsigned char*>(d.wv_frag_h[1]);
    a.weff_b = d.weff6[1];
    for (int i = 0; i < 2; ++i) {
        a.pos_sorted[i] = d.pos_sorted[i];
        a.bucket_ptr[i] = d.bucket_ptr96[i];
    }
    a.wva_tbl = reinterpret_cast<const unsigned char*>(d.tc_wva_tbl.get());
    a.x2_tbl = d.tk_x2_tbl;
    a.mpa_tbl = d.tk_mpa_tbl;
    a.x1t_tbl = d.tk_x1t_tbl;
    a.pt_tbl = d.tk_pt_tbl;
    a.conv2_b = d.conv_b[0];
    a.weff_a = d.weff_sorted[0];
    a.cycles = nullptr;
    a.split = 1;
}

static void launch(const ArgsK& a, bool prof, unsigned nwin, hipStream_t stream) {
    const unsigned n = nwin * (unsigned)a.split;
    if (prof) hipLaunchKernelGGL((fused_front_tk_kernel<true>), dim3(n), dim3(512), 0, stream, a);
    else hipLaunchKernelGGL((fused_front_tk_kernel<false>), dim3(n), dim3(512), 0, stream, a);
}

}

size_t kmer_tables_bytes() {
    return (size_t)tk::X2_ROWS * C * 4 + (size_t)NPAIR * tk::K9_ROWS * 4 + (size_t)(KS + 1) * tc::WvaTable::ROWS * C * 4;
}

void free_kmer_tables(gnn_ctx* ctx) {
    DeviceWeights& d = ctx->w;
    for (DevBuf<float>* b : {&d.tk_x2_tbl, &d.tk_mpa_tbl, &d.tk_pt_tbl, &d.tk_x1t_tbl, &d.tk_yp_const, &d.tk_mp_const}) b->reset();
}

int build_kmer_tables(gnn_ctx* ctx, size_t reserve) {
    using namespace tk;
    DeviceWeights& d = ctx->w;
    if (d.tk_x2_tbl && d.tk_mpa_tbl && d.tk_pt_tbl && d.tk_x1t_tbl && d.tk_yp_const) return GNN_OK;
    free_kmer_tables(ctx);
    const size_t x2_b = (size_t)X2_ROWS * C * 4, mpa_b = (size_t)NPAIR * K9_ROWS * 4;
    const size_t x1_b = (size_t)K9_ROWS * C * 4, p_b = (size_t)KS * K9_ROWS * C * 8;
    size_t free_b = 0, total_b = 0;
    GNN_HIP(hipMemGetInfo(&free_b, &total_b));
    const size_t pt_b = (size_t)KS * WvaTable::ROWS * C * 4, x1t_b = (size_t)WvaTable::ROWS * C * 4;
    const size_t need = x2_b + mpa_b + pt_b + x1t_b + x1_b + p_b + reserve;
    if (free_b < need) {
        set_error("k-mer tables: " + std::to_string(need >> 30) + " GiB needed (" + std::to_string((x2_b + mpa_b) >> 30) + " GiB of tables, the rest workspace reserve), " +
                  std::to_string(free_b >> 30) + " GiB free on the device: GNN_PREC_F16X3TC keeps serving");
        return GNN_ERR_NOMEM;
    }
    DevBuf<float> x2, mpa, x1, pt, x1t, eye;
    DevBuf<double> P;
    auto fail = [&](hipError_t e, const char* what) {
        (void)hipGetLastError();
        set_error(std::string("k-mer tables: ") + what + " failed: " + hipGetErrorString(e));
        return e == hipErrorOutOfMemory ? GNN_ERR_NOMEM : GNN_ERR_HIP;
    };
    hipError_t e;
    static const bool timing = debug_switch("GNN_TABLE_TIMING");
    auto t_last = std::chrono::steady_clock::now();
    auto lap = [&](const char* what) {
        if (!timing) return;
        (void)hipStreamSynchronize(ctx->stream);
        const auto now = std::chrono::steady_clock::now();
        std::fprintf(stderr, "genomad_nn k-mer tables: %-40s %.3f s\n", what, std::chrono::duration<double>(now - t_last).count());
        t_last = now;
    };
    int rc;
    if ((rc = x2.reserve(x2_b / 4, 0, "k-mer tables: hipMalloc of the 14-mer table"))) return rc;
    lap("hipMalloc 137 GB");
    if ((rc = mpa.reserve(mpa_b / 4, 0, "k-mer tables: hipMalloc of head A's pair-product table"))) return rc;
    if ((rc = x1.reserve(x1_b / 4, 0, "k-mer tables: hipMalloc of the 9-mer x1 table"))) return rc;
    if ((rc = pt.reserve(pt_b / 4, 0, "k-mer tables: hipMalloc of conv2's tap tables"))) return rc;
    if ((rc = x1t.reserve(x1t_b / 4, 0, "k-mer tables: hipMalloc of the x1 table"))) return rc;
    if ((rc = eye.reserve((size_t)C * C, 0, "k-mer tables: hipMalloc of the identity"))) return rc;
    if ((rc = P.reserve(p_b / 8, 0, "k-mer tables: hipMalloc of the f64 tap tables"))) return rc;
    {
        std::vector<float> id((size_t)C * C, 0.f);
        for (int k = 0; k < C; ++k) id[(size_t)k * C + k] = 1.f;
        if ((e = hipMemcpy(eye, id.data(), id.size() * 4, hipMemcpyHostToDevice)) != hipSuccess) return fail(e, "upload of the identity");
        if (build_wva_rows_table(ctx, eye, x1t)) return fail(hipGetLastError(), "launch of the x1 table build");
    }
    lap("hipMalloc of the other four");
    for (int j = 0; j < KS; ++j)
        if (build_wva_rows_table(ctx, d.conv_k[0] + (size_t)j * C * C, pt + (size_t)j * WvaTable::ROWS * C)) return fail(hipGetLastError(), "launch of a tap-table build");
    lap("tap tables over WvaTable's rows (6 x 2.7 M)");
    hipStream_t st = ctx->stream;
    hipLaunchKernelGGL(x1tab_kernel, dim3(K9_ROWS), dim3(128), 0, st, d.conv1_pairs6, x1.get());
    if ((e = hipGetLastError()) != hipSuccess) return fail(e, "launch of x1tab_kernel");
    lap("x1 per 9-mer");
    hipLaunchKernelGGL(pj_kernel, dim3((K9_ROWS + PJ_ROWS - 1) / PJ_ROWS, KS), dim3(128), 0, st, x1.get(), d.conv_k[0], P.get());
    if ((e = hipGetLastError()) != hipSuccess) return fail(e, "launch of pj_kernel");
    lap("f64 tap tables per 9-mer");
    hipLaunchKernelGGL(x2tab_kernel, dim3((X2_ROWS + X2TAB_ROWS - 1) / X2TAB_ROWS), dim3(256), 0, st, P.get(), d.conv_b[0], x2.get());
    if ((e = hipGetLastError()) != hipSuccess) return fail(e, "launch of x2tab_kernel");
    lap("x2 per 14-mer (137 GB)");
    hipLaunchKernelGGL(mpa_kernel, dim3((K9_ROWS + MPA_T - 1) / MPA_T, (NPAIR + MPA_T - 1) / MPA_T), dim3(256), 0, st, x1.get(),
                       d.weff_sorted[0], mpa.get());
    if ((e = hipGetLastError()) != hipSuccess) return fail(e, "launch of mpa_kernel");
    if ((e = hipStreamSynchronize(st)) != hipSuccess) return fail(e, "building the tables");
    lap("head A's pair products (8.8 GB)");
    x1.reset();
    P.reset();
    eye.reset();
    d.tk_x2_tbl = std::move(x2);
    d.tk_mpa_tbl = std::move(mpa);
    d.tk_pt_tbl = std::move(pt);
    d.tk_x1t_tbl = std::move(x1t);
    rc = all_n_consts(ctx, d.tk_yp_const, d.tk_mp_const, [&](const uint8_t* bn, float* yp, float* mp) {
        ArgsK a;
        fill_args(ctx, a, bn);
        a.mp = mp;
        a.yp = yp;
        a.yp_c = nullptr;
        a.mp_c = nullptr;
        launch(a, false, 1, st);
    });
    if (rc) {
        free_kmer_tables(ctx);
        set_error(std::string("k-mer tables: ") + gnn_last_error());
    }
    return rc;
}

int launch_front_tk(gnn_ctx* ctx, const uint8_t* bases, int64_t n) {
    using namespace tk;
    if (!ctx->w.tk_x2_tbl || !ctx->w.tk_mpa_tbl) {
        set_error("f16x3tk: the k-mer tables have not been built (gnn_build_kmer_tables)");
        return GNN_ERR_STATE;
    }
    if (reinterpret_cast<uintptr_t>(bases) & 3u) {
        set_error("f16x3tk: the window buffer must be 4-byte aligned");
        return GNN_ERR_ARG;
    }
    ArgsK a;
    fill_args(ctx, a, bases);
    a.mp = ctx->ws.mp;
    a.yp = ctx->ws.yp;
    a.yp_c = ctx->c6_pad_skip ? ctx->w.tk_yp_const.get() : nullptr;
    a.mp_c = ctx->c6_pad_skip ? ctx->w.tk_mp_const.get() : nullptr;
    a.cycles = ctx->phase_cycles;
    if (ctx->time_split && n > 0 && ctx->cu_count > 0) a.split = (int)std::max<int64_t>(1, std::min<int64_t>(4, ctx->cu_count / n));
    ctx->last_split = a.split;
    launch(a, ctx->phase_cycles != nullptr, (unsigned)n, ctx->stream);
    GNN_HIP(hipGetLastError());
    return GNN_OK;
}

}
```

include/genomad_nn.h:

```cpp
#ifndef GENOMAD_NN_H
#define GENOMAD_NN_H

#include <stddef.h>
#include <stdint.h>

#ifdef __cplusplus
extern "C" {
#endif

#define GNN_WINDOW 6000
#define GNN_TOKENS 5997
#define GNN_DEPTH 257
#define GNN_CH 128
#define GNN_KSIZE 6
#define GNN_PATCHES 2100
#define GNN_PATCH_SIZE 4
#define GNN_POOL 8
#define GNN_POOLED 749
#define GNN_FEAT 256
#define GNN_HIDDEN 512
#define GNN_CLASSES 3
#define GNN_EMBED_DIM 512

typedef enum gnn_status {
    GNN_OK = 0,
    GNN_ERR_ARG = -1,
    GNN_ERR_HIP = -2,
    GNN_ERR_STATE = -3,
    GNN_ERR_WEIGHTS = -4,
    GNN_ERR_NOMEM = -5
} gnn_status;

typedef enum gnn_precision {
    GNN_PREC_F32 = 0,
    GNN_PREC_BF16X3 = 1,
    GNN_PREC_BF16 = 2,
    GNN_PREC_F16C8 = 3,
    GNN_PREC_F16C6 = 5,
    GNN_PREC_F16X3TC = 6,
    GNN_PREC_F16X3TK = 7,
    GNN_PREC_F16X3 = 4
} gnn_precision;

int gnn_has_experimental(void);

typedef enum gnn_onehot_dtype { GNN_OH_U8 = 0, GNN_OH_BF16 = 1, GNN_OH_F32 = 2 } gnn_onehot_dtype;

typedef enum gnn_emb_dtype { GNN_EMB_F32 = 0, GNN_EMB_BF16 = 1 } gnn_emb_dtype;

typedef struct gnn_igloo_weights {
    const int32_t* patches;
    const float* w_mult;
    const float* w_summer;
    const float* w_bias;
    const float* w_qk;
    const float* w_v;
} gnn_igloo_weights;

typedef struct gnn_dense_bn {
    const float* kernel;
    const float* bias;
    const float* gamma;
    const float* beta;
    const float* mean;
    const float* var;
} gnn_dense_bn;

typedef struct gnn_weights {
    const float* conv1_kernel;
    const float* conv1_bias;
    const float* conv2_kernel;
    const float* conv2_bias;
    const float* conv3_kernel;
    const float* conv3_bias;
    gnn_igloo_weights igloo_a;
    gnn_igloo_weights igloo_b;
    gnn_dense_bn enc;
    gnn_dense_bn head;
    const float* out_kernel;
    const float* out_bias;
} gnn_weights;

typedef struct gnn_taps {
    float* x1;
    float* x2;
    float* x3;
    float* m_a;
    float* m_b;
    float* yp_a;
    float* yp_b;
    float* alpha_a;
    float* alpha_b;
    float* feat;
} gnn_taps;

typedef struct gnn_ctx gnn_ctx;

const char* gnn_last_error(void);
int gnn_version(void);
int gnn_device_count(int* count);
int gnn_create(int device, gnn_ctx** out);
int gnn_destroy(gnn_ctx* ctx);
int gnn_sync(gnn_ctx* ctx);
int gnn_device_info(gnn_ctx* ctx, char* name, size_t name_len, int* cus, int64_t* hbm_bytes);
int gnn_device_pci_bus_id(gnn_ctx* ctx, char* out, size_t out_len);
int gnn_device_mem_info(gnn_ctx* ctx, int64_t* free_bytes, int64_t* total_bytes);

int gnn_load_weights(gnn_ctx* ctx, const gnn_weights* w);

int gnn_build_kmer_tables(gnn_ctx* ctx, int64_t reserve_bytes);
int gnn_has_kmer_tables(gnn_ctx* ctx);
int gnn_drop_kmer_tables(gnn_ctx* ctx);
int64_t gnn_kmer_tables_bytes(void);
int gnn_debug_kmer_table_row(gnn_ctx* ctx, int which, uint64_t row, float* out_host);

int gnn_dev_alloc(gnn_ctx* ctx, size_t bytes, void** dev_ptr);
int gnn_dev_free(gnn_ctx* ctx, void* dev_ptr);
int gnn_memcpy_h2d(gnn_ctx* ctx, void* dst_dev, const void* src_host, size_t bytes);
int gnn_memcpy_d2h(gnn_ctx* ctx, void* dst_host, const void* src_dev, size_t bytes);

int gnn_tokenize(gnn_ctx* ctx, const uint8_t* bases_host, int64_t n_windows, uint16_t* tokens_host);
int gnn_tokenize_dev(gnn_ctx* ctx, const uint8_t* bases_dev, int64_t n_windows, uint16_t* tokens_dev);

int gnn_onehot_dev(gnn_ctx* ctx, const uint8_t* bases_dev, int64_t n_windows, int onehot_dtype,
                   void* onehot_dev);

int gnn_classify(gnn_ctx* ctx, const uint8_t* bases_host, int64_t n_windows, int precision,
                 float* scores_host);
int gnn_classify_dev_async(gnn_ctx* ctx, const uint8_t* bases_dev, int64_t n_windows, int precision, float* scores_dev);
int gnn_classify_flush(gnn_ctx* ctx);

int gnn_classify_dev(gnn_ctx* ctx, const uint8_t* bases_dev, int64_t n_windows, int precision,
                     float* scores_dev);

int gnn_embed(gnn_ctx* ctx, const uint8_t* bases_host, int64_t n_windows, int precision, int emb_dtype, void* emb_host,
              float* scores_host_or_null);
int gnn_embed_dev(gnn_ctx* ctx, const uint8_t* bases_dev, int64_t n_windows, int precision, int emb_dtype, void* emb_dev,
                  float* scores_dev_or_null);

int gnn_segment_mean(gnn_ctx* ctx, const float* scores_host, const int64_t* ids_host, int64_t n,
                     int64_t n_segments, float* out_host);

int gnn_span_byte_count(gnn_ctx* ctx, const uint8_t* seq_dev, const int64_t* starts_host,
                        const int32_t* lens_host, int64_t n_spans, int byte, int32_t* counts_host);
int gnn_classify_spans(gnn_ctx* ctx, const uint8_t* seq_dev, const int64_t* starts_host,
                       const int32_t* lens_host, int64_t n_spans, int precision, float* scores_host);

int gnn_classify_contigs(gnn_ctx* ctx, const uint8_t* seq, int seq_on_host, int64_t seq_bytes,
                         const int64_t* offsets_host, int64_t n_contigs, int single_window, int precision,
                         float* contig_scores_host, int64_t* window_ids_host, int64_t ids_capacity,
                         int64_t* n_windows_out);
int gnn_classify_contigs_embed(gnn_ctx* ctx, const uint8_t* seq, int seq_on_host, int64_t seq_bytes,
                               const int64_t* offsets_host, int64_t n_contigs, int single_window, int precision,
                               float* contig_scores_host, int64_t* window_ids_host, int64_t ids_capacity,
                               int64_t* n_windows_out, float* contig_emb_host);

int gnn_scan_plan(const int64_t* offsets_host, int64_t n_contigs, int stride, int single_window, int64_t* n_windows_out,
                  int64_t* n_bins_out, int64_t* win_offsets_or_null, int64_t* bin_offsets_or_null, int64_t* starts_or_null,
                  int32_t* lens_or_null);
int gnn_scan_contigs(gnn_ctx* ctx, const uint8_t* seq, int seq_on_host, int64_t seq_bytes, const int64_t* offsets_host,
                     int64_t n_contigs, int stride, int single_window, int precision, float* window_scores_host,
                     uint8_t* window_kept_host_or_null, int64_t windows_capacity, float* track_host_or_null,
                     int32_t* cover_host_or_null, int64_t bins_capacity, float* contig_scores_host_or_null);

typedef enum gnn_strand { GNN_STRAND_FORWARD = 0, GNN_STRAND_REVERSE = 1, GNN_STRAND_BOTH = 2 } gnn_strand;
int gnn_revcomp_spans_dev(gnn_ctx* ctx, const uint8_t* seq_dev, const int64_t* starts_host, const int32_t* lens_host, int64_t n_spans,
                          uint8_t* bases_dev_out);
int gnn_classify_contigs_strand(gnn_ctx* ctx, const uint8_t* seq, int seq_on_host, int64_t seq_bytes, const int64_t* offsets_host,
                                int64_t n_contigs, int single_window, int precision, float* contig_scores_host,
                                int64_t* window_ids_host, int64_t ids_capacity, int64_t* n_windows_out, float* contig_emb_host_or_null,
                                int strand, float* contig_scores_fwd_host_or_null, float* contig_scores_rev_host_or_null);
int gnn_scan_contigs_strand(gnn_ctx* ctx, const uint8_t* seq, int seq_on_host, int64_t seq_bytes, const int64_t* offsets_host,
                            int64_t n_contigs, int stride, int single_window, int precision, float* window_scores_host,
                            uint8_t* window_kept_host_or_null, int64_t windows_capacity, float* track_host_or_null,
                            int32_t* cover_host_or_null, int64_t bins_capacity, float* contig_scores_host_or_null, int strand,
                            float* window_scores_fwd_host_or_null, float* window_scores_rev_host_or_null);

int gnn_occlusion_plan(const int64_t* offsets_host, int64_t n_contigs, int block, int single_window,
                       int64_t* n_windows_out, int64_t* n_pairs_out, int64_t* win_offsets_or_null,
                       int64_t* starts_or_null, int32_t* lens_or_null, int64_t* blk_offsets_or_null);
int gnn_occlude_spans_dev(gnn_ctx* ctx, const uint8_t* seq_dev, const int64_t* starts_host, const int32_t* lens_host,
                          const int32_t* lo_host, const int32_t* hi_host, int64_t n_spans, uint8_t* bases_dev_out);
int gnn_occlude_contigs(gnn_ctx* ctx, const uint8_t* seq, int seq_on_host, int64_t seq_bytes, const int64_t* offsets_host,
                        int64_t n_contigs, int block, int single_window, int precision, float* window_scores_host,
                        uint8_t* window_kept_host_or_null, int64_t windows_capacity, float* delta_host,
                        int64_t pairs_capacity, float* contig_scores_host_or_null);

int gnn_attribute(gnn_ctx* ctx, const uint8_t* bases_host, int64_t n_windows, int precision, int bin, float* contrib_host,
                  float* bias_host_or_null, float* logits_host_or_null, float* scores_host_or_null);
int gnn_attribute_dev(gnn_ctx* ctx, const uint8_t* bases_dev, int64_t n_windows, int precision, int bin, float* contrib_dev,
                      float* bias_dev_or_null, float* logits_dev_or_null, float* scores_dev_or_null);
int gnn_attribute_contigs(gnn_ctx* ctx, const uint8_t* seq, int seq_on_host, int64_t seq_bytes, const int64_t* offsets_host,
                          int64_t n_contigs, int bin, int single_window, int precision, float* contrib_host, int64_t windows_capacity,
                          float* bias_host_or_null, float* logits_host_or_null, float* window_scores_host_or_null,
                          uint8_t* window_kept_host_or_null, float* contig_scores_host_or_null);

int gnn_call_regions(gnn_ctx* ctx, const float* track_host, const int64_t* bin_offsets_host, int64_t n_contigs, double penalty,
                     uint8_t* state_host_or_null, int64_t* region_contig, int64_t* region_lo, int64_t* region_hi,
                     uint8_t* region_state, int64_t* region_evidence, int64_t* region_qsum, int64_t regions_capacity,
                     int64_t* n_regions_out);
int gnn_region_states_dev(gnn_ctx* ctx, const float* track_dev, const int64_t* bin_offsets_host, int64_t n_contigs, double penalty,
                          uint8_t* state_dev);
int gnn_debug_set_region_tile(gnn_ctx* ctx, int bins);

int gnn_fasta_scan(const uint8_t* text, int64_t n, int64_t* n_headers, int64_t* header_bytes, int* has_cr);
int gnn_fasta_pack(const uint8_t* text, int64_t n, int strip_n, uint8_t* seq_out, int64_t* offsets,
                   uint8_t* headers_out, int64_t* header_offsets, int64_t capacity, int64_t* n_records);
int gnn_fasta_accession_digests(const uint8_t* text, int64_t n, uint64_t* digests, int64_t capacity, int64_t* n_records,
                                int* needs_python);

int gnn_branch_attention(gnn_ctx* ctx, const double* w_host, const double* b1_host, const double* b2_host,
                         int64_t n, double temperature, double* out_host);
int gnn_score_calibration(gnn_ctx* ctx, const double* scores_host, const double* composition3,
                          const double* kernel1, const double* bias1, const double* kernel2,
                          const double* bias2, const double* kernel3, const double* bias3, int64_t n,
                          double* out_host);

uint32_t gnn_crc32c(const void* data_host, size_t n_bytes);

int gnn_debug_forward(gnn_ctx* ctx, const uint8_t* bases_host, int64_t n_windows, int precision,
                      float* scores_host, const gnn_taps* taps);

#define GNN_COMM_ID_BYTES 128
int gnn_comm_unique_id(uint8_t* id128);
int gnn_comm_init(gnn_ctx* ctx, int n_ranks, int rank, const uint8_t* id128);
int gnn_comm_destroy(gnn_ctx* ctx);
int gnn_comm_info(gnn_ctx* ctx, int* n_ranks, int* rank);
int gnn_comm_gather_dev(gnn_ctx* ctx, const void* send_dev, void* recv_dev, size_t bytes_per_rank, int root);
int gnn_comm_gather(gnn_ctx* ctx, const void* send_host, void* recv_host, size_t bytes_per_rank, int root);
int gnn_comm_allgather(gnn_ctx* ctx, const void* send_host, void* recv_host, size_t bytes_per_rank);
int gnn_comm_allreduce_max(gnn_ctx* ctx, double* values_host, int n);
int gnn_comm_barrier(gnn_ctx* ctx);

int gnn_synth_windows_dev(gnn_ctx* ctx, uint64_t seed, int64_t first, int64_t n_windows,
                          uint8_t* bases_dev);

#define GNN_K_FUSED 0
#define GNN_K_BACKEND 1
#define GNN_K_ENCODER 2
#define GNN_K_F32_FRONT 3
#define GNN_K_ATTR_HEAD 4
#define GNN_K_ATTR_CONTRIB 5
#define GNN_K_REGIONS 6
#define GNN_K_COUNT 7
int gnn_profile_enable(gnn_ctx* ctx, int on);
int gnn_profile_reset(gnn_ctx* ctx);
int gnn_profile_get(gnn_ctx* ctx, int kernel_id, double* total_ms, int64_t* launches);

int gnn_phase_cycles(gnn_ctx* ctx, int on, unsigned long long* out16);

int gnn_mfma_probe(gnn_ctx* ctx, int ms_target, double* tflops_out);
int gnn_mfma_probe_kind(gnn_ctx* ctx, int kind, int ms_target, double* tflops_out);

int gnn_fused_rows_per_step(int precision);

int gnn_debug_set_pad_skip(gnn_ctx* ctx, int on);

int gnn_debug_set_time_split(gnn_ctx* ctx, int on);
int gnn_debug_last_split(gnn_ctx* ctx, int* workgroups_per_window);

int gnn_debug_pack_c6(const float* w, int k, int n, uint32_t* out, size_t out_words, size_t* need_words);

int gnn_set_chunk(gnn_ctx* ctx, int64_t windows_per_chunk);

#ifdef __cplusplus
}
#endif
#endif
```

Before: 313,500.

## Fuse head A attention pooling into the tk front kernel with look-ahead pair products

Measured after the change: 316,700 (median of 6 runs). 1.01x the previous value.

```diff
diff --git a/genomad_amd/_lib.py b/genomad_amd/_lib.py
--- a/genomad_amd/_lib.py
+++ b/genomad_amd/_lib.py
@@ -112,6 +112,9 @@
     "gnn_fused_rows_per_step": (_int, [_int]),
     "gnn_debug_set_pad_skip": (_int, [_vp, _int]),
     "gnn_debug_set_time_split": (_int, [_vp, _int]),
+    "gnn_debug_set_fuse_head_a": (_int, [_vp, _int]),
+    "gnn_debug_last_head_a_fused": (_int, [_vp, C.POINTER(_int)]),
+    "gnn_debug_workspace": (_int, [_vp, _int, _i64, _vp]),
     "gnn_debug_last_split": (_int, [_vp, C.POINTER(_int)]),
     "gnn_debug_pack_c6": (_int, [_f32p, _int, _int, C.POINTER(C.c_uint32), _sz, C.POINTER(_sz)]),
     "gnn_crc32c": (C.c_uint32, [_vp, _sz]),
diff --git a/genomad_amd/csrc/gnn_api.hip b/genomad_amd/csrc/gnn_api.hip
--- a/genomad_amd/csrc/gnn_api.hip
+++ b/genomad_amd/csrc/gnn_api.hip
@@ -187,7 +187,7 @@
 }
 
 int classify_chunks(gnn_ctx* ctx, const uint8_t* bases_dev, int64_t n, int precision, float* scores_dev, bool defer_last,
-                    void* emb_dev, int emb_dtype, const AttribOut* attr) {
+                    void* emb_dev, int emb_dtype, const AttribOut* attr, bool need_yp) {
     if (!ctx->has_weights) {
         set_error("gnn_load_weights has not been called");
         return GNN_ERR_STATE;
@@ -267,8 +267,11 @@
     struct StreamGuard {
         gnn_ctx* c;
         hipStream_t main;
-        ~StreamGuard() { c->stream = main; }
+        ~StreamGuard() { c->stream = main; c->head_a_ready = nullptr; }
     } guard{ctx, ctx->stream};
+    ctx->head_a_ready = nullptr;
+    const bool fuse_a = precision == GNN_PREC_F16X3TK && !attr && !need_yp && !overlap &&
+                        (ctx->fuse_head_a == 2 || (ctx->fuse_head_a == 1 && n > chunk));
     for (int64_t a = 0; a < n; a += chunk) {
         const int64_t m = std::min(chunk, n - a);
         const uint8_t* b = bases_dev + a * W;
@@ -286,6 +289,7 @@
             ctx->back_pending[buf] = false;
         }
         static const bool poison = debug_switch("GNN_DEBUG_POISON");
+        const bool look_ahead = fuse_a && !poison && b == bases_dev + a * W && a + chunk < n;
         if (poison) {
             const Workspace& ws = ctx->ws;
             const size_t mm = (size_t)std::min<int64_t>(m, ws.chunk);
@@ -305,7 +309,8 @@
             if ((rc = launch_front_f32(ctx, b, m))) return rc;
         } else {
             ProfScope ps(ctx, GNN_K_FUSED);
-            rc = precision == GNN_PREC_F16X3TK ? launch_front_tk(ctx, b, m)
+            rc = precision == GNN_PREC_F16X3TK ? launch_front_tk(ctx, b, m, !fuse_a, look_ahead ? bases_dev + (a + chunk) * W : nullptr,
+                                                                 look_ahead ? std::min(chunk, n - a - chunk) : 0)
                  : precision == GNN_PREC_F16X3TC ? launch_front_tc(ctx, b, m)
                  : precision == GNN_PREC_F16C6 ? launch_front_c6(ctx, b, m)
                                                : launch_front_x3(ctx, b, m, precision);
@@ -320,7 +325,8 @@
             ProfScope ps(ctx, GNN_K_BACKEND);
             void* emb = emb_dev ? static_cast<uint8_t*>(emb_dev) + (size_t)a * HID * emb_elem_bytes(emb_dtype) : nullptr;
             rc = launch_backend(ctx, m, (precision == GNN_PREC_F16X3TC || precision == GNN_PREC_F16X3TK) ? GNN_PREC_F16X3 : precision,
-                                scores_dev ? scores_dev + a * GNN_CLASSES : nullptr, emb, emb_dtype, !attr);
+                                scores_dev ? scores_dev + a * GNN_CLASSES : nullptr, emb, emb_dtype, !attr,
+                                precision == GNN_PREC_F16X3TK && ctx->head_a_fused);
         }
         if (attr && !rc) {
             ProfScope ps(ctx, GNN_K_ATTR_HEAD);
@@ -384,6 +390,37 @@
     if (rc) return rc;
     ctx->c6_pad_skip = on != 0;
     return GNN_OK;
+}
+
+int gnn_debug_set_fuse_head_a(gnn_ctx* ctx, int on) {
+    int rc = check_ctx(ctx);
+    if (rc) return rc;
+    ctx->fuse_head_a = on < 0 ? 0 : on > 2 ? 2 : on;
+    return GNN_OK;
+}
+
+int gnn_debug_last_head_a_fused(gnn_ctx* ctx, int* fused) {
+    if (!ctx || !fused) {
+        set_error("bad argument to gnn_debug_last_head_a_fused");
+        return GNN_ERR_ARG;
+    }
+    *fused = ctx->head_a_fused ? 1 : 0;
+    return GNN_OK;
+}
+
+int gnn_debug_workspace(gnn_ctx* ctx, int which, int64_t n_windows, float* out_host) {
+    int rc = check_ctx(ctx);
+    if (rc) return rc;
+    const Workspace& ws = ctx->ws;
+    const size_t per = which == 0 ? (size_t)2 * NPAIR : which == 1 ? (size_t)2 * POOLED : which == 2 ? (size_t)FEAT : 0;
+    if (!per || n_windows < 0 || n_windows > ws.chunk || (n_windows > 0 && !out_host)) {
+        set_error("bad argument to gnn_debug_workspace (which: 0 pair products, 1 attention weights, 2 features; n_windows within the last launch)");
+        return GNN_ERR_ARG;
+    }
+    if (n_windows == 0) return GNN_OK;
+    GNN_HIP(hipStreamSynchronize(ctx->stream));
+    const float* src = which == 0 ? ws.mp.get() : which == 1 ? ws.alpha.get() : ws.feat.get();
+    return gnn_memcpy_d2h(ctx, out_host, src, (size_t)n_windows * per * sizeof(float));
 }
 
 int gnn_debug_set_time_split(gnn_ctx* ctx, int on) {
@@ -475,6 +512,7 @@
     ctx->device = device;
     ctx->c6_pad_skip = !debug_switch("GNN_NO_PAD_SKIP");
     ctx->time_split = !debug_switch("GNN_NO_TIME_SPLIT");
+    ctx->fuse_head_a = debug_switch("GNN_NO_FUSE_A") ? 0 : 1;
     ctx->cu_count = prop.multiProcessorCount;
     hipError_t e = hipStreamCreateWithFlags(&ctx->stream, hipStreamNonBlocking);
     if (e != hipSuccess) {
@@ -964,7 +1002,8 @@
     for (int64_t a0 = 0; a0 < n && !rc; a0 += slab) {
         const int64_t m = std::min(slab, n - a0);
         rc = stage_upload(ctx, bases_host + a0 * W, (size_t)m * W);
-        if (!rc) rc = classify_chunks(ctx, ctx->stage_bases, m, precision, ctx->stage_scores);
+        if (!rc) rc = classify_chunks(ctx, ctx->stage_bases, m, precision, ctx->stage_scores, false, nullptr, GNN_EMB_F32, nullptr,
+                                      taps != nullptr);
         if (!rc) {
             GNN_HIP(hipMemcpyAsync(ctx->stage_scores_host, ctx->stage_scores, (size_t)m * GNN_CLASSES * sizeof(float),
                                    hipMemcpyDeviceToHost, ctx->stream));
diff --git a/genomad_amd/csrc/gnn_backend.hip b/genomad_amd/csrc/gnn_backend.hip
--- a/genomad_amd/csrc/gnn_backend.hip
+++ b/genomad_amd/csrc/gnn_backend.hip
@@ -7,9 +7,9 @@
 __global__ __launch_bounds__(256) void m_kernel(const float* __restrict__ mp, const float* __restrict__ w_bias0,
                                                 const float* __restrict__ w_bias1,
                                                 const int32_t* __restrict__ slot0,
-                                                const int32_t* __restrict__ slot1, float* __restrict__ m) {
+                                                const int32_t* __restrict__ slot1, float* __restrict__ m, int h0) {
     __shared__ float s[NPAIR];
-    const int wi = blockIdx.x, h = blockIdx.y;
+    const int wi = blockIdx.x, h = blockIdx.y + h0;
     const float* w_bias = h ? w_bias1 : w_bias0;
     const int32_t* slot = h ? slot1 : slot0;
     const float4* src = reinterpret_cast<const float4*>(mp + ((size_t)wi * 2 + h) * NPAIR);
@@ -26,10 +26,10 @@
 __global__ __launch_bounds__(256) void logits_kernel(const float* __restrict__ m,
                                                      const float* __restrict__ w_qk0,
                                                      const float* __restrict__ w_qk1, int n,
-                                                     float* __restrict__ logits) {
+                                                     float* __restrict__ logits, int h0) {
     __shared__ __attribute__((aligned(16))) float ms[LK][LW + 4];
     __shared__ __attribute__((aligned(16))) float qs[LK][LQ];
-    const int h = blockIdx.z;
+    const int h = blockIdx.z + h0;
     const float* w_qk = h ? w_qk1 : w_qk0;
     const int w0 = blockIdx.y * LW;
     const int q0 = blockIdx.x * LQ;
@@ -158,9 +158,9 @@
 template <int PASSES, bool F16 = false>
 __global__ __launch_bounds__(256) void logits_mfma_kernel(const float* __restrict__ m, const uint4* __restrict__ frag0,
                                                           const uint4* __restrict__ frag1, int n,
-                                                          float* __restrict__ logits) {
+                                                          float* __restrict__ logits, int h0) {
     const int lane = threadIdx.x & 63, wave = threadIdx.x >> 6;
-    const int h = blockIdx.z;
+    const int h = blockIdx.z + h0;
     const int w0 = blockIdx.y * 64;
     const int nb0 = blockIdx.x * 8 + wave * 2;
     const uint4* bfrag = (h ? frag1 : frag0) + (size_t)nb0 * 2 * 64 + lane;
@@ -197,14 +197,8 @@
         }
 }
 
-__global__ __launch_bounds__(256) void attn_kernel(const float* __restrict__ logits,
-                                                   const float* __restrict__ yp,
-                                                   float* __restrict__ alpha_out,
-                                                   float* __restrict__ feat) {
-    __shared__ float a[POOLED + 3];
-    __shared__ float red[256];
-    const int wi = blockIdx.x, h = blockIdx.y;
-    const float* lg = logits + ((size_t)wi * 2 + h) * POOLED;
+__device__ __forceinline__ void softmax_pooled(const float* __restrict__ lg, float* __restrict__ a, float* __restrict__ red,
+                                               float* __restrict__ alpha_out) {
     float mx = -INFINITY;
     for (int q = threadIdx.x; q < POOLED; q += 256) {
         const float v = lg[q];
@@ -236,9 +230,66 @@
     for (int q = threadIdx.x; q < POOLED; q += 256) {
         const float v = a[q] * inv;
         a[q] = v;
-        alpha_out[((size_t)wi * 2 + h) * POOLED + q] = v;
-    }
-    __syncthreads();
+        alpha_out[q] = v;
+    }
+    __syncthreads();
+}
+
+__global__ __launch_bounds__(256) void alpha_kernel(const float* __restrict__ logits, float* __restrict__ alpha_out) {
+    __shared__ float a[POOLED + 3];
+    __shared__ float red[256];
+    const size_t row = (size_t)blockIdx.x * 2 * POOLED;
+    softmax_pooled(logits + row, a, red, alpha_out + row);
+}
+
+__global__ __launch_bounds__(256) void attn_kernel(const float* __restrict__ logits,
+                                                   const float* __restrict__ yp,
+                                                   float* __restrict__ alpha_out,
+                                                   float* __restrict__ feat, int h0) {
+    __shared__ float a[POOLED + 3];
+    __shared__ float red[256];
+    __shared__ float4 part[8][32];
+    const int wi = blockIdx.x, h = blockIdx.y + h0;
+    softmax_pooled(logits + ((size_t)wi * 2 + h) * POOLED, a, red, alpha_out + ((size_t)wi * 2 + h) * POOLED);
+    if (h == 0) {
+        float* ps = reinterpret_cast<float*>(part);
+        if (threadIdx.x < 128) {
+            typedef float ntf4 __attribute__((ext_vector_type(4)));
+            const int g = threadIdx.x >> 5, cq = threadIdx.x & 31;
+            const ntf4* y = reinterpret_cast<const ntf4*>(yp + (size_t)wi * 2 * POOLED * C) + cq;
+            float4 acc = make_float4(0.f, 0.f, 0.f, 0.f);
+            constexpr int STEPS = (POOLED + HEAD_A_STEP_ROWS - 1) / HEAD_A_STEP_ROWS;
+            constexpr int U = 6;
+            for (int s0 = 0; s0 < STEPS; s0 += U) {
+                ntf4 v[U][HEAD_A_WAVE_ROWS];
+#pragma unroll
+                for (int u = 0; u < U; ++u)
+#pragma unroll
+                    for (int p = 0; p < HEAD_A_WAVE_ROWS; ++p) {
+                        const int q = min((s0 + u) * HEAD_A_STEP_ROWS + g * HEAD_A_WAVE_ROWS + p, POOLED - 1);
+                        v[u][p] = __builtin_nontemporal_load(y + (size_t)q * (C / 4));
+                    }
+#pragma unroll
+                for (int u = 0; u < U; ++u)
+#pragma unroll
+                    for (int p = 0; p < HEAD_A_WAVE_ROWS; ++p) {
+                        const int q = (s0 + u) * HEAD_A_STEP_ROWS + g * HEAD_A_WAVE_ROWS + p;
+                        if (q < POOLED) {
+                            const float aq = a[q];
+                            acc.x = fmaf(aq, v[u][p].x, acc.x); acc.y = fmaf(aq, v[u][p].y, acc.y);
+                            acc.z = fmaf(aq, v[u][p].z, acc.z); acc.w = fmaf(aq, v[u][p].w, acc.w);
+                        }
+                    }
+            }
+            *reinterpret_cast<float4*>(ps + g * C + 4 * cq) = acc;
+        }
+        __syncthreads();
+        if (threadIdx.x < C) {
+            const int c = threadIdx.x;
+            feat[(size_t)wi * FEAT + c] = (ps[c] + ps[C + c]) + (ps[2 * C + c] + ps[3 * C + c]);
+        }
+        return;
+    }
     const int cq = threadIdx.x & 31, g = threadIdx.x >> 5;
     const float4* y = reinterpret_cast<const float4*>(yp + ((size_t)wi * 2 + h) * POOLED * C) + cq;
     float4 acc = make_float4(0.f, 0.f, 0.f, 0.f);
@@ -259,7 +310,6 @@
         const float aq = a[q];
         acc.x = fmaf(aq, v.x, acc.x); acc.y = fmaf(aq, v.y, acc.y); acc.z = fmaf(aq, v.z, acc.z); acc.w = fmaf(aq, v.w, acc.w);
     }
-    __shared__ float4 part[8][32];
     part[g][cq] = acc;
     __syncthreads();
     if (threadIdx.x < 128) {
@@ -444,32 +494,46 @@
     }
 }
 
-int launch_backend(gnn_ctx* ctx, int64_t n, int precision, float* scores_dev, void* emb_dev, int emb_dtype, bool dense) {
+static void launch_m_logits(gnn_ctx* ctx, int64_t n, int precision, int h0, int nh) {
+    const DeviceWeights& d = ctx->w;
+    Workspace& ws = ctx->ws;
+    hipLaunchKernelGGL(m_kernel, dim3((unsigned)n, (unsigned)nh), dim3(256), 0, ctx->stream, ws.mp, d.w_bias[0], d.w_bias[1],
+                       d.slot[0], d.slot[1], ws.m, h0);
+    static_assert(QK_KSTEPS % 2 == 0 && QK_NBLK % 8 == 0, "logits_mfma_kernel tiling");
+    static const bool logits_f32 = debug_switch("GNN_LOGITS_F32");
+    const dim3 qk_grid(QK_NBLK / 8, (unsigned)((n + 63) / 64), (unsigned)nh);
+    const uint4* qf0 = reinterpret_cast<const uint4*>(d.wqk_frag[0]);
+    const uint4* qf1 = reinterpret_cast<const uint4*>(d.wqk_frag[1]);
+    if (precision == GNN_PREC_BF16X3 || precision == GNN_PREC_F16C8 || precision == GNN_PREC_F16C6)
+        hipLaunchKernelGGL(logits_mfma_kernel<3>, qk_grid, dim3(256), 0, ctx->stream, ws.m, qf0, qf1, (int)n, ws.logits, h0);
+    else if (precision == GNN_PREC_BF16)
+        hipLaunchKernelGGL(logits_mfma_kernel<1>, qk_grid, dim3(256), 0, ctx->stream, ws.m, qf0, qf1, (int)n, ws.logits, h0);
+    else if (precision == GNN_PREC_F16X3 && !logits_f32)
+        hipLaunchKernelGGL((logits_mfma_kernel<3, true>), qk_grid, dim3(256), 0, ctx->stream, ws.m,
+                           reinterpret_cast<const uint4*>(d.wqk_frag_h[0]), reinterpret_cast<const uint4*>(d.wqk_frag_h[1]), (int)n, ws.logits, h0);
+    else
+        hipLaunchKernelGGL(logits_kernel, dim3((POOLED + LQ - 1) / LQ, (unsigned)((n + LW - 1) / LW), (unsigned)nh), dim3(256), 0,
+                           ctx->stream, ws.m, d.w_qk[0], d.w_qk[1], (int)n, ws.logits, h0);
+}
+
+int launch_head_a_weights(gnn_ctx* ctx, int64_t n, int precision) {
+    launch_m_logits(ctx, n, precision, 0, 1);
+    hipLaunchKernelGGL(alpha_kernel, dim3((unsigned)n), dim3(256), 0, ctx->stream, ctx->ws.logits.get(), ctx->ws.alpha.get());
+    GNN_HIP(hipGetLastError());
+    return GNN_OK;
+}
+
+int launch_backend(gnn_ctx* ctx, int64_t n, int precision, float* scores_dev, void* emb_dev, int emb_dtype, bool dense, bool head_a_done) {
     if (emb_dev && (precision == GNN_PREC_F16C6 || precision == GNN_PREC_F16C8 || (emb_dtype != GNN_EMB_F32 && emb_dtype != GNN_EMB_BF16))) {
         set_error("embeddings: the dense head of this arithmetic does not produce them (f16c6 is frozen), or a bad gnn_emb_dtype");
         return GNN_ERR_ARG;
     }
     const DeviceWeights& d = ctx->w;
     Workspace& ws = ctx->ws;
-    hipLaunchKernelGGL(m_kernel, dim3((unsigned)n, 2), dim3(256), 0, ctx->stream, ws.mp, d.w_bias[0], d.w_bias[1],
-                       d.slot[0], d.slot[1], ws.m);
-    static_assert(QK_KSTEPS % 2 == 0 && QK_NBLK % 8 == 0, "logits_mfma_kernel tiling");
-    static const bool logits_f32 = debug_switch("GNN_LOGITS_F32");
-    const dim3 qk_grid(QK_NBLK / 8, (unsigned)((n + 63) / 64), 2);
-    const uint4* qf0 = reinterpret_cast<const uint4*>(d.wqk_frag[0]);
-    const uint4* qf1 = reinterpret_cast<const uint4*>(d.wqk_frag[1]);
-    if (precision == GNN_PREC_BF16X3 || precision == GNN_PREC_F16C8 || precision == GNN_PREC_F16C6)
-        hipLaunchKernelGGL(logits_mfma_kernel<3>, qk_grid, dim3(256), 0, ctx->stream, ws.m, qf0, qf1, (int)n, ws.logits);
-    else if (precision == GNN_PREC_BF16)
-        hipLaunchKernelGGL(logits_mfma_kernel<1>, qk_grid, dim3(256), 0, ctx->stream, ws.m, qf0, qf1, (int)n, ws.logits);
-    else if (precision == GNN_PREC_F16X3 && !logits_f32)
-        hipLaunchKernelGGL((logits_mfma_kernel<3, true>), qk_grid, dim3(256), 0, ctx->stream, ws.m,
-                           reinterpret_cast<const uint4*>(d.wqk_frag_h[0]), reinterpret_cast<const uint4*>(d.wqk_frag_h[1]), (int)n, ws.logits);
-    else
-        hipLaunchKernelGGL(logits_kernel, dim3((POOLED + LQ - 1) / LQ, (unsigned)((n + LW - 1) / LW), 2), dim3(256), 0,
-                           ctx->stream, ws.m, d.w_qk[0], d.w_qk[1], (int)n, ws.logits);
-    hipLaunchKernelGGL(attn_kernel, dim3((unsigned)n, 2), dim3(256), 0, ctx->stream, ws.logits, ws.yp, ws.alpha,
-                       ws.feat);
+    const int h0 = head_a_done ? 1 : 0, nh = 2 - h0;
+    launch_m_logits(ctx, n, precision, h0, nh);
+    hipLaunchKernelGGL(attn_kernel, dim3((unsigned)n, (unsigned)nh), dim3(256), 0, ctx->stream, ws.logits, ws.yp, ws.alpha,
+                       ws.feat, h0);
     if (!dense) {
         GNN_HIP(hipGetLastError());
         return GNN_OK;
diff --git a/genomad_amd/csrc/gnn_common.h b/genomad_amd/csrc/gnn_common.h
--- a/genomad_amd/csrc/gnn_common.h
+++ b/genomad_amd/csrc/gnn_common.h
@@ -19,6 +19,7 @@
 constexpr int NPAIR = NP * PS;
 constexpr int POOLED = GNN_POOLED;
 constexpr int FEAT = GNN_FEAT;
+constexpr int HEAD_A_STEP_ROWS = 12, HEAD_A_WAVE_ROWS = 3;
 constexpr int HID = GNN_HIDDEN;
 constexpr float LRELU = 0.1f;
 constexpr float BN_EPS = 1e-3f;
@@ -260,6 +261,11 @@
     int last_split = 1;
     bool time_split = true;
     bool c6_pad_skip = true;
+    int fuse_head_a = 1;
+    const uint8_t* head_a_ready = nullptr;
+    int64_t head_a_ready_n = 0;
+    const float* head_a_ready_mp = nullptr;
+    bool head_a_fused = false;
     gnn::DevBuf<unsigned long long> phase_cycles;
     gnn::ContigWorkspace* contig_ws = nullptr;
     gnn::DevBuf<uint8_t> stage_bases;
@@ -355,12 +361,13 @@
                                int64_t n, int64_t n_seg, float* out);
 int launch_front_f32(gnn_ctx* ctx, const uint8_t* bases, int64_t n);
 int launch_backend(gnn_ctx* ctx, int64_t n, int precision, float* scores_dev, void* emb_dev = nullptr, int emb_dtype = GNN_EMB_F32,
-                   bool dense = true);
+                   bool dense = true, bool head_a_done = false);
+int launch_head_a_weights(gnn_ctx* ctx, int64_t n, int precision);
 int check_attrib_args(int precision, int bin, const char* fn);
 int launch_attrib_head(gnn_ctx* ctx, int64_t n, float* scores_dev, const AttribOut& at, int64_t row0);
 int launch_attrib_contrib(gnn_ctx* ctx, int64_t n, const AttribOut& at, int64_t row0);
 int classify_chunks(gnn_ctx* ctx, const uint8_t* bases_dev, int64_t n, int precision, float* scores_dev, bool defer_last = false,
-                    void* emb_dev = nullptr, int emb_dtype = GNN_EMB_F32, const AttribOut* attr = nullptr);
+                    void* emb_dev = nullptr, int emb_dtype = GNN_EMB_F32, const AttribOut* attr = nullptr, bool need_yp = false);
 size_t emb_elem_bytes(int emb_dtype);
 int flush_backend(gnn_ctx* ctx);
 int finish_pending(gnn_ctx* ctx);
@@ -404,7 +411,8 @@
 int launch_front_c6(gnn_ctx* ctx, const uint8_t* bases, int64_t n);
 int launch_front_x3(gnn_ctx* ctx, const uint8_t* bases, int64_t n, int precision);
 int launch_front_tc(gnn_ctx* ctx, const uint8_t* bases, int64_t n);
-int launch_front_tk(gnn_ctx* ctx, const uint8_t* bases, int64_t n);
+int launch_front_tk(gnn_ctx* ctx, const uint8_t* bases, int64_t n, bool store_yp_a = true, const uint8_t* bases_next = nullptr,
+                    int64_t n_next = 0);
 int build_kmer_tables(gnn_ctx* ctx, size_t reserve);
 void free_kmer_tables(gnn_ctx* ctx);
 size_t kmer_tables_bytes();
diff --git a/genomad_amd/csrc/gnn_fused_tk.hip b/genomad_amd/csrc/gnn_fused_tk.hip
--- a/genomad_amd/csrc/gnn_fused_tk.hip
+++ b/genomad_amd/csrc/gnn_fused_tk.hip
@@ -26,7 +26,8 @@
 constexpr int PIDX_OFF = DIRTY_OFF + ((4 + DIRTY_MAX + 15) / 16) * 16;
 constexpr int BKT_OFF = PIDX_OFF + 4 * PIDX_N * 4;
 constexpr int LASTK_OFF = BKT_OFF + 2 * (STEPST + 1) * 4;
-constexpr int SMEMK = LASTK_OFF + 16;
+constexpr int QUADN_OFF = LASTK_OFF + 16;
+constexpr int SMEMK = QUADN_OFF + ((QUAD_N * 2 + 15) / 16) * 16;
 constexpr int X2_PER_WAVE = (BUF_ROWS + 3) / 4;
 static_assert(SMEMK <= 160 * 1024, "LDS budget");
 
@@ -52,6 +53,10 @@
     const float* mp_c;
     unsigned long long* cycles;
     int split;
+    const float* alpha;
+    float* feat;
+    const uint8_t* bases_next;
+    long long n_next;
 };
 
 __device__ __forceinline__ uint32_t quad_of(uint32_t w4) {
@@ -244,7 +249,70 @@
     }
 }
 
-template <bool PROF>
+__global__ __launch_bounds__(512) void head_a_pairs_kernel(ArgsK a) {
+    __shared__ uint16_t quads[QUAD_N];
+    const int tid = threadIdx.x;
+    const int64_t wi = blockIdx.x;
+    const uint8_t* bases = a.bases + wi * W;
+    for (int q = tid; q < QUAD_N; q += 512)
+        quads[q] = q < QUADS ? (uint16_t)quad_of(reinterpret_cast<const uint32_t*>(bases)[q]) : (uint16_t)0;
+    __syncthreads();
+    float* mp = a.mp + wi * 2 * NPAIR;
+    const int32_t* pos = a.pos_sorted[0];
+    constexpr int U = 4;
+    bool any_slow = false;
+    for (int e0 = tid; e0 < NPAIR; e0 += 512 * U) {
+        float v[U];
+#pragma unroll
+        for (int k = 0; k < U; ++k) {
+            const int e = min(e0 + 512 * k, NPAIR - 1);
+            const int u = pos[e];
+            uint32_t code, dirty;
+            kmer_q<9>(quads, max(u - 5, 0), code, dirty);
+            any_slow |= u < 5 || (dirty != 0u && !all_n_tokens<9>(dirty));
+            v[k] = __builtin_nontemporal_load(a.mpa_tbl + ((size_t)e * K9_ROWS + (dirty == 0u ? code : K9_NN)));
+        }
+#pragma unroll
+        for (int k = 0; k < U; ++k)
+            if (e0 + 512 * k < NPAIR) mp[e0 + 512 * k] = v[k];
+    }
+    if (!any_slow) return;
+    for (int e = tid; e < NPAIR; e += 512) {
+        const int u = pos[e];
+        uint32_t code, dirty;
+        kmer_q<9>(quads, max(u - 5, 0), code, dirty);
+        if (u < 5 || (dirty != 0u && !all_n_tokens<9>(dirty))) mp[e] = pair_a_slow(quads, a.x1t_tbl, a.weff_a, e, u);
+    }
+}
+
+__device__ __forceinline__ void alpha_fetch(float (&al)[HEAD_A_WAVE_ROWS], const float* __restrict__ alpha_w, int q0) {
+    typedef const __attribute__((address_space(4))) float* kptr;
+#pragma unroll
+    for (int p = 0; p < HEAD_A_WAVE_ROWS; ++p) al[p] = ((kptr)alpha_w)[min(q0 + p, POOLED - 1)];
+}
+__device__ __forceinline__ void wva_pool_acc(const WvaRows& r, float (&fa)[4], const float (&al)[HEAD_A_WAVE_ROWS], int t0, int hw) {
+    static_assert(FTT / GNN_POOL == HEAD_A_STEP_ROWS && WVA_ROWS_PER_WAVE / GNN_POOL == HEAD_A_WAVE_ROWS, "head A's summation order is that of this kernel's waves");
+    const int q0 = t0 / GNN_POOL + HEAD_A_WAVE_ROWS * hw;
+#pragma unroll
+    for (int p = 0; p < HEAD_A_WAVE_ROWS; ++p) {
+        float row[4];
+#pragma unroll
+        for (int c = 0; c < 4; ++c) {
+            float m = __uint_as_float(r.v[4 * p][c]);
+#pragma unroll
+            for (int j = 1; j < 4; ++j) m = max_nan(m, __uint_as_float(r.v[4 * p + j][c]));
+            const unsigned bits = __float_as_uint(m);
+            const auto sw = __builtin_amdgcn_permlane32_swap(bits, bits, false, false);
+            row[c] = max_nan(__uint_as_float(sw[0]), __uint_as_float(sw[1]));
+        }
+        if (q0 + p < POOLED) {
+#pragma unroll
+            for (int c = 0; c < 4; ++c) fa[c] = fmaf(al[p], row[c], fa[c]);
+        }
+    }
+}
+
+template <bool PROF, bool FUSE_A>
 __global__ __launch_bounds__(512, 2) void fused_front_tk_kernel(ArgsK a) {
     __shared__ __attribute__((aligned(16))) unsigned char smem[SMEMK];
     const unsigned long long t_entry = PROF ? __builtin_readcyclecounter() : 0ull;
@@ -256,15 +324,24 @@
     const int wave = __builtin_amdgcn_readfirstlane(tid >> 6);
     const bool helper = wave >= 4;
     const int hw = wave & 3;
+    uint16_t* quads_n = reinterpret_cast<uint16_t*>(smem + QUADN_OFF);
     const int ht = tid & 255;
     const int64_t wi = blockIdx.x / a.split;
     const int part = blockIdx.x % a.split;
     const uint8_t* bases = a.bases + wi * W;
     float* mp_w[2] = {a.mp + (wi * 2 + 0) * NPAIR, a.mp + (wi * 2 + 1) * NPAIR};
+    const bool do_a = FUSE_A ? (a.bases_next != nullptr && wi < a.n_next) : true;
+    const uint16_t* quads_a = FUSE_A ? quads_n : quads;
     const int woff = hw * WNBLK_B;
 
     for (int q = tid; q < QUAD_N; q += 512)
         quads[q] = q < QUADS ? (uint16_t)quad_of(reinterpret_cast<const uint32_t*>(bases)[q]) : (uint16_t)0;
+    if constexpr (FUSE_A) {
+        if (do_a) {
+            const uint32_t* bn = reinterpret_cast<const uint32_t*>(a.bases_next + wi * W);
+            for (int q = tid; q < QUAD_N; q += 512) quads_n[q] = q < QUADS ? (uint16_t)quad_of(bn[q]) : (uint16_t)0;
+        }
+    }
     if (tid < C) bias_s[tid] = a.conv_b3[tid];
     int* bkt = reinterpret_cast<int*>(smem + BKT_OFF);
     if (tid >= 128 && tid < 128 + 2 * (STEPST + 1)) bkt[tid - 128] = a.bucket_ptr[(tid - 128) / (STEPST + 1)][(tid - 128) % (STEPST + 1)];
@@ -339,7 +416,15 @@
             const wrsrc_t yp_w = make_wrsrc(reinterpret_cast<const unsigned char*>(a.yp + wi * 2 * (size_t)POOLED * C), 2 * POOLED * C * 4);
             WU ring[RINGT];
             prime_tc(ring, cw, 0, lane);
-            wva_pool_store<YP_NT>(w0, yp_w, s_lo * FTT, hw, lane);
+            float fa[4] = {0.f, 0.f, 0.f, 0.f};
+            float aw[HEAD_A_WAVE_ROWS] = {0.f, 0.f, 0.f};
+            const float* alpha_w = a.alpha + wi * 2 * POOLED;
+            if constexpr (FUSE_A) {
+                alpha_fetch(aw, alpha_w, s_lo * HEAD_A_STEP_ROWS + HEAD_A_WAVE_ROWS * hw);
+                wva_pool_acc(w0, fa, aw, s_lo * FTT, hw);
+            } else {
+                wva_pool_store<YP_NT>(w0, yp_w, s_lo * FTT, hw, lane);
+            }
             {
                 const HLane h0 = hlane(smem, (s_lo & 1) * BUF_BYTES, hw, lane);
                 Raw16 rm;
@@ -358,6 +443,7 @@
                 for (int xi = 0; xi < NXI; ++xi)
 #pragma unroll
                     for (int r = 0; r < 16; ++r) acc[xi][r] = 0.f;
+                if constexpr (FUSE_A) alpha_fetch(aw, alpha_w, (step + 1) * HEAD_A_STEP_ROWS + HEAD_A_WAVE_ROWS * hw);
                 GNN_TICK(5)
                 conv_tc(smem, cw, 0, ring, acc, lane, jitter_state);
                 GNN_TICK(0)
@@ -383,12 +469,44 @@
                         Raw16 rm;
                         load_rows(rm, hn, 1);
                         transform_store(rm, hn, 1);
-                        wva_pool_store<YP_NT>(wr, yp_w, t0 + FTT, hw, lane);
+                        if constexpr (FUSE_A) wva_pool_acc(wr, fa, aw, t0 + FTT, hw);
+                        else wva_pool_store<YP_NT>(wr, yp_w, t0 + FTT, hw, lane);
                     }
                     wva_next = wva_step_index_q(quads, t0 + 2 * FTT, hw, lane);
                     asm volatile("s_waitcnt lgkmcnt(0)" ::: "memory");
                     GNN_TICK(4)
                 }
+            }
+            if constexpr (FUSE_A) {
+                if (nsteps < STEPST) {
+                    constexpr int U = 4;
+                    const float4* yc = reinterpret_cast<const float4*>(a.yp_c) + (lane & 31);
+                    for (int st0 = nsteps; st0 < STEPST; st0 += U) {
+                        float4 v[U][HEAD_A_WAVE_ROWS];
+                        float al[U][HEAD_A_WAVE_ROWS];
+#pragma unroll
+                        for (int u = 0; u < U; ++u)
+#pragma unroll
+                            for (int p = 0; p < HEAD_A_WAVE_ROWS; ++p) {
+                                const int q = min((st0 + u) * HEAD_A_STEP_ROWS + HEAD_A_WAVE_ROWS * hw + p, POOLED - 1);
+                                v[u][p] = yc[(size_t)q * (C / 4)];
+                                al[u][p] = alpha_w[q];
+                            }
+#pragma unroll
+                        for (int u = 0; u < U; ++u)
+#pragma unroll
+                            for (int p = 0; p < HEAD_A_WAVE_ROWS; ++p) {
+                                const int q = (st0 + u) * HEAD_A_STEP_ROWS + HEAD_A_WAVE_ROWS * hw + p;
+                                if (st0 + u < STEPST && q < POOLED) {
+                                    fa[0] = fmaf(al[u][p], v[u][p].x, fa[0]);
+                                    fa[1] = fmaf(al[u][p], v[u][p].y, fa[1]);
+                                    fa[2] = fmaf(al[u][p], v[u][p].z, fa[2]);
+                                    fa[3] = fmaf(al[u][p], v[u][p].w, fa[3]);
+                                }
+                            }
+                    }
+                }
+                if (lane < 32) *reinterpret_cast<float4*>(smem + VRING_OFF + (hw * 32 + lane) * 16) = make_float4(fa[0], fa[1], fa[2], fa[3]);
             }
         } else {
             __builtin_amdgcn_s_setprio(3);
@@ -405,15 +523,15 @@
             bool va_slow = false, nxt_slow = false;
             const float* nxt_ptr = a.mpa_tbl;
             auto fetch = [&](int st, bool valid) {
-                nxt.ea = valid ? bkt[st] + ht : 0;
-                nxt.ea_end = valid ? bkt[st + 1] : 0;
+                nxt.ea = valid && do_a ? bkt[st] + ht : 0;
+                nxt.ea_end = valid && do_a ? bkt[st + 1] : 0;
                 nxt.ua = nxt.ea < nxt.ea_end ? a.pos_sorted[0][nxt.ea] : 0;
             };
             auto locate = [&]() {
                 nxt_slow = false;
                 uint32_t code = 0, dirty = 0;
                 if (nxt.ea < nxt.ea_end) {
-                    kmer_q<9>(quads, max(nxt.ua - 5, 0), code, dirty);
+                    kmer_q<9>(quads_a, max(nxt.ua - 5, 0), code, dirty);
                     const bool nn = all_n_tokens<9>(dirty);
                     nxt_slow = nxt.ua < 5 || (dirty != 0u && !nn);
                 }
@@ -484,14 +602,14 @@
                     load_rows(ra, hy, 2);
                 }
                 if (cur.ea < cur.ea_end) {
-                    if (va_slow) va = pair_a_slow(quads, a.x1t_tbl, a.weff_a, cur.ea, cur.ua);
+                    if (va_slow) va = pair_a_slow(quads_a, a.x1t_tbl, a.weff_a, cur.ea, cur.ua);
                     mp_w[0][cur.ea] = va;
                     for (int e = cur.ea + 256; e < cur.ea_end; e += 256) {
                         const int u = a.pos_sorted[0][e];
                         uint32_t code, dirty;
-                        kmer_q<9>(quads, max(u - 5, 0), code, dirty);
+                        kmer_q<9>(quads_a, max(u - 5, 0), code, dirty);
                         const bool nn = all_n_tokens<9>(dirty);
-                        mp_w[0][e] = (u < 5 || (dirty != 0u && !nn)) ? pair_a_slow(quads, a.x1t_tbl, a.weff_a, e, u)
+                        mp_w[0][e] = (u < 5 || (dirty != 0u && !nn)) ? pair_a_slow(quads_a, a.x1t_tbl, a.weff_a, e, u)
                                                                       : a.mpa_tbl[(size_t)e * K9_ROWS + (dirty == 0u ? code : K9_NN)];
                     }
                 }
@@ -514,16 +632,32 @@
         }
     }
     __syncthreads();
+    if constexpr (FUSE_A) {
+        if (tid < C) {
+            const float* ps = reinterpret_cast<const float*>(smem + VRING_OFF);
+            a.feat[wi * FEAT + tid] = (ps[tid] + ps[C + tid]) + (ps[2 * C + tid] + ps[3 * C + tid]);
+        }
+        if (do_a && nsteps < STEPST) {
+            for (int e = bkt[nsteps] + tid; e < NPAIR; e += 512) {
+                const int u = a.pos_sorted[0][e];
+                uint32_t code, dirty;
+                kmer_q<9>(quads_a, max(u - 5, 0), code, dirty);
+                const bool nn = all_n_tokens<9>(dirty);
+                mp_w[0][e] = (u < 5 || (dirty != 0u && !nn)) ? pair_a_slow(quads_a, a.x1t_tbl, a.weff_a, e, u)
+                                                              : a.mpa_tbl[(size_t)e * K9_ROWS + (dirty == 0u ? code : K9_NN)];
+            }
+        }
+    }
     if (nsteps < STEPST && part == a.split - 1) {
         const int q0 = nsteps * (FTT / GNN_POOL);
         const int nrow4 = (POOLED - q0) * (C / 4);
-        for (int i = tid; i < 2 * nrow4; i += 512) {
+        for (int i = tid + (FUSE_A ? nrow4 : 0); i < 2 * nrow4; i += 512) {
             const int h = i >= nrow4, j = i - h * nrow4;
             const size_t off = (size_t)h * POOLED * C + (size_t)q0 * C + (size_t)j * 4;
             *reinterpret_cast<float4*>(a.yp + wi * 2 * (size_t)POOLED * C + off) = *reinterpret_cast<const float4*>(a.yp_c + off);
         }
 #pragma unroll
-        for (int h = 0; h < 2; ++h)
+        for (int h = FUSE_A ? 1 : 0; h < 2; ++h)
             for (int e = a.bucket_ptr[h][nsteps] + tid; e < NPAIR; e += 512) mp_w[h][e] = a.mp_c[h * NPAIR + e];
     }
     if constexpr (PROF) {
@@ -651,12 +785,16 @@
     a.weff_a = d.weff_sorted[0];
     a.cycles = nullptr;
     a.split = 1;
+    a.alpha = nullptr;
+    a.feat = nullptr;
+    a.bases_next = nullptr;
+    a.n_next = 0;
 }
 
 static void launch(const ArgsK& a, bool prof, unsigned nwin, hipStream_t stream) {
     const unsigned n = nwin * (unsigned)a.split;
-    if (prof) hipLaunchKernelGGL((fused_front_tk_kernel<true>), dim3(n), dim3(512), 0, stream, a);
-    else hipLaunchKernelGGL((fused_front_tk_kernel<false>), dim3(n), dim3(512), 0, stream, a);
+    if (prof) hipLaunchKernelGGL((fused_front_tk_kernel<true, false>), dim3(n), dim3(512), 0, stream, a);
+    else hipLaunchKernelGGL((fused_front_tk_kernel<false, false>), dim3(n), dim3(512), 0, stream, a);
 }
 
 }
@@ -760,7 +898,7 @@
     return rc;
 }
 
-int launch_front_tk(gnn_ctx* ctx, const uint8_t* bases, int64_t n) {
+int launch_front_tk(gnn_ctx* ctx, const uint8_t* bases, int64_t n, bool store_yp_a, const uint8_t* bases_next, int64_t n_next) {
     using namespace tk;
     if (!ctx->w.tk_x2_tbl || !ctx->w.tk_mpa_tbl) {
         set_error("f16x3tk: the k-mer tables have not been built (gnn_build_kmer_tables)");
@@ -779,7 +917,29 @@
     a.cycles = ctx->phase_cycles;
     if (ctx->time_split && n > 0 && ctx->cu_count > 0) a.split = (int)std::max<int64_t>(1, std::min<int64_t>(4, ctx->cu_count / n));
     ctx->last_split = a.split;
-    launch(a, ctx->phase_cycles != nullptr, (unsigned)n, ctx->stream);
+    const bool fuse = ctx->fuse_head_a && !store_yp_a && a.split == 1 && !ctx->phase_cycles && n > 0;
+    ctx->head_a_fused = fuse;
+    const bool ready = fuse && ctx->head_a_ready == bases && ctx->head_a_ready_n >= n && ctx->head_a_ready_mp == ctx->ws.mp.get();
+    ctx->head_a_ready = nullptr;
+    if (fuse) {
+        a.alpha = ctx->ws.alpha;
+        a.feat = ctx->ws.feat;
+        if (!ready) {
+            hipLaunchKernelGGL(head_a_pairs_kernel, dim3((unsigned)n), dim3(512), 0, ctx->stream, a);
+            GNN_HIP(hipGetLastError());
+        }
+        if (bases_next && n_next > 0 && !(reinterpret_cast<uintptr_t>(bases_next) & 3u)) {
+            a.bases_next = bases_next;
+            a.n_next = std::min<int64_t>(n_next, n);
+            ctx->head_a_ready = bases_next;
+            ctx->head_a_ready_n = a.n_next;
+            ctx->head_a_ready_mp = ctx->ws.mp.get();
+        }
+        if (int rc = launch_head_a_weights(ctx, n, GNN_PREC_F16X3)) return rc;
+        hipLaunchKernelGGL((fused_front_tk_kernel<false, true>), dim3((unsigned)n), dim3(512), 0, ctx->stream, a);
+    } else {
+        launch(a, ctx->phase_cycles != nullptr, (unsigned)n, ctx->stream);
+    }
     GNN_HIP(hipGetLastError());
     return GNN_OK;
 }
diff --git a/include/genomad_nn.h b/include/genomad_nn.h
--- a/include/genomad_nn.h
+++ b/include/genomad_nn.h
@@ -257,6 +257,9 @@
 int gnn_debug_set_pad_skip(gnn_ctx* ctx, int on);
 
 int gnn_debug_set_time_split(gnn_ctx* ctx, int on);
+int gnn_debug_set_fuse_head_a(gnn_ctx* ctx, int on);
+int gnn_debug_last_head_a_fused(gnn_ctx* ctx, int* fused);
+int gnn_debug_workspace(gnn_ctx* ctx, int which, int64_t n_windows, float* out_host);
 int gnn_debug_last_split(gnn_ctx* ctx, int* workgroups_per_window);
 
 int gnn_debug_pack_c6(const float* w, int k, int n, uint32_t* out, size_t out_words, size_t* need_words);
```
